# nanleij/ClusteredLowRankSolver.jl

Measured on AMD Instinct MI355X. Metric: interior-point iterations/sec, higher is better.
Workload: dtype f64x5 (multi-word fp64: 5 limbs per number, ~262 bits; problem data f64x5); 1 GPU; SpherePacking cohnelkies(8,15): d=8, 2d=30; 2 clusters P=32, blocks 16x16 r1 + 1x1 dense, N=31; whole interior-point iterations with the reference's default options at its precision (prec=256 -> 5 limbs), 55 per solve; clusters=2, n_free=31, limbs=5, data_limbs=5, multi_gpu=single GPU

## Files before the change

### clusteredlowranksolver.jl_amd/csrc/clrs_hip.hip

```cpp
#include <hip/hip_runtime.h>

#include <algorithm>
#include <array>
#include <climits>
#include <cmath>
#include <cstdio>
#include <cstdlib>
#include <cstring>
#include <map>
#include <string>
#include <vector>

#include "../../include/clrs_hip.h"
#include "clrs_kernels.hip.h"
#include "clrs_fused.hip.h"
#include "clrs_assemble_w3.hip.h"
#include "clrs_assemble_w4.hip.h"
#include "clrs_assemble_w5.hip.h"
#include "clrs_solve_small.hip.h"
#include "clrs_factor_small.hip.h"
#include "clrs_ipm.hip.h"

using namespace clrs;
typedef long long i64;

static thread_local std::string g_last_error;
static int fail(int code, const std::string &msg) {
    g_last_error = msg;
    return code;
}
extern "C" void clrs_set_last_error(const char *msg) { g_last_error = msg ? msg : ""; }
#define HIPCHECK(expr)                                                                                   \
    do {                                                                                                 \
        hipError_t e_ = (expr);                                                                          \
        if (e_ != hipSuccess)                                                                            \
            return fail(CLRS_ERR_HIP, std::string(#expr) + ": " + hipGetErrorString(e_));                \
    } while (0)

static const int INFO_NONE = 0x7f7f7f7f;

static int g_cfg_fused_assemble = 1;
static int g_cfg_split_blocks = 1;
static int g_cfg_fused_factor = 1;
static int g_cfg_wave_assemble = 1;
static int g_cfg_wave2_assemble = 1;
static int g_cfg_wave5_assemble = 1;
static int g_cfg_wave4_assemble = 1;
static int g_cfg_wave3_assemble = 1;
static int g_cfg_dense_block = 1;
static int g_cfg_trsm_blockinv = 1;
static int g_cfg_potrf_levels = 1;
static int g_cfg_pairing_tri = 1;
static int g_cfg_factor_aug = 1;
static int g_cfg_dense_wave = 1;
static int g_cfg_factor_small = 1;
static int g_cfg_solve_small_max = 32768;
static int g_cfg_ipm_wmfma = 3;
int g_cfg_mw_stream_words = 1;
int g_cfg_mw_pipeline64 = 1;
int g_cfg_mw_zt_small_maxn = 64;
int g_cfg_mw_pipeline_x = 1;
int g_cfg_mw_pipeline_x_min = 24;
int g_cfg_mw_sharded_factor_limbs = 1;
int g_cfg_mw_pipeline = 1;
int g_cfg_mw_refine_predictor = 0;
int g_cfg_mw_refine = 1;
int g_cfg_mw_affine_corrector = 1;
int g_cfg_mw_factor_limbs = 0;
int g_cfg_mw_exact_products = 1;
static int g_cfg_solve_small2 = 1;
static const int LDS_BUDGET_DOUBLES = 20000;

enum StepKind { STEP_MEMCPY, STEP_GEMM, STEP_TRSM, STEP_POTRF, STEP_GATHER_S, STEP_GATHER_SCALAR, STEP_SUB, STEP_MEMSET_INFO, STEP_ZERO_UPPER, STEP_FUSED_ASSEMBLE, STEP_SMALL_POTRF, STEP_CLUSTER_FACTOR, STEP_GEMV_T, STEP_CSOLVE_FWD, STEP_Q_SOLVE, STEP_CSOLVE_BWD, STEP_SUM_SLABS, STEP_ASSEMBLE_W1, STEP_GRAM_SMALL, STEP_ASSEMBLE_W2, STEP_SOLVE_SMALL, STEP_DENSE_BLOCK, STEP_ASSEMBLE_W3, STEP_FACTOR_SMALL, STEP_SUM_S_SLABS, STEP_TRTRI32, STEP_DENSE_T32, STEP_TRTRI_DIAG, STEP_COPY2D, STEP_CHOL_LEVEL, STEP_CHOL_PACK, STEP_CHOL_UNPACK, STEP_ASSEMBLE_W4, STEP_ASSEMBLE_W5, STEP_NKINDS };
static const char *const STEP_NAMES[STEP_NKINDS] = {"hipMemcpyAsync(D2D)", "k_gemm_f64_t", "k_trsm_diag", "k_potrf_diag", "k_schur_gather",
                                                    "k_gather_scalar", "k_sub", "hipMemsetAsync", "k_zero_upper", "k_cluster_assemble", "k_small_potrf", "k_cluster_factor", "k_gemv_t",
                                                    "k_cluster_solve_fwd", "k_q_solve", "k_cluster_solve_bwd", "k_sum_slabs", "k_cluster_assemble_w1", "k_gram_small", "k_cluster_assemble_w2", "k_solve_small", "k_dense_block", "k_cluster_assemble_w3", "k_factor_small", "k_sum_S_slabs", "k_trtri32", "k_dense_T32", "k_trtri_diag", "k_copy2d", "k_chol_level", "k_chol_pack", "k_chol_unpack", "k_cluster_assemble_w4", "k_cluster_assemble_w5"};
static const int KT_MAX_EVENTS = 8192;

struct Step {
    StepKind kind;
    int grid = 0;
    void *d0 = nullptr, *d1 = nullptr, *d2 = nullptr;
    void *dst = nullptr;
    const void *src = nullptr;
    size_t bytes = 0;
    i64 n = 0;
    int nmax = 0;
    int aux0 = 0, aux1 = 0;
    bool s_inverse = false;
};

struct Plan {
    std::vector<Step> steps;
    hipGraphExec_t graph = nullptr;
    const void *captured[8] = {nullptr, nullptr, nullptr, nullptr, nullptr, nullptr, nullptr, nullptr};
    int launches() const { return (int)steps.size(); }
};

struct DeviceArena {
    char *base = nullptr;
    size_t size = 0, used = 0;
};

struct TrsmJob {
    const double *L;
    int ldl, n;
    double *B;
    int ldb, nrhs;
};
struct PotrfJob {
    double *A;
    int lda, n, code;
    int stop = 0;
// ... 2453 lines not shown
    c->kt_kinds.clear();
    return 0;
}

extern "C" int clrs_set_kernel_timing(clrs_ctx *c, int kind) {
    if (!c || kind < -2 || kind >= STEP_NKINDS) return fail(CLRS_ERR_INVALID, "bad kernel kind");
    int rc = kt_collect(c);
    if (rc) return rc;
    c->kt_kind = kind;
    for (int k = 0; k < STEP_NKINDS; k++) { c->kt_total[k] = 0; c->kt_count[k] = 0; }
    return 0;
}

extern "C" int clrs_get_kernel_times(clrs_ctx *c, int max_kinds, double *seconds, int64_t *launches) {
    if (!c || !seconds || !launches) return fail(CLRS_ERR_INVALID, "null argument");
    int rc = kt_collect(c);
    if (rc) return rc;
    for (int k = 0; k < max_kinds && k < STEP_NKINDS; k++) { seconds[k] = c->kt_total[k]; launches[k] = c->kt_count[k]; }
    return STEP_NKINDS;
}

extern "C" int clrs_config_set(const char *key, int value) {
    if (!key) return fail(CLRS_ERR_INVALID, "null argument");
    if (!std::strcmp(key, "fused_assemble")) { g_cfg_fused_assemble = value; return 0; }
    if (!std::strcmp(key, "split_blocks")) { g_cfg_split_blocks = value; return 0; }
    if (!std::strcmp(key, "fused_factor")) { g_cfg_fused_factor = value; return 0; }
    if (!std::strcmp(key, "wave_assemble")) { g_cfg_wave_assemble = value; return 0; }
    if (!std::strcmp(key, "wave2_assemble")) { g_cfg_wave2_assemble = value; return 0; }
    if (!std::strcmp(key, "wave3_assemble")) { g_cfg_wave3_assemble = value; return 0; }
    if (!std::strcmp(key, "wave4_assemble")) { g_cfg_wave4_assemble = value; return 0; }
    if (!std::strcmp(key, "wave5_assemble")) { g_cfg_wave5_assemble = value; return 0; }
    if (!std::strcmp(key, "dense_block")) { g_cfg_dense_block = value; return 0; }
    if (!std::strcmp(key, "dense_wave")) { g_cfg_dense_wave = value; return 0; }
    if (!std::strcmp(key, "factor_aug")) { g_cfg_factor_aug = value; return 0; }
    if (!std::strcmp(key, "pairing_tri")) { g_cfg_pairing_tri = value; return 0; }
    if (!std::strcmp(key, "potrf_levels")) { g_cfg_potrf_levels = value; return 0; }
    if (!std::strcmp(key, "trsm_blockinv")) { g_cfg_trsm_blockinv = value; return 0; }
    if (!std::strcmp(key, "solve_small2")) { g_cfg_solve_small2 = value; return 0; }
    if (!std::strcmp(key, "factor_small")) { g_cfg_factor_small = value; return 0; }
    if (!std::strcmp(key, "pin_limit")) { PIN_LIMIT = (size_t)std::max(value, 0); return 0; }
    if (!std::strcmp(key, "ipm_wmfma")) { g_cfg_ipm_wmfma = value; return 0; }
    if (!std::strcmp(key, "solve_small_max")) { g_cfg_solve_small_max = value; return 0; }
    if (!std::strcmp(key, "mw_exact_products")) { g_cfg_mw_exact_products = value; return 0; }
    if (!std::strcmp(key, "mw_refine")) { g_cfg_mw_refine = value; return 0; }
    if (!std::strcmp(key, "mw_factor_limbs")) { g_cfg_mw_factor_limbs = value; return 0; }
    if (!std::strcmp(key, "mw_affine_corrector")) { g_cfg_mw_affine_corrector = value; return 0; }
    if (!std::strcmp(key, "mw_pipeline")) { g_cfg_mw_pipeline = value; return 0; }
    if (!std::strcmp(key, "mw_pipeline64")) { g_cfg_mw_pipeline64 = value; return 0; }
    if (!std::strcmp(key, "mw_zt_small_maxn")) { g_cfg_mw_zt_small_maxn = value; return 0; }
    if (!std::strcmp(key, "mw_pipeline_x")) { g_cfg_mw_pipeline_x = value; return 0; }
    if (!std::strcmp(key, "mw_pipeline_x_min")) { g_cfg_mw_pipeline_x_min = value; return 0; }
    if (!std::strcmp(key, "mw_sharded_factor_limbs")) { g_cfg_mw_sharded_factor_limbs = value; return 0; }
    if (!std::strcmp(key, "mw_stream_words")) { g_cfg_mw_stream_words = value; return 0; }
    if (!std::strcmp(key, "mw_refine_predictor")) { g_cfg_mw_refine_predictor = value; return 0; }
    return fail(CLRS_ERR_INVALID, std::string("unknown configuration key ") + key);
}

#ifdef CLRS_W3_STAMPS
extern "C" int clrs_debug_cf_stamps(clrs_ctx *c, uint64_t out[16]) {
    if (!c || !out) return fail(CLRS_ERR_INVALID, "null argument");
    HIPCHECK(hipStreamSynchronize(c->stream));
    HIPCHECK(hipMemcpyFromSymbol(out, HIP_SYMBOL(g_cf_stamps), 16 * sizeof(uint64_t)));
    return 0;
}
extern "C" int clrs_debug_ss2_stamps(clrs_ctx *c, uint64_t out[16]) {
    if (!c || !out) return fail(CLRS_ERR_INVALID, "null argument");
    HIPCHECK(hipStreamSynchronize(c->stream));
    HIPCHECK(hipMemcpyFromSymbol(out, HIP_SYMBOL(g_ss2_stamps), 16 * sizeof(uint64_t)));
    return 0;
}
extern "C" int clrs_debug_w3_stamps(clrs_ctx *c, uint64_t out[16]) {
    if (!c || !out) return fail(CLRS_ERR_INVALID, "null argument");
    HIPCHECK(hipStreamSynchronize(c->stream));
    HIPCHECK(hipMemcpyFromSymbol(out, HIP_SYMBOL(g_w3_stamps), 16 * sizeof(uint64_t)));
    return 0;
}
#endif

extern "C" int clrs_debug_stamps(clrs_ctx *c, uint64_t out[64]) {
    if (!c || !out) return fail(CLRS_ERR_INVALID, "null argument");
    if (!c->ftables.stamps) { std::memset(out, 0, 64 * sizeof(uint64_t)); return 0; }
    HIPCHECK(hipStreamSynchronize(c->stream));
    HIPCHECK(hipMemcpy(out, c->ftables.stamps, 64 * sizeof(uint64_t), hipMemcpyDeviceToHost));
    return 0;
}

extern "C" int clrs_fused_clusters(const clrs_ctx *c) { return c ? c->n_fused_clusters : 0; }
extern "C" int clrs_wave_clusters(const clrs_ctx *c) { return c ? c->n_wave_clusters + c->n_wave2_clusters : 0; }
extern "C" int clrs_wave2_clusters(const clrs_ctx *c) { return c ? c->n_wave2_clusters : 0; }
extern "C" int clrs_wave4_clusters(const clrs_ctx *c) { return c ? c->n_wave4_clusters : 0; }
extern "C" int clrs_wave5_clusters(const clrs_ctx *c) { return c ? c->n_wave5_clusters : 0; }

extern "C" const char *clrs_kernel_name(int kind) { return (kind >= 0 && kind < STEP_NKINDS) ? STEP_NAMES[kind] : ""; }

extern "C" const char *clrs_strerror(int code) {
    switch (code) {
        case CLRS_OK: return "ok";
        case CLRS_ERR_INVALID: return "invalid argument or malformed SDP description";
        case CLRS_ERR_HIP: return "HIP runtime error";
        case CLRS_ERR_NO_DEVICE: return "no usable HIP device";
        case CLRS_ERR_STATE: return "call order violated";
        default: return code > 0 ? "factorisation failure (non-positive pivot)" : "unknown error";
    }
}
extern "C" const char *clrs_last_error(void) { return g_last_error.c_str(); }
extern "C" const char *clrs_version(void) { return "clrs-hip 0.1.0 (gfx950)"; }
// ... 127 lines not shown
```

### clusteredlowranksolver.jl_amd/csrc/clrs_mw.hip

```cpp
#include <hip/hip_runtime.h>

#include <dlfcn.h>

#include <algorithm>
#include <condition_variable>
#include <cstdio>
#include <cstring>
#include <map>
#include <mutex>
#include <string>
#include <tuple>
#include <vector>

#include "../../include/clrs_hip.h"
#include "clrs_mw_kernels.hip.h"
#include "clrs_mw_pipe.hip.h"
#include "clrs_mw_exact.hip.h"
#include "clrs_mw_ipm.hip.h"
#include "clrs_mw_rank.hip.h"
#include "clrs_mw_inst.h"
#ifdef MW_SPLIT_UNITS
MW_KERNELS_ALL(extern template, 4)
MW_KERNELS_ALL(extern template, 5)
MW_KERNELS_ALL(extern template, 6)
MW_KERNELS_ALL(extern template, 8)
MW_KERNELS_ALL(extern template, 10)
#endif

typedef long long i64;

extern int g_cfg_mw_stream_words;
extern int g_cfg_mw_pipeline64;
extern int g_cfg_mw_zt_small_maxn;
extern int g_cfg_mw_pipeline_x, g_cfg_mw_pipeline_x_min;
extern int g_cfg_mw_sharded_factor_limbs;
extern int g_cfg_mw_pipeline;
extern int g_cfg_mw_refine_predictor;
extern int g_cfg_mw_refine;
extern int g_cfg_mw_exact_products;
extern int g_cfg_mw_affine_corrector;
extern int g_cfg_mw_factor_limbs;
extern "C" void clrs_set_last_error(const char *msg);

static int mw_fail(int code, const std::string &msg) {
    clrs_set_last_error(msg.c_str());
    return code;
}
#define MWCHECK(expr)                                                                                    \
    do {                                                                                                 \
        hipError_t e_ = (expr);                                                                          \
        if (e_ != hipSuccess) return mw_fail(CLRS_ERR_HIP, std::string(#expr) + ": " + hipGetErrorString(e_)); \
    } while (0)

typedef struct { char internal[128]; } mw_nccl_id;
struct MwNccl {
    void *lib = nullptr;
    int (*GetUniqueId)(mw_nccl_id *) = nullptr;
    int (*CommInitRank)(void **, int, mw_nccl_id, int) = nullptr;
    int (*CommDestroy)(void *) = nullptr;
    int (*AllGather)(const void *, void *, size_t, int, void *, hipStream_t) = nullptr;
    const char *(*GetErrorString)(int) = nullptr;
};
static MwNccl g_nccl;
static int mw_nccl_load() {
    if (g_nccl.lib) return 0;
    const char *names[] = {"librccl.so.1", "librccl.so", "/opt/rocm/lib/librccl.so.1"};
    void *h = nullptr;
    for (const char *n : names) if ((h = dlopen(n, RTLD_NOW | RTLD_NOLOAD))) break;
    for (const char *n : names) { if (h) break; h = dlopen(n, RTLD_NOW | RTLD_GLOBAL); }
    if (!h) return mw_fail(CLRS_ERR_INVALID, std::string("RCCL is not available: ") + dlerror());
    g_nccl.GetUniqueId = (int (*)(mw_nccl_id *))dlsym(h, "ncclGetUniqueId");
    g_nccl.CommInitRank = (int (*)(void **, int, mw_nccl_id, int))dlsym(h, "ncclCommInitRank");
    g_nccl.CommDestroy = (int (*)(void *))dlsym(h, "ncclCommDestroy");
    g_nccl.AllGather = (int (*)(const void *, void *, size_t, int, void *, hipStream_t))dlsym(h, "ncclAllGather");
    g_nccl.GetErrorString = (const char *(*)(int))dlsym(h, "ncclGetErrorString");
    if (!g_nccl.GetUniqueId || !g_nccl.CommInitRank || !g_nccl.CommDestroy || !g_nccl.AllGather) return mw_fail(CLRS_ERR_INVALID, "RCCL symbols missing");
    g_nccl.lib = h;
    return 0;
}
#define NCCLCHECK(expr)                                                                                                          \
    do {                                                                                                                         \
        int r_ = (expr);                                                                                                         \
        if (r_ != 0) return mw_fail(CLRS_ERR_HIP, std::string(#expr) + ": " + (g_nccl.GetErrorString ? g_nccl.GetErrorString(r_) : "RCCL error")); \
// ... 35 lines not shown
    bool xinv_valid = false;
    bool lds_x = false, lds_q = false, lds_zt_L = false, dense_two = false;
    int nw_factor = 1;
    int maxcnt = 0;
    double *vz = nullptr;
    bool wide_solve = false;
    const double *ride_fwd = nullptr;
    const int *ride_wait = nullptr;
    int ride_wait_value = 0;
    bool fwd_rode = false;
    int n_one_term = 0, n_many_term = 0;
    int sa_lanes = MW_SA_W;
    int maxTb = 0;
    size_t sm_x = 0, sm_zt = 0, sm_dense = 0, sm_factor = 0, sm_q = 0, sm_fwd = 0, sm_mid = 0, sm_bwd = 0;
    int *h_info = nullptr;
    double *d_Xin = nullptr, *d_Xc = nullptr, *d_Y = nullptr, *d_rx = nullptr, *d_ry = nullptr, *d_dx = nullptr, *d_dy = nullptr;
    bool assembled = false, factored = false;
    bool timing = false;
    hipEvent_t ev[8] = {nullptr, nullptr, nullptr, nullptr, nullptr, nullptr, nullptr, nullptr};
    double times[6] = {0, 0, 0, 0, 0, 0};
    double cnt_mul = 0;
    double cnt_factor = 0, cnt_solve = 0;
    struct MwIpm *ipm = nullptr;
    size_t sm_bp_diag = 0, sm_bp_panel = 0, sm_bp_inv = 0;
    std::vector<MwBp> bp_S, bp_Q;
    const MwBp *d_bp = nullptr;
    bool any_lds_cluster = false;
    void *comm = nullptr;
    void *comm_side = nullptr;
    clrs_mw_local_group *lgroup = nullptr;
    bool local_factored = false, fwd_done = false;
    const double *split_rhs_x = nullptr;
    bool refine_ready = false;
    MwdDev mwd = {};
    int mwd_blocks = 0, mwd_tasks = 0;
    size_t sm_mwd = 0;
    MwxDev mwx = {};
    int mwx_blocks = 0, mwx_maxU16 = 0;
    MwsDev mws = {};
    int mws_blocks = 0;
    int mws_turns = 1;
    size_t sm_mws = 0;
    bool pipe_bp = false;
    bool pipe_S64 = false;
    bool pipe_X = false;
    unsigned long long *pipe_pcx = nullptr;
    double *xpipe_L = nullptr, *xpipe_rd = nullptr;
    int *xpipe_info = nullptr;
    bool pipe_S = false, pipe_Q = false;
    unsigned long long *pipe_pc64 = nullptr;
    int pipe_pcQ = 0;
    unsigned pipe_epoch = 0;
    bool stream_words = true;
    bool refine_skip_next = false;
    int refine_predictor = 0;
    int refine = 1;
    bool ipm_arms_info = false;
    int kf_low = 0, kf_entry = 0;
};

template <class T>
static int mw_upload(clrs_mw_ctx *c, const std::vector<T> &h, const T **d) {
    T *p = nullptr;
    size_t bytes = std::max<size_t>(h.size(), 1) * sizeof(T);
    MWCHECK(hipMalloc((void **)&p, bytes));
    c->allocs.push_back(p);
    if (!h.empty()) MWCHECK(hipMemcpy(p, h.data(), h.size() * sizeof(T), hipMemcpyHostToDevice));
    *d = p;
    return 0;
}
static int mw_dmalloc(clrs_mw_ctx *c, double **d, i64 n) {
    size_t bytes = (size_t)std::max<i64>(n, 1) * sizeof(double);
    MWCHECK(hipMalloc((void **)d, bytes));
    c->allocs.push_back(*d);
    MWCHECK(hipMemset(*d, 0, bytes));
    return 0;
}

#define MW_CASE(Kc, Dc, ...) if (c_K_ == Kc && c_D_ == Dc) { constexpr int KK = Kc; constexpr int DD = Dc; __VA_ARGS__; } else
#define MW_DISPATCH(ctx, ...)                                                                                       \
    do {                                                                                                            \
        const int c_K_ = (ctx)->K, c_D_ = (ctx)->DK;                                                                \
        MW_CASE(2, 1, __VA_ARGS__) MW_CASE(2, 2, __VA_ARGS__) MW_CASE(3, 1, __VA_ARGS__) MW_CASE(3, 2, __VA_ARGS__)  \
        MW_CASE(4, 1, __VA_ARGS__) MW_CASE(4, 2, __VA_ARGS__) MW_CASE(5, 1, __VA_ARGS__) MW_CASE(5, 2, __VA_ARGS__)  \
        MW_CASE(6, 1, __VA_ARGS__) MW_CASE(6, 2, __VA_ARGS__) MW_CASE(8, 1, __VA_ARGS__) MW_CASE(8, 2, __VA_ARGS__)  \
        MW_CASE(10, 1, __VA_ARGS__) MW_CASE(10, 2, __VA_ARGS__)                                                      \
        MW_CASE(3, 3, __VA_ARGS__) MW_CASE(4, 4, __VA_ARGS__) MW_CASE(5, 5, __VA_ARGS__) MW_CASE(6, 6, __VA_ARGS__)  \
        MW_CASE(8, 8, __VA_ARGS__) MW_CASE(10, 10, __VA_ARGS__)                                                      \
        return mw_fail(CLRS_ERR_INVALID, "limbs must be 2..6, 8 or 10 and data limbs 1, 2 or the limbs");           \
    } while (0)

template <class F>
static int mw_set_lds(F kernel, size_t bytes) {
    if (bytes > 48 * 1024) MWCHECK(hipFuncSetAttribute((const void *)kernel, hipFuncAttributeMaxDynamicSharedMemorySize, (int)bytes));
    return 0;
}

extern "C" void clrs_mw_destroy(clrs_mw_ctx *c);
static void mw_ipm_free(clrs_mw_ctx *c);
static int mw_launch_xrd(clrs_mw_ctx *c, const double *d_Xc);

extern "C" int clrs_mw_create_opts(const clrs_sdp_desc *d, int data_limbs, int device, int limbs, const clrs_mw_options *opts, clrs_mw_ctx **out);
extern "C" int clrs_mw_create(const clrs_sdp_desc *d, int device, int limbs, clrs_mw_ctx **out) {
    return clrs_mw_create_opts(d, 1, device, limbs, nullptr, out);
}
extern "C" int clrs_mw_create_ex(const clrs_sdp_desc *d, int data_limbs, int device, int limbs, clrs_mw_ctx **out) {
// ... 200 lines not shown
            (one ? c->n_one_term : c->n_many_term)++;
        }
    }
    c->cnt_mul = cnt_mul;
    for (int j = 0; j < J; j++) {
        const double P = c->clu[j].P;
        c->cnt_factor += P * P * P / 6.0 + 0.5 * P * P * N + 0.5 * P * (double)N * N;
        c->cnt_solve += P * P + 2.0 * P * N;
    }
    c->cnt_factor += (double)N * N * N / 6.0;
    c->cnt_solve += (double)N * N;
    const size_t lim = MW_LDS_MAX / sizeof(double);
    {
        size_t nn = (size_t)c->maxn * c->maxn * K;
        size_t bcw = MW_POTRF_SCR(K, (size_t)c->maxn);
        c->lds_x = nn + bcw <= lim;
        size_t xneed = (c->lds_x ? nn : 0) + bcw;
        for (auto &k : c->blk) {
            const size_t one = (size_t)k.n * k.n * K + MW_POTRF_SCR(K, (size_t)k.n) + (size_t)K * k.n;
            const size_t two = one + (size_t)MW_TRI(k.n) * K;
            k.inv = !c->lds_x ? 0 : two <= lim ? 1 : one <= lim ? 2 : 0;
            if (k.inv) xneed = std::max(xneed, k.inv == 1 ? two : one);
        }
        c->all_inv = !c->blk.empty();
        for (auto &k : c->blk) c->all_inv = c->all_inv && (k.kind != 0 || k.inv != 0);
        c->sm_x = xneed * 8;
        size_t zt = (size_t)c->maxn * MW_CT * K;
        c->lds_zt_L = zt + nn <= lim;
        c->sm_zt = (zt + (c->lds_zt_L ? nn : 0)) * 8;
        if (zt > lim) MW_BAIL(CLRS_ERR_INVALID, "PSD block too large for the multi-word kernels");
        size_t maxnd = 0;
        for (auto &k : c->blk) if (k.kind != 0 && k.n > 1) maxnd = std::max(maxnd, (size_t)k.n);
        if (maxnd * maxnd * K > lim) MW_BAIL(CLRS_ERR_INVALID, "dense block too large for the multi-word kernels");
        c->dense_two = 2 * maxnd * maxnd * K <= lim;
        c->sm_dense = (c->dense_two ? 2 : 1) * maxnd * maxnd * K * 8;
        size_t fmax = 0;
        for (auto &q : c->clu) {
            const size_t need = ((size_t)q.P * q.P + (size_t)MW_TRI(q.P)) * K + MW_POTRF_SCR(K, (size_t)q.P);
            q.lds = need <= lim ? 1 : 0;
            if (q.lds) fmax = std::max(fmax, need);
        }
        c->sm_factor = std::max<size_t>(fmax, 1) * 8;
        c->nw_factor = std::max(1, std::min(MW_INV_WG, 256 / std::max(J, 1)));
        c->sm_fwd = 2 * (size_t)c->maxP * K * 8;
        c->sm_bwd = 3 * (size_t)c->maxP * K * 8;
        const size_t qn = (size_t)N * N * K;
        const size_t qneed = qn + (size_t)MW_TRI(N) * K + MW_POTRF_SCR(K, (size_t)N);
        c->lds_q = qneed <= lim;
        c->sm_q = (c->lds_q ? qneed : 1) * 8;
        c->sm_mid = 2 * (size_t)std::max(N, 1) * K * 8;
        if (c->sm_fwd > MW_LDS_MAX || c->sm_mid > MW_LDS_MAX) MW_BAIL(CLRS_ERR_INVALID, "cluster too large for the multi-word solve kernels");
    }
    MW_DISPATCH(c, {
        MW_TRY(mw_set_lds(k_mw_potrf_x<KK>, c->sm_x)); MW_TRY(mw_set_lds(k_mw_zt<KK, DD>, c->sm_zt)); MW_TRY(mw_set_lds((k_mw_dense_t<KK, DD>), c->sm_dense));
        constexpr int KC = mw_kc(KK);
        const size_t bw = std::min(c->sm_mid + c->sm_bwd, MW_LDS_MAX);
        MW_TRY(mw_set_lds(k_mw_factor<KK>, c->sm_factor)); MW_TRY(mw_set_lds(k_mw_potrf_q<KK>, c->lds_q ? std::max(c->sm_q, c->sm_fwd) : c->sm_fwd));
        MW_TRY(mw_set_lds(k_mw_solve_fwd<KK>, c->sm_fwd)); MW_TRY(mw_set_lds((k_mw_solve_mid<KK, KK>), c->sm_mid)); MW_TRY(mw_set_lds((k_mw_solve_mid<KK, KC>), c->sm_mid));
        MW_TRY(mw_set_lds((k_mw_solve_bwd<KK, KK, DD, 0>), bw)); MW_TRY(mw_set_lds((k_mw_solve_bwd<KK, KK, DD, 1>), bw)); MW_TRY(mw_set_lds((k_mw_solve_bwd<KK, KK, DD, 2>), bw));
        MW_TRY(mw_set_lds((k_mw_solve_bwd<KK, KC, DD, 1>), bw)); MW_TRY(mw_set_lds((k_mw_solve_bwd<KK, KC, DD, 2>), bw));
    });
    std::vector<long long> mws_off((size_t)std::max(NB, 1), -1);
    {
        const int S = mws_slices(K);
        std::vector<float> hVs;
        std::vector<int> hVe, hve_off((size_t)std::max(NB, 1), 0), hsv((size_t)std::max(NB, 1), 0);
        for (int b = 0; b < NB; b++) {
            const MwBlk &k = c->blk[b];
            if (k.kind != 0 || !k.inv || k.n > 32) continue;
            const int n = k.n, U = k.U, np = (n + 3) & ~3, n16 = (n + 15) & ~15, U16 = (U + 15) & ~15, rV = mws_rowstride(U16);
            if ((n16 / 16) * (U16 / 16) > 4 || mws_lds_bytes(S, mws_sv_class(S, 1), n, U) > MW_LDS_MAX) continue;
            if (2 * (n16 / 16) * (U16 / 16) > 4) c->mws_turns = 2;
            mws_off[b] = (long long)hVs.size();
            hve_off[b] = (int)hVe.size();
            hVs.resize(hVs.size() + (size_t)S * np * rV, 0.0f);
            hVe.resize(hVe.size() + U16, 0);
            float *dst = hVs.data() + mws_off[b];
            int sv = 0;
            for (int u = 0; u < U; u++) {
                double mx = 0;
                for (int i = 0; i < n; i++) mx = std::max(mx, std::fabs(hVl[0][k.v_off + (i64)u * n + i]));
                const int e = mwk::mws_exponent(mx);
                hVe[hve_off[b] + u] = e;
                for (int i = 0; i < n; i++) {
                    mwa::mw<2> x;
                    x.l[0] = hVl[0][k.v_off + (i64)u * n + i];
                    x.l[1] = DK > 1 ? hVl[1][k.v_off + (i64)u * n + i] : 0.0;
                    double r0 = std::ldexp(x.l[0], -e), r1 = std::ldexp(x.l[1], -e);
                    for (int s = 0; s < S; s++) {
                        const double g = std::ldexp(1.0, -(s + 1) * MWS_BETA), C = 0x1.8p52 * g;
                        volatile double tv = r0 + C;
                        const double t = tv - C;
                        const float dgt = (float)(t * std::ldexp(1.0, (s + 1) * MWS_BETA));
                        dst[(size_t)s * np * rV + (size_t)i * rV + mws_col(i, u, U16)] = dgt;
                        if (dgt != 0.0f) sv = std::max(sv, s + 1);
                        r0 -= t;
                        double sm, er;
                        mwa::two_sum(r0, r1, sm, er);
                        r0 = sm; r1 = er;
                    }
                }
            }
            if (mws_lds_bytes(S, mws_sv_class(S, sv), n, U) > MW_LDS_MAX) {
                hVs.resize((size_t)mws_off[b]); hVe.resize((size_t)hve_off[b]);
                mws_off[b] = -1;
                continue;
            }
// ... 141 lines not shown
                for (int r = 0; r < P; r++) hBs[(size_t)l * std::max<i64>(Bp, 1) + c->clu[j].coff + r + (i64)a * xlen] = d->B[(i64)l * Bp + off + r + (i64)a * P];
            off += (i64)P * N;
        }
    }
    q.Vp = std::max<i64>((i64)hVl[0].size(), 1); q.dAp = std::max<i64>((i64)hdAl[0].size(), 1); q.lamp = std::max<i64>(T, 1); q.Bp = std::max<i64>(Bp, 1);
    hV.assign((size_t)q.Vp * DK, 0.0);
    hdA.assign((size_t)q.dAp * DK, 0.0);
    for (int l = 0; l < DK; l++) {
        std::copy(hVl[l].begin(), hVl[l].end(), hV.begin() + (size_t)l * q.Vp);
        std::copy(hdAl[l].begin(), hdAl[l].end(), hdA.begin() + (size_t)l * q.dAp);
    }
    MW_TRY(mw_upload(c, c->blk, &q.blk)); MW_TRY(mw_upload(c, c->clu, &q.clu));
    MW_TRY(mw_upload(c, lr_list, &q.lr_list)); MW_TRY(mw_upload(c, dn_list, &q.dn_list));
    MW_TRY(mw_upload(c, hV, &q.V)); MW_TRY(mw_upload(c, hvrow, &q.vrow));
    MW_TRY(mw_upload(c, st_a, &q.st_a)); MW_TRY(mw_upload(c, st_b, &q.st_b)); MW_TRY(mw_upload(c, st_lam, &q.st_lam));
    MW_TRY(mw_upload(c, htptr, &q.tptr));
    MW_TRY(mw_upload(c, st_orig, &q.st_orig)); MW_TRY(mw_upload(c, st_p, &q.st_p)); MW_TRY(mw_upload(c, st_war, &q.st_war)); MW_TRY(mw_upload(c, st_wac, &q.st_wac));
    MW_TRY(mw_upload(c, st_trl, &q.st_trl)); MW_TRY(mw_upload(c, st_trd, &q.st_trd)); MW_TRY(mw_upload(c, st_flag, &q.st_flag));
    MW_TRY(mw_upload(c, ay_a, &q.ay_a)); MW_TRY(mw_upload(c, ay_b, &q.ay_b)); MW_TRY(mw_upload(c, ay_blk, &q.ay_blk));
    MW_TRY(mw_upload(c, hdA, &q.dA)); MW_TRY(mw_upload(c, hdmap, &q.dmap)); MW_TRY(mw_upload(c, hdense_p, &q.dense_p));
    {
        std::sort(drow_pairs.begin(), drow_pairs.end());
        std::vector<int> hptr((size_t)xlen + 1, 0), hblk, hen;
        for (auto &t : drow_pairs) hptr[(size_t)std::get<0>(t) + 1]++;
        for (i64 g = 0; g < xlen; g++) hptr[(size_t)g + 1] += hptr[(size_t)g];
        for (auto &t : drow_pairs) { hblk.push_back(std::get<1>(t)); hen.push_back(std::get<2>(t)); }
        MW_TRY(mw_upload(c, hptr, &q.drow_ptr)); MW_TRY(mw_upload(c, hblk, &q.drow_blk)); MW_TRY(mw_upload(c, hen, &q.drow_en));
        q.dn_big = 0;
        for (auto &k : c->blk) if (k.kind != 0) { c->maxcnt = std::max(c->maxcnt, k.cnt); if (k.n > 1) q.dn_big = 1; }
        q.maxcnt = c->maxcnt;
    }
    MW_TRY(mw_upload(c, hBs, &q.B));
    MW_TRY(mw_dmalloc(c, &q.Z, q.zlen * K)); MW_TRY(mw_dmalloc(c, &q.Tm, q.zlen * K));
    MW_TRY(mw_dmalloc(c, &q.GX, q.glen * K)); MW_TRY(mw_dmalloc(c, &q.GY, q.glen * K));
    MW_TRY(mw_dmalloc(c, &q.W, q.wlen * K)); MW_TRY(mw_dmalloc(c, &q.Sd, q.sdlen * K));
    MW_TRY(mw_dmalloc(c, &q.S, Slen * K)); MW_TRY(mw_dmalloc(c, &q.LB, xlen * (i64)N * K)); MW_TRY(mw_dmalloc(c, &q.Q, (i64)N * N * K));
    MW_TRY(mw_dmalloc(c, &q.Si, Slen * K)); MW_TRY(mw_dmalloc(c, &q.Qi, (i64)N * N * K));

    MW_TRY(mw_dmalloc(c, &q.Xf, xyoff * K)); MW_TRY(mw_dmalloc(c, &q.Xb, xyoff * K)); MW_TRY(mw_dmalloc(c, &q.Xi, xyoff * K));
    MW_TRY(mw_dmalloc(c, &q.xrd, rdoff * K)); MW_TRY(mw_dmalloc(c, &q.srd, xlen * K)); MW_TRY(mw_dmalloc(c, &q.qrd, (i64)N * K));
    MW_TRY(mw_dmalloc(c, &q.t, xlen * K)); MW_TRY(mw_dmalloc(c, &q.u, (i64)J * N * K)); MW_TRY(mw_dmalloc(c, &q.AY, T * K));
    q.AX = nullptr;
    q.aff_mu = q.aff_rhs = q.aff_t = q.aff_u = nullptr; q.aff_wait = nullptr; q.ride2_rhs = nullptr; q.ride2_t = q.ride2_u = nullptr;
    MW_TRY(mw_dmalloc(c, &c->vz, 2 * (i64)N * K));
    MW_TRY(mw_dmalloc(c, &q.S0, Slen * K)); MW_TRY(mw_dmalloc(c, &q.ub, (i64)J * N * K));
    MW_TRY(mw_dmalloc(c, &q.rx2, xlen * K)); MW_TRY(mw_dmalloc(c, &q.dx2, xlen * K));
    MW_TRY(mw_dmalloc(c, &q.u2, (i64)N * K)); MW_TRY(mw_dmalloc(c, &q.dy2, (i64)N * K));
    q.uadd = nullptr;
    c->refine = cfg_refine;
    c->refine_predictor = cfg_refine_pred;
    {
        const char *e = std::getenv("CLRS_MW_STREAM_WORDS");
        c->stream_words = e && *e ? std::atoi(e) != 0 : g_cfg_mw_stream_words != 0;
    }
    c->wide_solve = c->maxP > 64 || N > 64;
    MW_TRY(mw_dmalloc(c, &c->d_Xin, xyoff * K)); MW_TRY(mw_dmalloc(c, &c->d_Xc, xyoff * K)); MW_TRY(mw_dmalloc(c, &c->d_Y, xyoff * K));
    MW_TRY(mw_dmalloc(c, &c->d_rx, xlen * K)); MW_TRY(mw_dmalloc(c, &c->d_dx, xlen * K));
    MW_TRY(mw_dmalloc(c, &c->d_ry, (i64)N * K)); MW_TRY(mw_dmalloc(c, &c->d_dy, (i64)N * K));
    {
        int *info = nullptr;
        MWCHECK(hipMalloc((void **)&info, 2 * sizeof(int)));
        c->allocs.push_back(info);
        q.info = info;
        int init[2] = {MW_INFO_NONE, MW_INFO_NONE};
        MWCHECK(hipMemcpy(info, init, sizeof(init), hipMemcpyHostToDevice));
        int *pc = nullptr;
        MWCHECK(hipMalloc((void **)&pc, (size_t)(2 * J + 3) * sizeof(int)));
        c->allocs.push_back(pc);
        MWCHECK(hipMemset(pc, 0, (size_t)(2 * J + 3) * sizeof(int)));
        q.pcnt = pc;
    }
    {
        for (int j = 0; j < J; j++) {
            const MwClu &cl = c->clu[j];
            if (cl.lds) { c->any_lds_cluster = true; continue; }
            c->bp_S.push_back(MwBp{q.S + cl.Soff, q.Si + cl.Soff, q.srd + cl.coff, q.Slen, q.xlen, cl.P, cl.P, j + 1, 0, (int)c->bp_S.size(), 0});
        }
        if (N > 0) c->bp_Q.push_back(MwBp{q.Q, q.Qi, q.qrd, (i64)N * N, (i64)N, N, N, J + 1, 0, (int)c->bp_S.size(), 0});
        std::vector<MwBp> all = c->bp_S;
        all.insert(all.end(), c->bp_Q.begin(), c->bp_Q.end());
        MW_TRY(mw_upload(c, all, &c->d_bp));
    }
    {
        bool small = c->maxP <= MWP_N;
        for (auto &cl : c->clu) small = small && cl.lds;
        c->pipe_S = cfg_pipe != 0 && (K <= 6 || cfg_pipe >= 2) && small && (i64)J * ((MWP_N / MWP_W) + MWP_WW) <= 256;
        c->pipe_Q = (cfg_pipe >= 2 || (cfg_pipe == 1 && K <= 6 && N > MWP_W)) && N > 0 && N <= MWP_N;
        bool lds_all = !c->clu.empty();
        for (auto &cl : c->clu) lds_all = lds_all && cl.lds;
        c->pipe_S64 = cfg_pipe != 0 && K <= 6 && lds_all && c->maxP > MWP_N && c->maxP <= MWP_N64 && (i64)J * 16 <= 256 && g_cfg_mw_pipeline64 != 0 &&
                      (cfg_pipe >= 2 || c->maxP >= 48);
        const size_t nbp = c->bp_S.size() + c->bp_Q.size();
        const bool any_bp = !c->bp_S.empty() || (N > 0 && !c->lds_q);
        c->pipe_bp = cfg_pipe != 0 && any_bp && (i64)std::max<size_t>(c->bp_S.size(), 1) * ((MWP_N / MWP_W) + MWP_WW) <= 256;
        q.pipe_pc = nullptr;
        q.pipe_stamps = nullptr;
        q.pipe_bp = 0;
        {
            bool all_inv = c->d.NB > 0 && c->lds_x;
            int maxn_x = 0;
            i64 working = 0;
            for (auto &kb : c->blk) {
                all_inv = all_inv && kb.inv == 1;
                maxn_x = std::max(maxn_x, kb.n);
                working += 2 * ((kb.n + MWP_W - 1) / MWP_W + (kb.n > MWP_N ? MWP_N64 / MWP_W : MWP_WW));
            }
            c->pipe_X = cfg_pipe != 0 && K <= 6 && all_inv && maxn_x <= MWP_N64 && g_cfg_mw_pipeline_x != 0 &&
                        (cfg_pipe >= 2 || (maxn_x >= g_cfg_mw_pipeline_x_min && working <= 256));
            if (c->pipe_X) {
                double *pcx = nullptr, *ti = nullptr;
                MW_TRY(mw_dmalloc(c, &pcx, (i64)2 * c->d.NB * MWP_PC_WORDS_N(K, MWP_N64)));
                c->pipe_pcx = (unsigned long long *)pcx;
                MW_TRY(mw_dmalloc(c, &c->xpipe_L, c->d.xylen * K));
                MW_TRY(mw_dmalloc(c, &c->xpipe_rd, c->d.xrdlen * K));
                MW_TRY(mw_dmalloc(c, &ti, c->d.NB + 1));
                c->xpipe_info = (int *)ti;
                MW_DISPATCH(c, { if constexpr (KK <= 6) { MW_TRY(mw_set_lds(k_mw_potrf_x_pipe<KK>, MWP_LDS_ALONE64)); } });
            }
        }
        if (c->pipe_S64) {
            const size_t words64 = (size_t)J * MWP_PC_WORDS_N(K, MWP_N64);
            unsigned long long *pc64 = nullptr;
            if (hipMalloc((void **)&pc64, words64 * sizeof(unsigned long long)) != hipSuccess) MW_BAIL(CLRS_ERR_HIP, "hipMalloc failed");
            c->allocs.push_back(pc64);
            if (hipMemset(pc64, 0xff, words64 * sizeof(unsigned long long)) != hipSuccess) MW_BAIL(CLRS_ERR_HIP, "hipMemset failed");
            c->pipe_pc64 = pc64;
            MW_DISPATCH(c, { if constexpr (KK <= 6) { MW_TRY(mw_set_lds(k_mw_factor_pipe64<KK>, MWP_LDS_ALONE64)); } });
        }
        if (c->pipe_S || c->pipe_Q || c->pipe_bp) {
            const size_t own = (size_t)(c->pipe_S ? J : 0) + 1;
            const size_t words = (own + (c->pipe_bp ? nbp : 0)) * MWP_PC_WORDS(K);
            unsigned long long *pc = nullptr;
            if (hipMalloc((void **)&pc, words * sizeof(unsigned long long)) != hipSuccess) MW_BAIL(CLRS_ERR_HIP, "hipMalloc failed");
            c->allocs.push_back(pc);
            if (hipMemset(pc, 0xff, words * sizeof(unsigned long long)) != hipSuccess) MW_BAIL(CLRS_ERR_HIP, "hipMemset failed");
            q.pipe_pc = pc;
            c->pipe_pcQ = c->pipe_S ? J : 0;
            q.pipe_q = c->pipe_pcQ;
            q.pipe_bp = (int)own;
            MW_DISPATCH(c, {
                MW_TRY(mw_set_lds(k_mw_factor_pipe<KK>, MWP_LDS_ALONE));
                MW_TRY(mw_set_lds(k_mw_potrf_q_pipe<KK>, std::max<size_t>(MWP_LDS_ALONE, c->sm_fwd)));
                MW_TRY(mw_set_lds(k_mw_bp_diag_pipe<KK>, std::max<size_t>(MWP_LDS_ALONE, c->sm_factor)));
            });
        }
    }
    const int MW_PB = MW_PB_OF(K);
    c->sm_bp_diag = ((size_t)MW_POTRF_SCR(K, MW_PB) + (size_t)K * MW_PB * MW_PB + (size_t)K * MW_TRI(MW_PB) + (size_t)K * MW_PB) * 8;
    c->sm_bp_panel = (size_t)K * MW_BP_PR * MW_PB * 8;
    c->sm_bp_inv = (size_t)K * MW_PB * MW_BP_IC * 8;
    MW_DISPATCH(c, { MW_TRY(mw_set_lds(k_mw_bp_diag<KK>, std::max(c->sm_bp_diag, c->sm_factor))); MW_TRY(mw_set_lds(k_mw_bp_panel<KK>, c->sm_bp_panel)); MW_TRY(mw_set_lds(k_mw_bp_inv<KK>, c->sm_bp_inv)); MW_TRY(mw_set_lds(k_mw_bp_inv_row<KK>, c->sm_bp_inv)); });
    q.rank = 0; q.world = 1; q.gathered = 0;
    MW_TRY(mw_dmalloc(c, &q.Qg, (i64)N * N * K)); MW_TRY(mw_dmalloc(c, &q.ug, (i64)N * K));
    {
        bool all_lds = true;
        for (auto &cl : c->clu) all_lds = all_lds && cl.lds;
        (void)all_lds;
        const bool may = mw_kf_of(K) < K && c->refine == 1;
        c->kf_low = may ? mw_kf_of(K) : K;
// ... 13 lines not shown
    return 0;
#undef MW_BAIL
#undef MW_TRY
}

extern "C" void clrs_mw_destroy(clrs_mw_ctx *c) {
    if (!c) return;
    (void)hipSetDevice(c->device);
    if (c->stream) (void)hipStreamSynchronize(c->stream);
    mw_ipm_free(c);
    if (c->comm && g_nccl.CommDestroy) { (void)g_nccl.CommDestroy(c->comm); c->comm = nullptr; }
    if (c->comm_side && g_nccl.CommDestroy) { (void)g_nccl.CommDestroy(c->comm_side); c->comm_side = nullptr; }
    if (c->lgroup) { std::lock_guard<std::mutex> lk(c->lgroup->m); c->lgroup->attached--; c->lgroup = nullptr; }
    for (void *p : c->allocs) (void)hipFree(p);
    for (auto &e : c->ev) if (e) (void)hipEventDestroy(e);
    if (c->h_info) (void)hipHostFree(c->h_info);
    if (c->stream && c->own_stream) (void)hipStreamDestroy(c->stream);
    delete c;
}

extern "C" int clrs_mw_limbs(const clrs_mw_ctx *c) { return c ? c->K : 0; }
extern "C" void *clrs_mw_stream(clrs_mw_ctx *c) { return c ? (void *)c->stream : nullptr; }
extern "C" int clrs_mw_set_stream(clrs_mw_ctx *c, void *stream) {
    if (!c) return mw_fail(CLRS_ERR_INVALID, "null context");
    if (c->own_stream && c->stream) { (void)hipStreamSynchronize(c->stream); (void)hipStreamDestroy(c->stream); }
    c->stream = (hipStream_t)stream;
    c->own_stream = false;
    return 0;
}
extern "C" int clrs_mw_get_dims(const clrs_mw_ctx *c, clrs_dims *o) {
    if (!c || !o) return mw_fail(CLRS_ERR_INVALID, "null argument");
    o->xy_len = c->d.xylen; o->x_len = c->d.xlen; o->S_len = c->d.Slen; o->n_terms = c->d.T;
    o->n_free = c->d.N; o->n_clusters = c->d.J; o->n_blocks = c->d.NB; o->reserved = c->K;
    return 0;
}
extern "C" int clrs_mw_get_unique_count(const clrs_mw_ctx *c, int32_t block, int32_t *n_unique) {
    if (!c || !n_unique || block < 0 || block >= c->d.NB) return mw_fail(CLRS_ERR_INVALID, "bad argument");
    *n_unique = c->blk[block].U;
    return 0;
}
extern "C" int clrs_mw_set_timing(clrs_mw_ctx *c, int on) {
    if (!c) return mw_fail(CLRS_ERR_INVALID, "null context");
    c->timing = on != 0;
    return 0;
}
extern "C" int clrs_mw_get_counters(const clrs_mw_ctx *c, double *assemble_muladds, double *factor_muladds, double *solve_muladds) {
    if (!c) return mw_fail(CLRS_ERR_INVALID, "null context");
    if (assemble_muladds) *assemble_muladds = c->cnt_mul;
    if (factor_muladds) *factor_muladds = c->cnt_factor;
    if (solve_muladds) *solve_muladds = c->cnt_solve;
    return 0;
}

static int mw_reset_info(clrs_mw_ctx *c, int which) {
    if (c->ipm_arms_info) return 0;
    MWCHECK(hipMemsetAsync(c->d.info + which, 0x7f, sizeof(int), c->stream));
    return 0;
}
static int mw_read_info(clrs_mw_ctx *c, int which, int *status) {
    MWCHECK(hipMemcpyAsync(c->h_info + which, c->d.info + which, sizeof(int), hipMemcpyDeviceToHost, c->stream));
    MWCHECK(hipStreamSynchronize(c->stream));
    *status = c->h_info[which] == MW_INFO_NONE ? 0 : c->h_info[which];
    return 0;
}

static int mw_cholesky_blocks_dev2(clrs_mw_ctx *c, const double *d_X, double *d_Xchol, const double *d_Y2, double *d_Yi, int *d_yfail) {
    if (!c || !d_X || !d_Xchol) return mw_fail(CLRS_ERR_INVALID, "null argument");
    MWCHECK(hipSetDevice(c->device));
    int rc;
    if ((rc = mw_reset_info(c, 1))) return rc;
    if (c->d.NB == 0) return 0;
    const int grid = d_Y2 ? 2 * c->d.NB : c->d.NB;
    bool in_mem = false;
    for (auto &k : c->blk) in_mem = in_mem || k.inv == 2 || mw_x_shares(k);
    if (c->pipe_X) {
        c->pipe_epoch = (c->pipe_epoch + 1) & 0x3ffffff;
        MW_DISPATCH(c, { if constexpr (KK <= 6) { hipLaunchKernelGGL(k_mw_potrf_x_pipe<KK>, dim3(mwp_blocks64(grid)), dim3(MWP_NT64), MWP_LDS_ALONE64, c->stream, c->d, d_X, d_Xchol, d_Y2, d_Yi, d_yfail,
                                                                     c->xpipe_L, c->xpipe_rd, c->xpipe_info, c->pipe_pcx, c->pipe_epoch); } });
    } else
    MW_DISPATCH(c, hipLaunchKernelGGL(k_mw_potrf_x<KK>, dim3(grid, in_mem && c->lds_x ? MW_INV_WG : 1), dim3(MW_PT), c->sm_x, c->stream, c->d, d_X, d_Xchol, c->lds_x ? 1 : 0, d_Y2, d_Yi, d_yfail));
    MWCHECK(hipGetLastError());
    c->xinv_valid = true;
    return 0;
}
extern "C" int clrs_mw_cholesky_blocks_dev(clrs_mw_ctx *c, const double *d_X, double *d_Xchol) { return mw_cholesky_blocks_dev2(c, d_X, d_Xchol, nullptr, nullptr, nullptr); }
extern "C" int clrs_mw_sync_status_cholesky(clrs_mw_ctx *c) {
    if (!c) return mw_fail(CLRS_ERR_INVALID, "null context");
    int st = 0, rc;
    if ((rc = mw_read_info(c, 1, &st))) return rc;
    return st;
}

extern "C" int clrs_mw_schur_assemble_dev(clrs_mw_ctx *c, const double *d_Xchol, const double *d_Y) {
    if (!c || !d_Xchol || !d_Y) return mw_fail(CLRS_ERR_INVALID, "null argument");
    MWCHECK(hipSetDevice(c->device));
    const MwDev &q = c->d;
    if (c->timing) MWCHECK(hipEventRecord(c->ev[0], c->stream));
    MW_DISPATCH(c, {
        const bool exact = c->mws_blocks > 0 && c->xinv_valid;
        bool dense_done = exact && q.ndn && !q.dn_big;
        const int pair_grid = q.nlr + (dense_done ? q.ndn : 0);
        if constexpr (DD <= 2) {
            if (exact && c->mws_turns == 1) hipLaunchKernelGGL((k_mws_pair<KK, DD, 1>), dim3(pair_grid), dim3(MWS_NT), c->sm_mws, c->stream, q, c->mws, d_Y);
            else if (exact) hipLaunchKernelGGL((k_mws_pair<KK, DD, 2>), dim3(pair_grid), dim3(MWS_NT), c->sm_mws, c->stream, q, c->mws, d_Y);
        }
        if (q.nlr && !(exact && c->mws_blocks == q.nlr)) {
            MwDev q2 = q;
            q2.mws_on = exact ? 1 : 0;
            const int gper = MW_NT / MW_GRAM_W;
            const int zt_ct = (c->xinv_valid && c->all_inv && (i64)q.nlr * c->maxU <= 2048 && c->maxn <= g_cfg_mw_zt_small_maxn) ? 2 : MW_CT;
            hipLaunchKernelGGL((k_mw_zt<KK, DD>), dim3((c->maxU + zt_ct - 1) / zt_ct, q.nlr), dim3(MW_NT), c->sm_zt, c->stream, q2, d_Y, c->lds_zt_L ? 1 : 0, c->xinv_valid ? 1 : 0, zt_ct);
            const bool ride_gram = !dense_done && q.ndn && !q.dn_big;
            dense_done = dense_done || ride_gram;
            q2.mwx_on = c->mwx_blocks > 0 ? 1 : 0;
            hipLaunchKernelGGL((k_mw_gram<KK, DD>), dim3((c->maxU * (c->maxU + 1) / 2 + gper - 1) / gper, q.nlr + (ride_gram ? q.ndn : 0)), dim3(MW_NT), 0, c->stream, q2, d_Y);
            if (q2.mwx_on) {
                const int nt = c->mwx_maxU16 / 16;
                hipLaunchKernelGGL(k_mwx_slice<KK>, dim3(nt, 2, q.nlr), dim3(MWS_NT), 0, c->stream, q2, c->mwx);
                hipLaunchKernelGGL(k_mwx_gram<KK>, dim3((nt * (nt + 1) / 2 + MWS_NT / 64 - 1) / (MWS_NT / 64), 2, q.nlr), dim3(MWS_NT), 0, c->stream, q2, c->mwx);
            }
        }
        if (q.ndn && !dense_done) {
            const bool panels = c->xinv_valid && c->maxn_dense > 16 && c->maxn_dense <= MW_NT;
            MwDev q3 = q;
            q3.mwd_on = (panels && c->mwd_blocks > 0) ? 1 : 0;
            hipLaunchKernelGGL((k_mw_dense_t<KK, DD>), dim3(q.ndn, q.dn_big ? c->maxcnt : 1), dim3(MW_NT), c->sm_dense, c->stream, q3, d_Y, c->xinv_valid ? 1 : 0, c->dense_two ? 1 : 0, panels ? 1 : 0);
            if (panels) {
                const int pcmin = std::max(1, MW_NT / c->maxn_dense);
                if (c->mwd_blocks < q.ndn)
                    hipLaunchKernelGGL((k_mw_dense_tp<KK, DD>), dim3(q.ndn, c->maxcnt, (c->maxn_dense + pcmin - 1) / pcmin), dim3(MW_NT), (size_t)2 * KK * MW_NT * 8, c->stream, q3, d_Y);
                c->mwd.stamps = c->mws.stamps;
                if constexpr (DD <= 2) { if (q3.mwd_on) hipLaunchKernelGGL((k_mwx_dense<KK, DD>), dim3(c->mwd_tasks), dim3(MWS_NT), c->sm_mwd, c->stream, q3, c->mwd, d_Y); }
            }
            const int pairs = c->maxcnt * (c->maxcnt + 1) / 2;
            const int ds_lanes = c->maxn_dense * c->maxn_dense <= 128 ? 8 : c->maxn_dense * c->maxn_dense <= 512 ? 16 : 64;
            if (q.dn_big) hipLaunchKernelGGL((k_mw_dense_s<KK, DD>), dim3(q.ndn, (pairs + MW_NT / ds_lanes - 1) / (MW_NT / ds_lanes)), dim3(MW_NT), 0, c->stream, q, ds_lanes);
        }
        if (c->n_many_term) hipLaunchKernelGGL((k_mw_saccum<KK, DD>), dim3((c->maxP * (c->maxP + 1) / 2 * c->sa_lanes + MW_NT - 1) / MW_NT, q.J), dim3(MW_NT), 0, c->stream, q, c->sa_lanes);
        if (c->n_one_term) hipLaunchKernelGGL((k_mw_saccum_one<KK, DD>), dim3((c->maxP * (c->maxP + 1) / 2 + MW_NT - 1) / MW_NT, q.J), dim3(MW_NT), 0, c->stream, q, c->n_many_term ? 0 : 1);
    });
    MWCHECK(hipGetLastError());
    if (c->timing) MWCHECK(hipEventRecord(c->ev[1], c->stream));
    c->assembled = true;
    c->factored = false;
    c->local_factored = false;
    return 0;
}


extern "C" int clrs_comm_unique_id(void *id128) {
    if (!id128) return mw_fail(CLRS_ERR_INVALID, "null argument");
    int rc = mw_nccl_load();
    if (rc) return rc;
    NCCLCHECK(g_nccl.GetUniqueId((mw_nccl_id *)id128));
    return 0;
}

extern "C" int clrs_mw_set_shard(clrs_mw_ctx *c, int rank, int world) {
    if (!c || world < 1 || rank < 0 || rank >= world) return mw_fail(CLRS_ERR_INVALID, "bad rank / world");
    MWCHECK(hipSetDevice(c->device));
    MWCHECK(hipStreamSynchronize(c->stream));
    MwDev &q = c->d;
    if (world != q.world) {
// ... 694 lines not shown
```

### clusteredlowranksolver.jl_amd/csrc/clrs_mw_inst.h

```cpp
#ifndef CLRS_MW_INST_H
#define CLRS_MW_INST_H

#define MW_KERNELS_K(X, K)                                                                                             \
    X __global__ void k_mw_potrf_x<K>(const MwDev, const double *, double *, int, const double *, double *, int *);    \
    X __global__ void k_mw_factor<K>(const MwDev);                                                                     \
    X __global__ void k_mw_qgram<K>(const MwDev, int);                                                                 \
    X __global__ void k_mw_potrf_q<K>(const MwDev, int, const double *, const int *, int);                             \
    X __global__ void k_mw_factor_pipe<K>(const MwDev, unsigned);                                                      \
    X __global__ void k_mw_factor_pipe64<K>(const MwDev, unsigned);                                                    \
    X __global__ void k_mw_potrf_x_pipe<K>(const MwDev, const double *, double *, const double *, double *, int *, double *, double *, int *, unsigned long long *, unsigned); \
    X __global__ void k_mw_potrf_q_pipe<K>(const MwDev, unsigned, const double *, const int *, int);                   \
    X __global__ void k_mw_bp_diag_pipe<K>(const MwDev, const MwBp *, int, int, unsigned, int, int);                   \
    X __global__ void k_mw_bp_inv_row<K>(const MwDev, const MwBp *, int);                                               \
    X __global__ void k_mw_qsum<K>(const MwDev);                                                                       \
    X __global__ void k_mw_bp_diag<K>(const MwDev, const MwBp *, int, int);                                             \
    X __global__ void k_mw_bp_panel<K>(const MwDev, const MwBp *, int);                                                \
    X __global__ void k_mw_bp_syrk<K>(const MwDev, const MwBp *, int);                                                 \
    X __global__ void k_mw_bp_inv<K>(const MwDev, const MwBp *, int);                                                  \
    X __global__ void k_mw_bp_finish<K>(const MwDev, const MwBp *);                                                    \
    X __global__ void k_mw_usum<K>(const MwDev);                                                                       \
    X __global__ void k_mw_keep_S<K>(const MwDev);                                                                     \
    X __global__ void k_mw_solve_fwd<K>(const MwDev, const double *);                                                  \
    X __global__ void k_mw_solve_mid<K, K>(const MwDev, const double *, double *);                                     \
    X __global__ void k_mw_solve_mid<K, mw_kc(K)>(const MwDev, const double *, double *);                              \
    X __global__ void k_mw_solve_wide<K>(const MwDev, int, const double *, const double *, double *, double *, double *);\
    X __global__ void k_mw_xrd<K>(const MwDev, const double *);                                                        \
    X __global__ void k_mwi_R<K>(const MwDev, const MwIpmDev, int);                                                    \
    X __global__ void k_mwi_Z<K>(const MwDev, const MwIpmDev, int, int);                                               \
    X __global__ void k_mwi_Zi<K>(const MwDev, const MwIpmDev, int);                                                   \
    X __global__ void k_mwi_bmm<K>(const MwDev, const MwIpmDev, int, int);                                             \
    X __global__ void k_mwx_slice<K>(const MwDev, const MwxDev);                                                       \
    X __global__ void k_mwx_gram<K>(const MwDev, const MwxDev);                                                        \
    X __global__ void k_mwi_update<K>(const MwDev, const MwIpmDev);                                                    \
    X __global__ void k_mwi_init<K>(const MwDev, const MwIpmDev, double, double);                                      \
    X __global__ void k_mw_rank_reveal<K>(const MwRankMat *, double *, double *, mwi64, double *, int *, int *, double *, mwi64);

#define MW_KERNELS_KD(X, K, DK)                                                                                        \
    X __global__ void k_mw_zt<K, DK>(const MwDev, const double *, int, int, int);                                      \
    X __global__ void k_mw_gram<K, DK>(const MwDev, const double *);                                                                   \
    X __global__ void k_mw_dense_t<K, DK>(const MwDev, const double *, int, int, int);                                 \
    X __global__ void k_mw_dense_tp<K, DK>(const MwDev, const double *);                                               \
    X __global__ void k_mw_dense_s<K, DK>(const MwDev, int);                                                           \
    X __global__ void k_mw_saccum<K, DK>(const MwDev, int);                                                                 \
    X __global__ void k_mw_saccum_one<K, DK>(const MwDev, int);                                                             \
    X __global__ void k_mw_linvb<K, DK>(const MwDev);                                                                  \
    X __global__ void k_mw_refine<K, DK>(const MwDev, int, const double *, double *, double *);                        \
    X __global__ void k_mw_solve_bwd<K, K, DK, 0>(const MwDev, const double *, double *, const double *, double *, const double *);        \
    X __global__ void k_mw_solve_bwd<K, K, DK, 1>(const MwDev, const double *, double *, const double *, double *, const double *);        \
    X __global__ void k_mw_solve_bwd<K, K, DK, 2>(const MwDev, const double *, double *, const double *, double *, const double *);        \
    X __global__ void k_mw_solve_bwd<K, mw_kc(K), DK, 1>(const MwDev, const double *, double *, const double *, double *, const double *); \
    X __global__ void k_mw_solve_bwd<K, mw_kc(K), DK, 2>(const MwDev, const double *, double *, const double *, double *, const double *); \
    X __global__ void k_mwi_scalar<K, DK>(const MwDev, const MwIpmDev, int, int);                                      \
    X __global__ void k_mwi_dots<K, DK>(const MwDev, const MwIpmDev, int, int);                                             \
    X __global__ void k_mwi_coef<K, DK>(const MwDev, const MwIpmDev, const double *);                                  \
    X __global__ void k_mwi_wA<K, DK>(const MwDev, const MwIpmDev, int, int, int);                                          \
    X __global__ void k_mwi_wB<K, DK>(const MwDev, const MwIpmDev, int);                                                    \
    X __global__ void k_mwi_MV<K, DK>(const MwDev, const double *);                                                    \
    X __global__ void k_mwi_rows_dn<K, DK>(const MwDev, const MwIpmDev, int);                                          \
    X __global__ void k_mwi_rows<K, DK>(const MwDev, const MwIpmDev, int, int);                                        \
    X __global__ void k_mwi_rows_fwd<K, DK>(const MwDev, const MwIpmDev);                                              \
    X __global__ void k_mwi_pv<K, DK>(const MwDev, const MwIpmDev, int);                                               \
    X __global__ void k_mwi_pvfin<K, DK>(const MwDev, const MwIpmDev);                                                 \
    X __global__ void k_mwi_gpack<K, DK>(const MwDev, const MwIpmDev, int);                                               \
    X __global__ void k_mwi_step<K, DK>(const MwDev, const MwIpmDev, int, int, int, int);

#define MW_KERNELS_KDX(X, K, DK)                                                                                       \
    X __global__ void k_mws_pair<K, DK, 1>(const MwDev, const MwsDev, const double *);                                 \
    X __global__ void k_mws_pair<K, DK, 2>(const MwDev, const MwsDev, const double *);                                 \
    X __global__ void k_mwx_dense<K, DK>(const MwDev, const MwdDev, const double *);

#define MW_KERNELS_ALL(X, K) MW_KERNELS_K(X, K) MW_KERNELS_KD(X, K, 1) MW_KERNELS_KDX(X, K, 1) MW_KERNELS_KD(X, K, 2) MW_KERNELS_KDX(X, K, 2) MW_KERNELS_KD(X, K, K)

#endif
```

### clusteredlowranksolver.jl_amd/csrc/clrs_mw_ipm.hip.h

```cpp

enum { MSC_MU = 0, MSC_MUS, MSC_XY, MSC_XdY, MSC_dXY, MSC_dXdY, MSC_CY, MSC_DOBJ, MSC_POBJ, MSC_GAP, MSC_COUNT = 16 };
enum { MREC_ITER = 0, MREC_MU, MREC_DOBJ, MREC_POBJ, MREC_GAP, MREC_DERR, MREC_PERR, MREC_AD, MREC_AP, MREC_BETA, MREC_MAXP, MREC_MAXp, MREC_MAXd,
       MREC_PDFEAS, MREC_ERR, MREC_FSTAT, MREC_XSTAT, MREC_REFB, MREC_COUNT = 24 };

struct MwIpmDev {
    double *x, *y, *X, *Y, *dx, *dy, *dX, *dY, *R, *Xc, *Pm, *d, *rhsx, *pv, *coef;
    double *Yi;
    int *yfail;
    int wBn;
    double *Zs;
    double *Zt;
    double *wB;
    int *zcnt;
    unsigned long long *stamps;
    double *dtr;
    double *sc, *part;
    unsigned long long *fmax;
    double *eig;
    double *Wd;
    int *wcnt;
    double *rec;
    int *flags;
    int klow, pad4;
    double *tau, *ttau, *utau;
    int *sync;
    const double *C, *c, *b;
    const int *row_clu;
    double sgn, constant;
    int Ktot, pad;
    double beta_infeasible, beta_feasible, gamma, dual_thr, primal_thr, max_gap, step_thr;
    int safe_step, corrector_only;
    double gap_thr;
    int stop_on, need_dual, need_primal, pad3;
    double *gsM, *gsS;
    int GL, Jglob;
    const int *clu_gid, *blk_gid;
};
#define MWG_S1(K, N) 0
#define MWG_S2(K, N) (K)
#define MWG_BX(K, N) (2 * (K))
#define MWG_D(K, N) (2 * (K) + (K) * (N))
#define MWG_XY(K, N) (MWG_D(K, N) + 8)
#define MWG_LEN(K, N) (MWG_D(K, N) + 8 + (K))

namespace mwk {

template <int K> __device__ __noinline__ mw<K> s_div(const mw<K> a, const mw<K> b) { return div<K>(a, b); }
template <int K> __device__ __noinline__ mw<K> s_mul(const mw<K> a, const mw<K> b) { return mul<K>(a, b); }
template <int K> __device__ __noinline__ mw<K> s_mul_d(const mw<K> a, double b) { return mul_d<K>(a, b); }
template <int K> __device__ __noinline__ mw<K> s_add(const mw<K> a, const mw<K> b) { return add<K>(a, b); }
template <int K> __device__ __noinline__ mw<K> s_sub(const mw<K> a, const mw<K> b) { return sub<K>(a, b); }
template <int K> __device__ __noinline__ mw<K> s_result(const acc<K> s) { return acc_result<K>(s); }
template <int K> __device__ __noinline__ mw<K> s_lanes64(const mw<K> v) { return lanes_sum<K, 64>(v); }
template <int K> __device__ __forceinline__ bool s_less(const mw<K> &a, const mw<K> &b) { return s_sub<K>(a, b).l[0] < 0.0; }

template <int K>
__device__ __noinline__ mw<K> wg_reduce_sum(const mw<K> &v, lds_d *red, int tid) {
    mw<K> w = lanes_sum<K, 64>(v);
    if ((tid & 63) == 0) stx<K>(red, MW_NT / 64, tid >> 6, w);
    __syncthreads();
    acc<K> s;
    acc_zero<K>(s);
#pragma unroll
    for (int i = 0; i < MW_NT / 64; i++) acc_add<K, K>(s, ldx<K>(red, MW_NT / 64, i));
    __syncthreads();
    return acc_result<K>(s);
}
__device__ __forceinline__ void atomic_max_abs(unsigned long long *slot, double v) {
    atomicMax(slot, (unsigned long long)__double_as_longlong(__builtin_fabs(v)));
}

__device__ __forceinline__ double wg_sum_d(double v, lds_d *red, int tid) {
#pragma unroll
    for (int off = 32; off > 0; off >>= 1) v += __shfl_xor(v, off, 64);
    if ((tid & 63) == 0) red[tid >> 6] = v;
    __syncthreads();
// ... 194 lines not shown
        d2[tid] = (tid < n) ? ldexp(dd[tid], -sexp) : 0.0;
        const double es = (tid >= 1 && tid < n) ? ldexp(ee[tid - 1], -sexp) : 0.0;
        e2s[tid] = es * es;
    }
    lo = ldexp(lo, -sexp) - 1e-3;
    hi = ldexp(hi, -sexp) + 1e-3;
    __syncthreads();
    MWS_STAMP(7);
    constexpr int ROUNDS = NT >= 1024 ? 6 : 7;
    for (int round = 0; round < ROUNDS; round++) {
        const double h = (hi - lo) * (1.0 / (NT + 1));
        const double sft = lo + h * (tid + 1);
        double pm = 1.0, pc = (d2[0] - sft) + 1e-300;
        auto hi32 = [](double v) { return (unsigned)(__double_as_longlong(v) >> 32); };
        unsigned cnt = hi32(pc) >> 31;
        auto step = [&](double tvu, double e2u) {
            const double pn = __builtin_fma(tvu, pc, __builtin_fma(-e2u, pm, 1e-300));
            cnt += (hi32(pn) ^ hi32(pc)) >> 31;
            pm = pc;
            pc = pn;
        };
        int i0 = 1;
        for (; i0 + 4 <= n; i0 += 4) {
#pragma unroll
            for (int u = 0; u < 4; u++) step(d2[i0 + u] - sft, e2s[i0 + u]);
            const int ex = __builtin_amdgcn_frexp_exp(pc);
            pc = ldexp(pc, -ex);
            pm = ldexp(pm, -ex);
        }
        for (; i0 < n; i0++) step(d2[i0] - sft, e2s[i0]);
        const unsigned long long zero = __ballot(cnt == 0u);
        if (lane == 0) zc[round & 1][wave] = __popcll(zero);
        __syncthreads();
        int idx = 0;
#pragma unroll
        for (int w = 0; w < NT / 64; w++) idx += zc[round & 1][w];
        const double nlo = lo + h * idx;
        hi = (idx == NT) ? hi : lo + h * (idx + 1);
        lo = nlo;
    }
    return ldexp(0.5 * (lo + hi), sexp);
}

}

template <int K>
__device__ __noinline__ mwa::mw<K> mwi_sum_part(const MwDev &q, const MwIpmDev &p, int slot) {
    using namespace mwk;
    acc<K> s;
    acc_zero<K>(s);
    for (int b = 0; b < q.NB; b++) acc_add<K, K>(s, ldx<K>(p.part, 5L * q.NB, (long)slot * q.NB + b));
    return acc_result<K>(s);
}
__device__ __forceinline__ bool mwi_last_block(int *counter, unsigned total) { return mwk::wg_last_block(counter, total); }
template <int K>
__device__ __noinline__ mwa::mw<K> mwi_gsum(const MwDev &q, const double *gs, int GL, int off) {
    using namespace mwk;
    acc<K> s;
    acc_zero<K>(s);
    for (int r = 0; r < q.world; r++) {
        mw<K> v;
#pragma unroll
        for (int l = 0; l < K; l++) v.l[l] = gs[(long)r * GL + off + l];
        acc_add<K, K>(s, v);
    }
    return acc_result<K>(s);
}
template <int K>
__device__ __forceinline__ void mwi_scalar_stage3(const MwDev &q, const MwIpmDev &p) {
    using namespace mwk;
    const bool pre = q.world <= 1 && q.NB <= 8;
    double pev[2][8];
#pragma unroll
    for (int w = 0; w < 2; w++)
#pragma unroll
        for (int b = 0; b < 8; b++) pev[w][b] = (pre && b < q.NB) ? p.eig[(long)w * q.NB + b] : 1e300;
    const int f0 = p.flags[0];
    int f1 = p.flags[1], f2 = p.flags[2];
    unsigned long long rs[4] = {0ull, 0ull, 0ull, 0ull};
    if (q.refstat) {
        if (q.world > 1) {
#pragma unroll
            for (int i = 0; i < 4; i++) {
                double m = 0.0;
                for (int r = 0; r < q.world; r++) m = fmax(m, p.gsM[(long)r * p.GL + MWG_S1(K, q.N) + i]);
                rs[i] = (unsigned long long)__double_as_longlong(m);
            }
        } else {
#pragma unroll
            for (int i = 0; i < 4; i++) rs[i] = q.refstat[i];
        }
    }
    double al[2];
    for (int w = 0; w < 2; w++) {
        double mn;
        if (q.world > 1) {
            mn = p.gsM[MWG_D(K, q.N) + 2 + w];
            for (int r = 1; r < q.world; r++) mn = fmin(mn, p.gsM[(long)r * p.GL + MWG_D(K, q.N) + 2 + w]);
            for (int r = 0; r < q.world; r++) if (p.gsM[(long)r * p.GL + MWG_D(K, q.N) + 6] != 0.0) f2 = 1;
        } else if (pre) {
            mn = pev[w][0];
#pragma unroll
            for (int b = 1; b < 8; b++) mn = fmin(mn, pev[w][b]);
        } else {
            mn = p.eig[(long)w * q.NB];
            for (int b = 1; b < q.NB; b++) mn = fmin(mn, p.eig[(long)w * q.NB + b]);
        }
        const bool unsafe = f0 && !p.safe_step;
        al[w] = (mn > -p.gamma && !unsafe) ? 1.0 : -p.gamma / mn;
    }
    if (f2 && f1 == 0) f1 = 1;
    double amin = fmin(al[0], al[1]);
    if (!(amin >= p.step_thr) && f1 == 0) f1 = 4;
    double refb = 0.0;
    if (q.refstat) {
        const double c0 = __longlong_as_double((long long)rs[0]), v0 = __longlong_as_double((long long)rs[1]);
        const double c1 = __longlong_as_double((long long)rs[2]), v1 = __longlong_as_double((long long)rs[3]);
        double ratio = 0.0;
        if (v0 > 0.0) ratio = fmax(ratio, c0 / v0);
        if (v1 > 0.0) ratio = fmax(ratio, c1 / v1);
        refb = (v0 > 0.0 || v1 > 0.0) ? (ratio > 0.0 ? fmin(1023.0, fmax(1.0, -log2(ratio))) : 1023.0) : 0.0;
    }
    p.flags[2] = f2;
    p.flags[1] = f1;
    p.rec[MREC_AD] = al[0]; p.rec[MREC_AP] = al[1];
    if (f0 && p.safe_step) al[0] = al[1] = amin;
    p.sc[MSC_COUNT * 0 + 10] = al[0];
    p.sc[MSC_COUNT * 0 + 11] = al[1];
    p.rec[MREC_ERR] = f1;
    if (q.refstat) {
        p.rec[MREC_REFB] = refb;
        q.refstat[0] = q.refstat[1] = q.refstat[2] = q.refstat[3] = 0ull;
    }
}
template <int K, int DK>
__device__ void mwi_scalar_stage(const MwDev &q, const MwIpmDev &p, int stage, int iter) {
    using namespace mwk;
    const long SP = MSC_COUNT;
    if (stage == 4) {
        const int lane = threadIdx.x;
        acc<K> s;
        acc_zero<K>(s);
        for (long i = lane; i < q.xlen; i += 64) acc_fma<K, K, DK>(s, ldx<K>(p.x, q.xlen, i), ldx<DK>(p.c, q.xlen, i), p.sgn);
        mw<K> cx = s_lanes64<K>(s_result<K>(s));
        acc_zero<K>(s);
        for (int a = lane; a < q.N; a += 64) acc_fma<K, K, DK>(s, ldx<K>(p.y, q.N, a), ldx<DK>(p.b, q.N, a));
        mw<K> by = s_lanes64<K>(s_result<K>(s));
        if (lane != 0) return;
        if (q.world > 1) cx = mwi_gsum<K>(q, p.gsS, p.GL, MWG_S2(K, q.N));
        mw<K> dobj = s_add<K>(cx, from_double<K>(p.constant));
        acc_zero<K>(s);
        acc_add<K, K>(s, q.world > 1 ? mwi_gsum<K>(q, p.gsS, p.GL, MWG_S1(K, q.N)) : mwi_sum_part<K>(q, p, 4));
        acc_add<K, K>(s, by);
        acc_add_d<K>(s, p.constant);
        mw<K> pobj = s_result<K>(s);
        mw<K> den = abs<K>(s_add<K>(dobj, pobj));
        if (s_less<K>(den, from_double<K>(1.0))) den = from_double<K>(1.0);
        mw<K> gap = s_div<K>(abs<K>(s_sub<K>(dobj, pobj)), den);
        stx<K>(p.sc, SP, MSC_DOBJ, dobj); stx<K>(p.sc, SP, MSC_POBJ, pobj); stx<K>(p.sc, SP, MSC_GAP, gap);
// ... 569 lines not shown
    using namespace mwk;
    const bool nomu = which == 2;
    if (nomu) which = 0;
    const MwBlk &k = q.blk[blockIdx.x];
    if (!k.inv) return;
    const int n = k.n, tid = threadIdx.x, sub = tid % MWI_ZL;
    const int zs = gridDim.y, pc0 = (n + zs - 1) / zs, c0 = blockIdx.y * pc0, pc = max(0, min(pc0, n - c0));
    const long np = (long)n * pc0;
    lds_d *M = MW_LDS, *M2 = M + (long)K * np;
    const double *A = (which == 0 ? p.Pm : p.dX) + k.xyoff, *Xi = q.Xi + k.xyoff;
    const double sg = which == 0 ? 1.0 : -1.0;
#ifdef CLRS_MW_STAMPS
    const bool stamp = p.stamps && blockIdx.x == 0 && blockIdx.y == 0 && tid == 0;
    int nst = 0;
#define MWZ_STAMP() do { if (stamp) p.stamps[nst++] = wall_clock64(); } while (0)
#else
#define MWZ_STAMP() do { } while (0)
#endif
    MWZ_STAMP();
    for (int e0 = 0; e0 < n * pc; e0 += MW_PT / MWI_ZL) {
        const int e = e0 + tid / MWI_ZL;
        const bool live = e < n * pc;
        const int ee = live ? e : 0, i = ee % n, c = c0 + ee / n;
        acc<KA> s;
        acc_zero<KA>(s);
        for (int kk = sub; kk < n; kk += MWI_ZL) acc_fma<KA, KA, KA>(s, ldx<KA>(A, q.xylen, i + (long)kk * n), ldx<KA>(p.Y + k.xyoff, q.xylen, kk + (long)c * n), sg);
        if (sub == 0) acc_add<KA, KA>(s, ldx<KA>(p.R + k.xyoff, q.xylen, i + (long)c * n), -sg);
        if (sub == 1 && i == c && !nomu) acc_add<KA, KA>(s, ldx<KA>(p.sc, MSC_COUNT, MSC_MUS), -sg);
        const mw<KA> v = lanes_sum<KA, MWI_ZL>(acc_result<KA>(s));
        if (live && sub == 0) stx<KA>(M, np, ee, v);
    }
    __syncthreads();
    MWZ_STAMP();
    for (int e0 = 0; e0 < n * pc; e0 += MW_PT / MWI_ZL) {
        const int e = e0 + tid / MWI_ZL;
        const bool live = e < n * pc;
        const int ee = live ? e : 0, i = ee % n, cl = ee / n;
        acc<KA> s;
        acc_zero<KA>(s);
        for (int r = sub; r <= i; r += MWI_ZL) acc_fma<KA, KA, KA>(s, ldx<KA>(Xi, q.xylen, i + (long)r * n), ldx<KA>(M, np, r + (long)cl * n));
        const mw<KA> v = lanes_sum<KA, MWI_ZL>(acc_result<KA>(s));
        if (live && sub == 0) stx<KA>(M2, np, ee, v);
    }
    __syncthreads();
    MWZ_STAMP();
    for (int e0 = 0; e0 < n * pc; e0 += MW_PT / MWI_ZL) {
        const int e = e0 + tid / MWI_ZL;
        const bool live = e < n * pc;
        const int ee = live ? e : 0, i = ee % n, cl = ee / n;
        acc<KA> s;
        acc_zero<KA>(s);
        for (int r = i + sub; r < n; r += MWI_ZL) acc_fma<KA, KA, KA>(s, ldx<KA>(Xi, q.xylen, r + (long)i * n), ldx<KA>(M2, np, r + (long)cl * n));
        const mw<KA> v = lanes_sum<KA, MWI_ZL>(acc_result<KA>(s));
        if (live && sub == 0) stx<K>(p.Zs + k.xyoff, q.xylen, i + (long)(c0 + cl) * n, cvt<K, KA>(v));
    }
    MWZ_STAMP();
    if (!mwi_last_block(&p.zcnt[blockIdx.x], zs)) return;
    MWZ_STAMP();
    for (int e = tid; e < n * n; e += MW_PT) {
        const int i = e % n, c = e / n;
        if (c > i) continue;
        const mw<K> v = cvt<K, KA>(mul_pow2<KA>(add<KA>(ldx<KA>(p.Zs + k.xyoff, q.xylen, i + (long)c * n), ldx<KA>(p.Zs + k.xyoff, q.xylen, c + (long)i * n)), 0.5));
        stx<K>(p.dY + k.xyoff, q.xylen, i + (long)c * n, v);
        stx<K>(p.dY + k.xyoff, q.xylen, c + (long)i * n, v);
    }
    MWZ_STAMP();
#undef MWZ_STAMP
}
template <int K>
__global__ __launch_bounds__(MW_PT) void k_mwi_Zi(const MwDev q, const MwIpmDev p, int which) {
    mw_mark(q);
    if constexpr (mw_kf_of(K) < K) { if (p.klow < K) { mwi_Zi_body<K, mw_kf_of(K)>(q, p, which); return; } }
    mwi_Zi_body<K, K>(q, p, which);
}

#ifndef MWI_BT
#define MWI_BT 8
#endif
template <int K>
__global__ __launch_bounds__(MW_NT) void k_mwi_bmm(const MwDev q, const MwIpmDev p, int op, int which) {
    using namespace mwk;
    const MwBlk &k = q.blk[blockIdx.y];
    if (!k.inv) return;
    const int n = k.n, nt = (n + MWI_BT - 1) / MWI_BT;
    if ((int)blockIdx.x >= nt * nt) return;
    const int ti = blockIdx.x % nt, tj = blockIdx.x / nt;
    if (op == 3) {
        if (tj > ti) return;
        const int e = threadIdx.x;
        if (e >= MWI_BT * MWI_BT) return;
        const int i = ti * MWI_BT + e % MWI_BT, c = tj * MWI_BT + e / MWI_BT;
        if (i >= n || c > i) return;
        mw<K> v = mul_pow2<K>(add<K>(ldx<K>(p.Zt + k.xyoff, q.xylen, i + (long)c * n), ldx<K>(p.Zt + k.xyoff, q.xylen, c + (long)i * n)), 0.5);
        stx<K>(p.dY + k.xyoff, q.xylen, i + (long)c * n, v);
        stx<K>(p.dY + k.xyoff, q.xylen, c + (long)i * n, v);
        return;
    }
    constexpr int LW = MW_NT / (MWI_BT * MWI_BT);
    const int e = threadIdx.x / LW, sub = threadIdx.x % LW;
    const int i0 = ti * MWI_BT + e % MWI_BT, c0 = tj * MWI_BT + e / MWI_BT;
    const bool live = i0 < n && c0 < n;
    const int wh = blockIdx.z;
    if (op >= 4) {
        if (n == 1 || (wh == 1 && p.yfail[blockIdx.y])) return;
        if (op == 5 && tj > ti) return;
    }
    const double *Lp, *Rp;
    int l_si, l_sk, r_sk, r_sc, k_lo = 0, k_hi = n;
    const double *Xi = q.Xi + k.xyoff;
    if (op == 0) { Lp = (which == 0 ? p.Pm : p.dX) + k.xyoff; l_si = 1; l_sk = n; Rp = p.Y + k.xyoff; r_sk = 1; r_sc = n; }
    else if (op == 1) { Lp = Xi; l_si = 1; l_sk = n; Rp = p.Zt + k.xyoff; r_sk = 1; r_sc = n; k_hi = min(n, ti * MWI_BT + MWI_BT); }
    else if (op == 2) { Lp = Xi; l_si = n; l_sk = 1; Rp = p.Zs + k.xyoff; r_sk = 1; r_sc = n; k_lo = ti * MWI_BT; }
    else if (op == 4) { Lp = (wh == 0 ? p.dX : p.dY) + k.xyoff; l_si = 1; l_sk = n; Rp = (wh == 0 ? q.Xi : p.Yi) + k.xyoff; r_sk = n; r_sc = 1; k_hi = min(n, tj * MWI_BT + MWI_BT); }
    else { Lp = (wh == 0 ? q.Xi : p.Yi) + k.xyoff; l_si = 1; l_sk = n; Rp = (wh == 0 ? p.Zs : p.Zt) + k.xyoff; r_sk = 1; r_sc = n; k_hi = min(n, ti * MWI_BT + MWI_BT); }
    const int klen = k_hi - k_lo;
// ... 53 lines not shown
}

template <int K, class PF, class PR, class PW>
__device__ __forceinline__ void mwi_step_congruence(PF F, PR rd, PW W, long wplane, long nn, int n, const double *dMg, long gplane, mwk::lds_d *Wd, int tid) {
    using namespace mwk;
    wg_copy<K>(W, wplane, n, dMg, gplane, n, n, n, tid);
    __syncthreads();
    wg_trsm_f<K>(F, nn, n, rd, n, n, W, wplane, n, n, tid);
    for (int e = tid; e < nn; e += MW_NT) {
        const int i = e % n, c = e / n;
        if (c >= i) continue;
        mw<K> a = ldx<K>(W, wplane, i + (long)c * n), b2 = ldx<K>(W, wplane, c + (long)i * n);
        stx<K>(W, wplane, i + (long)c * n, b2);
        stx<K>(W, wplane, c + (long)i * n, a);
    }
    __syncthreads();
    wg_trsm_f<K>(F, nn, n, rd, n, n, W, wplane, n, n, tid);
    for (int e = tid; e < nn; e += MW_NT) {
        const int i = e % n, c = e / n;
        Wd[e] = 0.5 * ((double)W[i + (long)c * n] + (double)W[c + (long)i * n]);
    }
}

#define MWI_SW 4
template <int K, int KA, int SW>
__device__ __forceinline__ bool mwi_step_panels_ka(const MwDev &q, const MwIpmDev &p, const MwBlk &k, int which, const double *Li, const double *dMg) {
    using namespace mwk;
    const int n = k.n, tid = threadIdx.x, sub = tid % SW;
    const int zs = gridDim.z, pc0 = (n + zs - 1) / zs, c0 = blockIdx.z * pc0, pc = max(0, min(pc0, n - c0));
    const long np = (long)n * pc0;
    lds_d *Us = MW_LDS;
    for (int e0 = 0; e0 < n * pc; e0 += MW_NT / SW) {
        const int e = e0 + tid / SW;
        const bool live = e < n * pc;
        const int ee = live ? e : 0, r = ee % n, c = c0 + ee / n;
        acc<KA> s;
        acc_zero<KA>(s);
        for (int t = sub; t <= c; t += SW) acc_fma<KA, KA, KA>(s, ldx<KA>(dMg, q.xylen, r + (long)t * n), ldx<KA>(Li, q.xylen, c + (long)t * n));
        const mw<KA> v = lanes_sum<KA, SW>(acc_result<KA>(s));
        if (live && sub == 0) stx<KA>(Us, np, ee, v);
    }
    __syncthreads();
    MWS_STAMP(1);
    double *Wg = p.Wd + (long)which * q.xylen + k.xyoff;
    for (int e0 = 0; e0 < n * pc; e0 += MW_NT / SW) {
        const int e = e0 + tid / SW;
        const bool live = e < n * pc;
        const int ee = live ? e : 0, i = ee % n, cl = ee / n, c = c0 + cl;
        acc<KA> s;
        acc_zero<KA>(s);
        if (i >= c)
            for (int r = sub; r <= i; r += SW) acc_fma<KA, KA, KA>(s, ldx<KA>(Li, q.xylen, i + (long)r * n), ldx<KA>(Us, np, r + (long)cl * n));
        const mw<KA> v = lanes_sum<KA, SW>(acc_result<KA>(s));
        if (live && sub == 0 && i >= c) Wg[i + (long)c * n] = v.l[0];
    }
    MWS_STAMP(2);
    return mwi_last_block(&p.wcnt[which * q.NB + blockIdx.x], zs);
}
template <int K>
__device__ __forceinline__ bool mwi_step_panels(const MwDev &q, const MwIpmDev &p, const MwBlk &k, int which, const double *Li, const double *dMg) {
    const bool wide = (int)gridDim.z >= k.n && k.n <= 16;
    if constexpr (mw_kf_of(K) < K) {
        if (q.kf < K) return wide ? mwi_step_panels_ka<K, mw_kf_of(K), 16>(q, p, k, which, Li, dMg) : mwi_step_panels_ka<K, mw_kf_of(K), MWI_SW>(q, p, k, which, Li, dMg);
    }
    return wide ? mwi_step_panels_ka<K, K, 16>(q, p, k, which, Li, dMg) : mwi_step_panels_ka<K, K, MWI_SW>(q, p, k, which, Li, dMg);
}

template <int K>
__device__ __forceinline__ bool mwi_step_body(const MwDev &q, const MwIpmDev &p, int w_in_lds, int inv_path, int which_base) {
    using namespace mwk;
    const int which = which_base + blockIdx.y;
    MWS_STAMP(0);
    const MwBlk &k = q.blk[blockIdx.x];
    const int n = k.n, tid = threadIdx.x;
    const long nn = (long)n * n;
    const double *Mg = (which == 0 ? p.X : p.Y) + k.xyoff, *dMg = (which == 0 ? p.dX : p.dY) + k.xyoff;
    if (blockIdx.z != 0 && (n == 1 || inv_path != 2 || (which == 1 && p.yfail[blockIdx.x]))) return false;
    if (n == 1) {
        if (tid == 0) {
            mw<K> m = ldx<K>(Mg, q.xylen, 0);
            if (!(m.l[0] > 0.0)) { p.flags[2] = 1; p.eig[(long)which * q.NB + blockIdx.x] = 0.0; }
            else p.eig[(long)which * q.NB + blockIdx.x] = div<K>(ldx<K>(dMg, q.xylen, 0), m).l[0];
        }
        return true;
    }
    if (inv_path >= 2) {
        lds_d *T1 = MW_LDS, *Wd = T1 + (long)K * nn, *work = Wd + nn;
        if (which == 1 && p.yfail[blockIdx.x]) {
            if (tid == 0) { p.flags[2] = 1; p.eig[(long)which * q.NB + blockIdx.x] = 0.0; }
            return true;
        }
        if (gridDim.z > 1 || inv_path == 3) {
            if (inv_path == 2 && !mwi_step_panels<K>(q, p, k, which, (which == 0 ? q.Xi : p.Yi) + k.xyoff, dMg)) return false;
            MWS_STAMP(3);
            lds_d *Wl = MW_LDS, *wk = Wl + nn;
            const double *Wg = p.Wd + (long)which * q.xylen + k.xyoff;
            for (int e = tid; e < nn; e += MW_NT) {
                const int i = e % n, c = e / n;
                Wl[e] = i >= c ? Wg[e] : Wg[c + (long)i * n];
            }
            __syncthreads();
            MWS_STAMP(4);
            const double ev = n <= 64 ? wg_min_eig32(Wl, n, wk, tid) : wg_min_eig(Wl, n, wk, tid);
            if (tid == 0) p.eig[(long)which * q.NB + blockIdx.x] = ev - 1e-5;
            MWS_STAMP(5);
            return true;
        }
        mwi_step_congruence_inv<K>((which == 0 ? q.Xi : p.Yi) + k.xyoff, q.xylen, n, dMg, q.xylen, T1, Wd, tid);
        __syncthreads();
        const double ev = n <= 64 ? wg_min_eig32(Wd, n, work, tid) : wg_min_eig(Wd, n, work, tid);
        if (tid == 0) p.eig[(long)which * q.NB + blockIdx.x] = ev - 1e-5;
        return true;
    }
    if (inv_path && k.inv == 1) {
        lds_d *Li = MW_LDS, *T1 = Li + (long)K * nn, *Mf = T1 + (long)K * nn;
        lds_d *rd = Mf + (long)K * nn, *Wd = rd + (long)K * n, *work = Wd + nn, *scr = work + 3 * n + 2 * MW_NT;
        if (which == 0) {
            mwi_step_congruence_inv<K>(q.Xi + k.xyoff, q.xylen, n, dMg, q.xylen, T1, Wd, tid);
        } else {
            wg_copy<K>(Mf, nn, n, Mg, q.xylen, n, n, n, tid);
            __syncthreads();
            if (!wg_potrf<K, true, MW_NT, false>(Mf, nn, n, n, rd, n, Li, nn, n, scr, tid)) {
                if (tid == 0) { p.flags[2] = 1; p.eig[(long)which * q.NB + blockIdx.x] = 0.0; }
                return true;
            }
            mwi_step_congruence_inv<K>(Li, nn, n, dMg, q.xylen, T1, Wd, tid);
        }
        __syncthreads();
        const double ev = n <= 64 ? wg_min_eig32(Wd, n, work, tid) : wg_min_eig(Wd, n, work, tid);
        if (tid == 0) p.eig[(long)which * q.NB + blockIdx.x] = ev - 1e-5;
        return true;
    }
    lds_d *F = MW_LDS;
    lds_d *Wl = F + (long)K * nn;
    lds_d *rd = w_in_lds ? Wl + (long)K * nn : Wl;
    lds_d *Wd = rd + (long)K * n, *work = Wd + nn, *bc = work + 3 * n + 2 * MW_NT;
    if (which == 0) {
        wg_copy<K>(F, nn, n, q.Xf + k.xyoff, q.xylen, n, n, n, tid);
        for (int i = tid; i < n; i += MW_NT) stx<K>(rd, n, i, ldx<K>(q.xrd + k.rd_off, q.xrdlen, i));
        __syncthreads();
    } else {
        wg_copy<K>(F, nn, n, Mg, q.xylen, n, n, n, tid);
        __syncthreads();
        if (!wg_potrf<K, false>(F, nn, n, n, rd, n, F, 0, 0, bc, tid)) {
            if (tid == 0) { p.flags[2] = 1; p.eig[(long)which * q.NB + blockIdx.x] = 0.0; }
            return true;
        }
        for (int e = tid; e < nn; e += MW_NT) {
            const int i = e % n, c = e / n;
            if (i > c) stx<K>(F, nn, e, mul<K>(ldx<K>(F, nn, e), ldx<K>(rd, n, i)));
        }
        __syncthreads();
    }
    if (w_in_lds) mwi_step_congruence<K>(F, rd, Wl, nn, nn, n, dMg, q.xylen, Wd, tid);
    else mwi_step_congruence<K>(F, rd, (which == 0 ? p.R : p.Pm) + k.xyoff, q.xylen, nn, n, dMg, q.xylen, Wd, tid);
    __syncthreads();
    const double ev = n <= 64 ? wg_min_eig32(Wd, n, work, tid) : wg_min_eig(Wd, n, work, tid);
    if (tid == 0) p.eig[(long)which * q.NB + blockIdx.x] = ev - 1e-5;
    return true;
}

template <int K>
__global__ __launch_bounds__(MW_NT) void k_mwi_update(const MwDev q, const MwIpmDev p) {
    using namespace mwk;
    if (p.flags[1] != 0 || p.flags[6] != 0) return;
    const double ad = p.sc[10], ap = p.sc[11];
    const mwi64 tot = q.xylen + q.xlen + q.N;
    for (mwi64 i = (mwi64)blockIdx.x * MW_NT + threadIdx.x; i < tot; i += (mwi64)gridDim.x * MW_NT) {
        if (i < q.xylen) {
            acc<K> s;
            acc_zero<K>(s);
            acc_add<K, K>(s, ldx<K>(p.X, q.xylen, i));
            acc_fma_d<K, K>(s, ldx<K>(p.dX, q.xylen, i), ad);
            stx<K>(p.X, q.xylen, i, acc_result<K>(s));
            acc_zero<K>(s);
            acc_add<K, K>(s, ldx<K>(p.Y, q.xylen, i));
            acc_fma_d<K, K>(s, ldx<K>(p.dY, q.xylen, i), ap);
            stx<K>(p.Y, q.xylen, i, acc_result<K>(s));
        } else if (i < q.xylen + q.xlen) {
            const mwi64 g = i - q.xylen;
            acc<K> s;
            acc_zero<K>(s);
            acc_add<K, K>(s, ldx<K>(p.x, q.xlen, g));
            acc_fma_d<K, K>(s, ldx<K>(p.dx, q.xlen, g), ad);
            stx<K>(p.x, q.xlen, g, acc_result<K>(s));
        } else {
            const mwi64 a = i - q.xylen - q.xlen;
            acc<K> s;
            acc_zero<K>(s);
            acc_add<K, K>(s, ldx<K>(p.y, q.N, a));
            acc_fma_d<K, K>(s, ldx<K>(p.dy, q.N, a), ap);
            stx<K>(p.y, q.N, a, acc_result<K>(s));
        }
    }
}

template <int K, int DK>
__global__ __launch_bounds__(MW_NT) void k_mwi_step(const MwDev q, const MwIpmDev p, int w_in_lds, int inv_path, int iter, int which_base) {
    if (!mwi_step_body<K>(q, p, w_in_lds, inv_path, which_base)) return;
    if (q.world > 1) return;
#ifdef CLRS_MW_STAMPS
    if (mwi_last_block(&p.flags[4], 2u * q.NB)) {
        if (threadIdx.x == 0) mwi_scalar_stage3<K>(q, p);
        if (threadIdx.x == 0 && p.stamps) {
            const int me = blockIdx.x + gridDim.x * (blockIdx.y + gridDim.y * blockIdx.z);
            unsigned long long t0 = ~0ull;
            const int nw = gridDim.x * gridDim.y * gridDim.z;
            for (int w = 0; w < nw && w < 256; w++) t0 = mwk::g_mws_stamp[w][0] < t0 ? mwk::g_mws_stamp[w][0] : t0;
            p.stamps[8] = t0;
            { const int sel[6] = {0, 2, 4, 6, 7, 5}; for (int i = 0; i < 6; i++) p.stamps[9 + i] = mwk::g_mws_stamp[me][sel[i]]; }
            p.stamps[15] = wall_clock64();
        }
    }
    return;
#endif
    if (mwi_last_block(&p.flags[4], 2u * q.NB) && threadIdx.x == 0) mwi_scalar_stage3<K>(q, p);
}

template <int K>
__global__ __launch_bounds__(MW_NT) void k_mwi_init(const MwDev q, const MwIpmDev p, double omega_p, double omega_d) {
    const MwBlk &k = q.blk[blockIdx.x];
    const int n = k.n;
    for (int e = threadIdx.x; e < n * n; e += MW_NT) {
        const int i = e % n, c = e / n;
        for (int l = 0; l < K; l++) {
            p.X[(long)l * q.xylen + k.xyoff + e] = (l == 0 && i == c) ? omega_p : 0.0;
            p.Y[(long)l * q.xylen + k.xyoff + e] = (l == 0 && i == c) ? omega_d : 0.0;
        }
    }
}
```

### clusteredlowranksolver.jl_amd/csrc/clrs_mw_ipm_host.inc

```
struct MwIpm {
    MwIpmDev d = {};
    bool ready = false;
    int iter = 0;
    bool xy_with_tail = false;
    bool upd_recorded = false;
    int sync_seq = 0;
    bool global_set = false;
    int gs_world = 0;
    bool forked = false, tail_pending = false;
    bool frozen = false;
    int held_refine_bits = 0;
    bool aff_ok = false;
    double *AX = nullptr;
    int kf_now = 0;
    double *h_rec = nullptr;
    double *d_rec = nullptr;
    size_t sm_Z = 0, sm_Zi = 0, sm_step = 0;
    int zs = MWI_ZS;
    int zs_step = MWI_ZS;
    size_t sm_bmm = 0;
    bool z_tiled = false;
    size_t maxn_inv = 0;
    bool lds_ZL = false, step_w_lds = true, step_inv = false, y_with_x = false, any_xinv = false, any_xsub = false;
    hipStream_t side = nullptr;
// ... 10 lines not shown
    delete c->ipm;
    c->ipm = nullptr;
}

extern "C" int clrs_mw_ipm_create_ex(clrs_mw_ctx *c, const clrs_ipm_data *data, int data_limbs);
extern "C" int clrs_mw_ipm_create(clrs_mw_ctx *c, const clrs_ipm_data *data) { return clrs_mw_ipm_create_ex(c, data, 1); }

extern "C" int clrs_mw_ipm_create_ex(clrs_mw_ctx *c, const clrs_ipm_data *data, int data_limbs) {
    if (!c || !data) return mw_fail(CLRS_ERR_INVALID, "null argument");
    if (data_limbs < 1 || data_limbs > c->DK) return mw_fail(CLRS_ERR_INVALID, "data limbs of the objective exceed those of the context");
    MWCHECK(hipSetDevice(c->device));
    const MwDev &q = c->d;
    const int K = c->K, N = q.N, NB = q.NB;
    if (NB == 0) return mw_fail(CLRS_ERR_INVALID, "no PSD blocks");
    if (!c->ipm) c->ipm = new MwIpm();
    MwIpm *st = c->ipm;
    MwIpmDev &p = st->d;
    int rc;
    if (!st->ready) {
        double **xy[] = {&p.X, &p.Y, &p.dX, &p.dY, &p.R, &p.Xc, &p.Pm};
        for (double **b : xy) if ((rc = mw_dmalloc(c, b, q.xylen * K))) return rc;
        double **xs[] = {&p.x, &p.dx, &p.d, &p.rhsx};
        for (double **b : xs) if ((rc = mw_dmalloc(c, b, q.xlen * K))) return rc;
        double **ys[] = {&p.y, &p.dy, &p.pv};
        for (double **b : ys) if ((rc = mw_dmalloc(c, b, (i64)N * K))) return rc;
        if ((rc = mw_dmalloc(c, &p.coef, q.T * K)) || (rc = mw_dmalloc(c, &p.dtr, q.xlen * K))) return rc;
        p.wBn = 0; p.wB = nullptr;
        if (c->maxTb >= 128) {
            int maxn_lr = 1;
            for (auto &k : c->blk) if (k.kind == 0) maxn_lr = std::max(maxn_lr, k.n);
            p.wBn = maxn_lr;
            if ((rc = mw_dmalloc(c, &p.wB, q.T * (i64)maxn_lr * K))) return rc;
        }
        if ((rc = mw_dmalloc(c, &p.Yi, q.xylen * K)) || (rc = mw_dmalloc(c, &p.Zs, q.xylen * K))) return rc;
        if ((rc = mw_dmalloc(c, &p.Zt, q.xylen * K))) return rc;
        { double *t3 = nullptr; if ((rc = mw_dmalloc(c, &t3, (NB + 1) / 2 + 1))) return rc; p.zcnt = (int *)t3; }
        { double *t2 = nullptr; if ((rc = mw_dmalloc(c, &t2, (NB + 1) / 2 + 1))) return rc; p.yfail = (int *)t2; }
        if ((rc = mw_dmalloc(c, &p.sc, (i64)MSC_COUNT * K))) return rc;
        if ((rc = mw_dmalloc(c, &p.part, 5LL * NB * K))) return rc;
        if ((rc = mw_dmalloc(c, &p.eig, 2LL * NB))) return rc;
        if ((rc = mw_dmalloc(c, &p.Wd, 2LL * q.xylen))) return rc;
        { double *t4 = nullptr; if ((rc = mw_dmalloc(c, &t4, NB + 1))) return rc; p.wcnt = (int *)t4; }
        if ((rc = mw_dmalloc(c, &st->d_rec, 2 * MREC_COUNT))) return rc;
        p.rec = st->d_rec;
        double *tmp = nullptr;
        if ((rc = mw_dmalloc(c, &tmp, 4))) return rc;
        p.fmax = (unsigned long long *)tmp;
        if ((rc = mw_dmalloc(c, &tmp, 4))) return rc;
        p.flags = (int *)tmp;
        if ((rc = mw_dmalloc(c, &tmp, 4))) return rc;
        p.sync = (int *)tmp;
        p.tau = p.ttau = p.utau = nullptr;
        p.klow = K;
        std::vector<int> row_clu((size_t)q.xlen);
        for (int j = 0; j < q.J; j++)
            for (int r = 0; r < c->clu[j].P; r++) row_clu[c->clu[j].coff + r] = j;
        if ((rc = mw_upload(c, row_clu, &p.row_clu))) return rc;
        double *dC, *dc, *db;
        if ((rc = mw_dmalloc(c, &dC, q.xylen * c->DK)) || (rc = mw_dmalloc(c, &dc, q.xlen * c->DK)) || (rc = mw_dmalloc(c, &db, (i64)N * c->DK))) return rc;
        p.C = dC; p.c = dc; p.b = db;
        MWCHECK(hipHostMalloc((void **)&st->h_rec, sizeof(double) * 2 * MREC_COUNT, hipHostMallocDefault));
        MWCHECK(hipStreamCreateWithFlags(&st->side, hipStreamNonBlocking));
        for (int e = 0; e < MwIpm::E_COUNT; e++)
            MWCHECK(hipEventCreateWithFlags(&st->ev[e], e < MwIpm::E_REC0 ? (hipEventDisableTiming | hipEventDisableSystemFence) : hipEventDisableTiming));
        p.Ktot = 0;
        size_t maxn = 0;
        for (auto &k : c->blk) { p.Ktot += k.n; maxn = std::max(maxn, (size_t)k.n); }
        const size_t lim = MW_LDS_MAX / sizeof(double), nnK = maxn * maxn * K;
        if (nnK > lim) return mw_fail(CLRS_ERR_INVALID, "device-resident multi-word iteration needs PSD blocks that fit in LDS");
        st->lds_ZL = 3 * nnK <= lim;
        st->sm_Z = (st->lds_ZL ? 3 : 1) * nnK * 8;
        const size_t step_rest = (size_t)K * maxn + maxn * maxn + 3 * maxn + 2 * MW_NT + MW_POTRF_SCR(K, maxn) + 8;
        st->step_w_lds = 2 * nnK + step_rest <= lim;
        const size_t stepd = (st->step_w_lds ? 2 : 1) * nnK + step_rest;
        if (stepd > lim) return mw_fail(CLRS_ERR_INVALID, "device-resident multi-word iteration needs PSD blocks that fit in LDS");
        st->sm_step = stepd * 8;
        size_t &maxn_inv = st->maxn_inv;
        maxn_inv = 0;
        for (auto &k : c->blk) {
            if (k.inv) { st->any_xinv = true; maxn_inv = std::max(maxn_inv, (size_t)k.n); }
            else st->any_xsub = true;
        }
        {
            const int pc = std::max<int>(1, (MW_PT / MWI_ZL) / (int)std::max<size_t>(maxn_inv, 1)), want = ((int)maxn_inv + pc - 1) / pc;
            const int old_rule = std::max<int>(MWI_ZS, (int)((maxn_inv + 7) / 8));
            st->zs = std::max<int>(old_rule, std::min<int>(want, 320 / std::max(q.NB, 1)));
            {
                const int pcs = std::max<int>(1, 64 / (int)std::max<size_t>(maxn_inv, 1)), wants = ((int)maxn_inv + pcs - 1) / pcs;
                st->zs_step = std::max<int>(old_rule, std::min<int>(wants, 320 / std::max(q.NB, 1)));
            }
        }
        st->z_tiled = maxn_inv > 24;
        st->sm_bmm = (size_t)2 * K * MWI_BT * maxn_inv * 8;
        st->sm_Zi = 2 * maxn_inv * ((maxn_inv + st->zs - 1) / st->zs) * K * 8;
        const size_t step_inv_need = 3 * maxn_inv * maxn_inv * K + step_rest;
        bool all_lds_inv = st->any_xinv;
        for (auto &k : c->blk) all_lds_inv = all_lds_inv && k.inv == 1;
        st->step_inv = all_lds_inv && step_inv_need <= lim;
        const size_t step_need2 = nnK + maxn * maxn + 3 * maxn + 2 * MW_NT + 8;
        st->y_with_x = st->any_xinv && !st->any_xsub && step_need2 <= lim;
        if (st->step_inv) st->sm_step = std::max(st->sm_step, step_inv_need * 8);
        if (st->y_with_x) st->sm_step = std::max(st->sm_step, step_need2 * 8);
        MW_DISPATCH(c, {
            if ((rc = mw_set_lds(k_mwi_Zi<KK>, st->sm_Zi))) return rc;
            if ((rc = mw_set_lds((k_mwi_rows_fwd<KK, DD>), c->sm_fwd))) return rc;
            if ((rc = mw_set_lds(k_mwi_bmm<KK>, st->sm_bmm))) return rc;
            if ((rc = mw_set_lds(k_mwi_Z<KK>, st->sm_Z))) return rc;
            if ((rc = mw_set_lds((k_mwi_step<KK, DD>), st->sm_step))) return rc;
        });
        {
            int mostb = 1;
            for (int j = 0; j < q.J; j++) mostb = std::max(mostb, c->clu[j].b1 - c->clu[j].b0);
            st->aff_ok = N > 0 && !c->wide_solve && (c->lds_q || c->pipe_Q) && mostb < 16 && q.J <= 4 && !q.dn_big && st->any_xinv && !st->any_xsub && !st->z_tiled &&
                         !q.mws_on && !q.mwx_on && c->refine != 0 && g_cfg_mw_affine_corrector != 0;
            if (st->aff_ok) {
                if ((rc = mw_dmalloc(c, &st->AX, q.T * K)) || (rc = mw_dmalloc(c, &p.tau, q.xlen * K)) || (rc = mw_dmalloc(c, &p.ttau, q.xlen * K)) ||
                    (rc = mw_dmalloc(c, &p.utau, (i64)q.J * N * K))) return rc;
            }
        }
        p.beta_infeasible = 0.3; p.beta_feasible = 0.1; p.gamma = 0.9; p.dual_thr = 1e-30; p.primal_thr = 1e-30;
        p.max_gap = 1e100; p.step_thr = 1e-7; p.safe_step = 1; p.corrector_only = 0;
        p.gap_thr = 0.0; p.stop_on = 0; p.need_dual = 0; p.need_primal = 0;
        st->ready = true;
    }
    MWCHECK(hipMemset((void *)p.C, 0, sizeof(double) * q.xylen * c->DK));
    MWCHECK(hipMemset((void *)p.c, 0, sizeof(double) * q.xlen * c->DK));
    if (N) MWCHECK(hipMemset((void *)p.b, 0, sizeof(double) * N * c->DK));
    MWCHECK(hipMemcpy((void *)p.C, data->C, sizeof(double) * q.xylen * data_limbs, hipMemcpyHostToDevice));
    MWCHECK(hipMemcpy((void *)p.c, data->c, sizeof(double) * q.xlen * data_limbs, hipMemcpyHostToDevice));
    if (N) MWCHECK(hipMemcpy((void *)p.b, data->b, sizeof(double) * N * data_limbs, hipMemcpyHostToDevice));
    p.sgn = data->maximize ? 1.0 : -1.0;
    p.constant = data->constant;
    return 0;
}

extern "C" int clrs_mw_ipm_set_params(clrs_mw_ctx *c, const clrs_ipm_params *prm) {
    if (!c || !prm || !c->ipm || !c->ipm->ready) return mw_fail(CLRS_ERR_STATE, "clrs_mw_ipm_create first");
    MwIpmDev &p = c->ipm->d;
    p.beta_infeasible = prm->beta_infeasible; p.beta_feasible = prm->beta_feasible; p.gamma = prm->gamma;
    p.dual_thr = prm->dual_error_threshold; p.primal_thr = prm->primal_error_threshold; p.max_gap = prm->max_complementary_gap;
    p.step_thr = prm->step_length_threshold; p.safe_step = prm->safe_step; p.corrector_only = prm->corrector_only != 0;
    return 0;
}

static int mw_ipm_exchange(clrs_mw_ctx *c, hipStream_t stream, int stage) {
    const MwDev &q = c->d;
    if (q.world <= 1) return 0;
    MwIpm *st = c->ipm;
    const MwIpmDev &p = st->d;
    if (!st->global_set || st->gs_world != q.world) return mw_fail(CLRS_ERR_STATE, "sharded interior-point iteration: clrs_mw_ipm_set_global first");
    const bool onM = stage == 2 || stage == 3;
    MW_DISPATCH(c, hipLaunchKernelGGL((k_mwi_gpack<KK, DD>), dim3(1), dim3(64), 0, stream, q, p, stage));
    MWCHECK(hipGetLastError());
// ... 137 lines not shown
    const MwDev &q = c->d;
    const MwIpmDev &p = c->ipm->d;
    const int maxnn = c->maxn * c->maxn;
    const size_t sm = (size_t)c->maxTb * c->K * 8;
    const bool in_lds = sm <= 48 * 1024;
    MW_DISPATCH(c, {
        if (q.T && !in_lds) hipLaunchKernelGGL((k_mwi_coef<KK, DD>), dim3((unsigned)((q.T + MW_NT - 1) / MW_NT)), dim3(MW_NT), 0, stream, q, p, (const double *)(mode == 0 ? p.x : p.dx));
        const int ew = c->maxTb >= 24 ? 16 : MWI_EW;
        if (p.wBn) hipLaunchKernelGGL((k_mwi_wB<KK, DD>), dim3((unsigned)((q.T * (i64)p.wBn + MW_NT - 1) / MW_NT)), dim3(MW_NT), 0, stream, q, p, mode);
        hipLaunchKernelGGL((k_mwi_wA<KK, DD>), dim3((maxnn * ew + MW_NT - 1) / MW_NT, q.NB), dim3(MW_NT), in_lds && !p.wBn ? sm : 0, stream, q, p, mode, in_lds && !p.wBn ? 1 : 0, p.wBn ? 17 : ew);
    });
    MWCHECK(hipGetLastError());
    return 0;
}
static int mw_ipm_solve_dX(clrs_mw_ctx *c, bool predictor = false) {
    const MwIpmDev &p = c->ipm->d;
    int rc;
    c->refine_skip_next = predictor && !c->refine_predictor;
    if ((rc = clrs_mw_schur_solve_dev(c, p.rhsx, p.pv, p.dx, p.dy))) return rc;
    return mw_ipm_wA(c, c->stream, 1);
}

static int mw_ipm_tail(clrs_mw_ctx *c, int word_value = 0, bool with_next = false) {
    MwIpm *st = c->ipm;
    if (!st->tail_pending) return 0;
    const int par = st->iter & 1;
    int rc;
    if (word_value > 0) hipLaunchKernelGGL(k_mwi_wait<0>, dim3(1), dim3(64), 0, st->side, (const int *)(st->d.sync + 2), word_value, c->d.info, c->d.J + 1);
    else {
        if (!st->upd_recorded) MWCHECK(hipEventRecord(st->ev[MwIpm::E_UPD], c->stream));
        MWCHECK(hipStreamWaitEvent(st->side, st->ev[MwIpm::E_UPD], 0));
    }
    if ((rc = mw_ipm_objectives(c, st->side, word_value != 0 || with_next))) return rc;
    st->xy_with_tail = word_value != 0 || with_next;
    MWCHECK(hipMemcpyAsync(st->h_rec + (size_t)par * MREC_COUNT, st->d.rec, sizeof(double) * MREC_COUNT, hipMemcpyDeviceToHost, st->side));
    MWCHECK(hipEventRecord(st->ev[MwIpm::E_REC0 + par], st->side));
    st->tail_pending = false;
    return 0;
}
static int mw_ipm_enqueue_body(clrs_mw_ctx *c) {
    const MwDev &q = c->d;
    MwIpm *st = c->ipm;
    const int maxnn = c->maxn * c->maxn;
    const size_t sm_red = (size_t)c->K * 8 * 8;
    hipStream_t M = c->stream, S = st->side;
    int rc;
    const bool words = !q.gathered && c->stream_words;
    c->d.kf = st->kf_now;
    const int seq = ++st->sync_seq;
    const MwIpmDev &p = st->d;
    c->ipm_arms_info = true;
    c->d.mark_word = words ? p.sync + 2 : nullptr;
    c->d.mark_value = seq;
    rc = mw_cholesky_blocks_dev2(c, p.X, p.Xc, st->y_with_x ? p.Y : nullptr, p.Yi, p.yfail);
    c->d.mark_word = nullptr;
    if (rc) return rc;
    st->xy_with_tail = false;
    if ((rc = mw_ipm_tail(c, words ? seq : 0, true))) return rc;
    if (!st->forked) {
        MWCHECK(hipEventRecord(st->ev[MwIpm::E_UPD], M));
        MWCHECK(hipStreamWaitEvent(S, st->ev[MwIpm::E_UPD], 0));
        st->forked = true;
    }
    st->iter++;
    st->d.rec = st->d_rec + (size_t)(st->iter & 1) * MREC_COUNT;
    const bool aff = st->aff_ok && !q.gathered;
    c->d.AX = aff ? st->AX : nullptr;
    if ((rc = clrs_mw_schur_assemble_dev(c, p.Xc, p.Y))) return rc;
    if (!words) MWCHECK(hipEventRecord(st->ev[MwIpm::E_ASM], M));
    c->d.mark_word = words ? p.sync + 1 : nullptr;
    const bool split_factor = q.N > 0;
    rc = split_factor ? clrs_mw_schur_factor_local_dev(c) : clrs_mw_schur_factor_dev(c);
    c->d.mark_word = nullptr;
    if (rc) return rc;
    if (split_factor && q.gathered && (rc = mw_allgather(c, 0, q.Qg, (size_t)q.N * q.N * c->K, M))) return rc;
    c->ipm_arms_info = false;
    if (!st->xy_with_tail) {
        MW_DISPATCH(c, hipLaunchKernelGGL((k_mwi_dots<KK, DD>), dim3(q.NB), dim3(MW_NT), sm_red, S, q, p, 1, 0));
        if ((rc = mw_ipm_exchange(c, S, 0))) return rc;
    }
    MW_DISPATCH(c, hipLaunchKernelGGL((k_mwi_scalar<KK, DD>), dim3(1), dim3(1), 0, S, q, p, st->xy_with_tail ? 10 : 0, st->iter));
    MWCHECK(hipGetLastError());
    const bool res_with_tail = st->xy_with_tail && q.world > 1;
    if (res_with_tail) {
        MW_DISPATCH(c, hipLaunchKernelGGL((k_mwi_pvfin<KK, DD>), dim3(1), dim3(MW_NT), 0, S, q, p));
        MWCHECK(hipGetLastError());
    } else if ((rc = mw_ipm_wA(c, S, 0))) return rc;
    MW_DISPATCH(c, hipLaunchKernelGGL(k_mwi_R<KK>, dim3((maxnn * MWI_EW + MW_NT - 1) / MW_NT, q.NB), dim3(MW_NT), 0, S, q, p, 0));
    MWCHECK(hipGetLastError());
    if (words) hipLaunchKernelGGL(k_mwi_wait<0>, dim3(1), dim3(64), 0, S, (const int *)(p.sync + 1), seq, q.info, q.J + 1);
    else MWCHECK(hipStreamWaitEvent(S, st->ev[MwIpm::E_ASM], 0));
    if ((rc = mw_ipm_rhs(c, S, 0))) return rc;
    if ((rc = mw_ipm_trace_rhs(c, S))) return rc;
    MW_DISPATCH(c, {
        if (q.dn_big) hipLaunchKernelGGL((k_mwi_rows_dn<KK, DD>), dim3((unsigned)((q.xlen + MW_NT / 64 - 1) / (MW_NT / 64))), dim3(MW_NT), 0, S, q, p, 0);
    });
    {
        double *const keep_tau = st->d.tau;
        if (!aff) st->d.tau = nullptr;
        rc = mw_ipm_rows(c, S, 0);
        st->d.tau = keep_tau;
        if (rc) return rc;
    }
    if (!res_with_tail) {
        MW_DISPATCH(c, {
            if (q.N) hipLaunchKernelGGL((k_mwi_pv<KK, DD>), dim3((q.N + MW_NT / 8 - 1) / (MW_NT / 8)), dim3(MW_NT), 0, S, q, p, st->iter);
        });
        if ((rc = mw_ipm_exchange(c, S, 1))) return rc;
    }
    MW_DISPATCH(c, {
        if (q.world > 1 && !res_with_tail) hipLaunchKernelGGL((k_mwi_pvfin<KK, DD>), dim3(1), dim3(MW_NT), 0, S, q, p);
        if (q.dn_big) hipLaunchKernelGGL((k_mwi_rows_dn<KK, DD>), dim3((unsigned)((q.xlen + MW_NT / 64 - 1) / (MW_NT / 64))), dim3(MW_NT), 0, S, q, p, 1);
    });
    MWCHECK(hipGetLastError());
    if ((rc = mw_ipm_rows(c, S, 1))) return rc;
    const bool word_sync = words && split_factor && !c->wide_solve && (c->lds_q || c->pipe_Q);
    if (word_sync) hipLaunchKernelGGL(k_mwi_mark<0>, dim3(1), dim3(1), 0, S, p.sync, seq);
    else {
        MWCHECK(hipEventRecord(st->ev[MwIpm::E_PREP], S));
        MWCHECK(hipStreamWaitEvent(M, st->ev[MwIpm::E_PREP], 0));
    }
// ... 32 lines not shown
    } else {
        MW_DISPATCH(c, hipLaunchKernelGGL((k_mwi_scalar<KK, DD>), dim3(1), dim3(1), 0, M, q, p, 2, st->iter));
        MWCHECK(hipGetLastError());
        if ((rc = mw_ipm_rhs(c, M, aff ? 2 : 0))) return rc;
    }
    if ((rc = mw_ipm_trace_rhs(c, M))) return rc;
    {
        int mostb = 1;
        for (int j = 0; j < q.J; j++) mostb = std::max(mostb, c->clu[j].b1 - c->clu[j].b0);
        if (!c->wide_solve && mostb < 16 && q.J <= 64) {
            MW_DISPATCH(c, hipLaunchKernelGGL((k_mwi_rows_fwd<KK, DD>), dim3(q.J), dim3(MW_NT), c->sm_fwd, M, q, p));
            MWCHECK(hipGetLastError());
            c->fwd_rode = true;
        } else if ((rc = mw_ipm_rows(c, M, 1))) return rc;
    }
    if (aff) {
        if (!c->fwd_rode) return mw_fail(CLRS_ERR_STATE, "affine corrector without the fused forward half");
        c->d.aff_mu = p.sc + MSC_MUS; c->d.aff_mu_plane = MSC_COUNT; c->d.aff_rhs = p.tau; c->d.aff_t = p.ttau; c->d.aff_u = p.utau;
        c->d.aff_wait = aff_async ? p.sync + 4 : nullptr; c->d.aff_wait_value = seq;
    }
    rc = mw_ipm_solve_dX(c);
    c->d.aff_mu = nullptr;
    if (rc) return rc;
    if ((rc = mw_ipm_rhs(c, M, 1))) return rc;
    const int ip = st->y_with_x ? 2 : st->step_inv ? 1 : 0, wl = st->step_w_lds ? 1 : 0;
    if (ip == 2 && st->z_tiled) {
        const int nt = ((int)st->maxn_inv + MWI_BT - 1) / MWI_BT;
        MW_DISPATCH(c, {
            hipLaunchKernelGGL(k_mwi_bmm<KK>, dim3(nt * nt, q.NB, 2), dim3(MW_NT), st->sm_bmm, M, q, p, 4, 0);
            hipLaunchKernelGGL(k_mwi_bmm<KK>, dim3(nt * nt, q.NB, 2), dim3(MW_NT), st->sm_bmm, M, q, p, 5, 0);
            hipLaunchKernelGGL((k_mwi_step<KK, DD>), dim3(q.NB, 2, 1), dim3(MW_NT), st->sm_step, M, q, p, wl, 3, st->iter, 0);
        });
    } else
    MW_DISPATCH(c, hipLaunchKernelGGL((k_mwi_step<KK, DD>), dim3(q.NB, 2, ip == 2 ? st->zs_step : 1), dim3(MW_NT), st->sm_step, M, q, p, wl, ip, st->iter, 0));
    if ((rc = mw_ipm_exchange(c, M, 3))) return rc;
    MW_DISPATCH(c, {
        if (q.world > 1) hipLaunchKernelGGL((k_mwi_scalar<KK, DD>), dim3(1), dim3(1), 0, M, q, p, 3, st->iter);
        hipLaunchKernelGGL(k_mwi_update<KK>, dim3((unsigned)std::min<i64>(1024, (q.xylen + q.xlen + q.N + MW_NT - 1) / MW_NT)), dim3(MW_NT), 0, M, q, p);
    });
    MWCHECK(hipGetLastError());
    if (!words) MWCHECK(hipEventRecord(st->ev[MwIpm::E_UPD], M));
    st->upd_recorded = !words;
    st->tail_pending = true;
    return 0;
}
static int mw_ipm_enqueue(clrs_mw_ctx *c) {
    const int rc = mw_ipm_enqueue_body(c);
    c->d.kf = c->kf_entry;
    c->ipm->d.klow = c->K;
    c->d.AX = nullptr; c->d.aff_mu = nullptr; c->d.ride2_rhs = nullptr;
    c->ipm_arms_info = false;
    c->ride_fwd = nullptr;
    c->ride_wait = nullptr;
    c->d.mark_word = nullptr;
    if (rc) { c->fwd_rode = false; c->ipm->tail_pending = false; }
    return rc;
}
static int mw_ipm_finish(clrs_mw_ctx *c) { return mw_ipm_tail(c); }
static void mw_ipm_read_record(const double *r, clrs_ipm_record *out) {
    out->iter = (int)r[MREC_ITER]; out->pd_feas = (int)r[MREC_PDFEAS]; out->error_code = (int)r[MREC_ERR];
    out->factor_status = (int)r[MREC_FSTAT]; out->cholesky_status = (int)r[MREC_XSTAT]; out->refine_bits = (int)r[MREC_REFB];
    out->mu = r[MREC_MU]; out->d_obj = r[MREC_DOBJ]; out->p_obj = r[MREC_POBJ]; out->gap = r[MREC_GAP];
    out->dual_error = r[MREC_DERR]; out->primal_error = r[MREC_PERR]; out->alpha_d = r[MREC_AD]; out->alpha_p = r[MREC_AP];
    out->beta_c = r[MREC_BETA]; out->max_P = r[MREC_MAXP]; out->max_p = r[MREC_MAXp]; out->max_d = r[MREC_MAXd];
}
static int mw_ipm_drain(clrs_mw_ctx *c) {
    MWCHECK(hipStreamSynchronize(c->stream));
    MWCHECK(hipStreamSynchronize(c->ipm->side));
    return 0;
}

extern "C" int clrs_mw_ipm_iterate(clrs_mw_ctx *c, clrs_ipm_record *out) {
    if (!c || !out || !c->ipm || !c->ipm->ready) return mw_fail(CLRS_ERR_STATE, "clrs_mw_ipm_create first");
    MWCHECK(hipSetDevice(c->device));
    MwIpm *st = c->ipm;
    st->d.stop_on = 0;
    int rc;
    if (st->frozen) { MWCHECK(hipMemsetAsync(st->d.flags + 6, 0, sizeof(int), c->stream)); st->frozen = false; }
    const int held = st->held_refine_bits;
    if ((rc = mw_ipm_enqueue(c))) return rc;
    mw_ipm_note_bits(c, held);
    if ((rc = mw_ipm_finish(c))) return rc;
    MWCHECK(hipEventSynchronize(st->ev[MwIpm::E_REC0 + (st->iter & 1)]));
    mw_ipm_read_record(st->h_rec + (size_t)(st->iter & 1) * MREC_COUNT, out);
    st->held_refine_bits = out->refine_bits;
    return 0;
}

static int mw_ipm_solve_body(clrs_mw_ctx *c, const clrs_ipm_stop *stop, clrs_ipm_record_fn on_record, void *user, clrs_ipm_record *records, int max_records, int *n_iter, int *error_code);
extern "C" int clrs_mw_ipm_solve_cb(clrs_mw_ctx *c, const clrs_ipm_stop *stop, clrs_ipm_record_fn on_record, void *user, clrs_ipm_record *records, int max_records,
                                    int *n_iter, int *error_code) {
    if (!c || !stop || !n_iter || !error_code || !c->ipm || !c->ipm->ready) return mw_fail(CLRS_ERR_STATE, "clrs_mw_ipm_create first");
    MWCHECK(hipSetDevice(c->device));
    const int rc = mw_ipm_solve_body(c, stop, on_record, user, records, max_records, n_iter, error_code);
    c->ipm->d.stop_on = 0;
    if (rc) c->ipm->frozen = true;
    return rc;
}
extern "C" int clrs_mw_ipm_solve(clrs_mw_ctx *c, const clrs_ipm_stop *stop, clrs_ipm_record *records, int max_records, int *n_iter, int *error_code) {
    return clrs_mw_ipm_solve_cb(c, stop, nullptr, nullptr, records, max_records, n_iter, error_code);
}
static int mw_ipm_solve_body(clrs_mw_ctx *c, const clrs_ipm_stop *stop, clrs_ipm_record_fn on_record, void *user, clrs_ipm_record *records, int max_records, int *n_iter,
                             int *error_code) {
    MwIpm *st = c->ipm;
    MwIpmDev &p = st->d;
    p.stop_on = 1; p.gap_thr = stop->duality_gap_threshold; p.need_dual = stop->need_dual_feasible; p.need_primal = stop->need_primal_feasible;
// ... 85 lines not shown
```

### clusteredlowranksolver.jl_amd/csrc/clrs_mw_kernels.hip.h

```cpp
#ifndef CLRS_MW_KERNELS_HIP_H
#define CLRS_MW_KERNELS_HIP_H

#include <hip/hip_runtime.h>

#include <type_traits>

#include "clrs_mw_arith.h"

#define MW_NT 256
#define MW_PT 512
#define MW_CT 8
#define MW_INFO_NONE 0x7f7f7f7f
#define MW_INFO_TIMEOUT 0x7f7f7f00
#define MW_WAIT_TICKS 3000000000ull
#define MW_INV_WG 4

typedef long long mwi64;

struct MwBlk {
    int j, n, kind, delta, U, cnt, P, inv;
    mwi64 xyoff;
    mwi64 rd_off;
    mwi64 v_off;
    mwi64 vrow_off;
// ... 18 lines not shown
__host__ __device__ constexpr bool mw_km_ok(int K, int KM) { return KM == K || (KM < K && 2 * KM >= K && (KM <= 6 || KM == 8)); }
#define MW_KM_CASE(KMc) if constexpr (mw_km_ok(K, KMc) && KMc < K) { if (km == KMc) { f(std::integral_constant<int, KMc>{}); return; } }
template <int K, class F>
__device__ __forceinline__ void mw_km_switch(int km, F f) {
    MW_KM_CASE(2) MW_KM_CASE(3) MW_KM_CASE(4) MW_KM_CASE(5) MW_KM_CASE(6) MW_KM_CASE(8)
    f(std::integral_constant<int, K>{});
}

struct MwDev {
    int J, N, NB, nlr, ndn, kf;
    mwi64 xylen, xlen, Slen, T, xrdlen;
    const MwBlk *blk;
    const MwClu *clu;
    const int *lr_list, *dn_list;
    const double *V;
    const int *vrow;
    const int *st_a, *st_b;
    const double *st_lam;
    const int *tptr;
    const int *st_orig, *st_p, *st_war, *st_wac, *st_trl, *st_trd, *st_flag;
    const int *ay_a, *ay_b, *ay_blk;
    const double *dA;
    const int *dmap, *dense_p;
    const int *drow_ptr, *drow_blk, *drow_en;
    int dn_big, maxcnt;
    const double *B;
    mwi64 Vp, lamp, dAp, Bp;
    double *Z, *Tm, *GX, *GY, *W, *Sd;
    mwi64 zlen, glen, wlen, sdlen;
    double *S, *LB, *Q, *Qs;
    double *Xf, *Xb;
    double *xrd, *srd, *qrd;
    double *Si, *Qi;
    double *Xi;
    double *t, *u, *AY;
    double *S0;
    int *mark_word;
    int mark_value, km;
    int pipe_q, pipe_bp;
    unsigned long long *pipe_stamps;
    unsigned long long *pipe_pc;
    double *ub;
    const double *aff_mu, *aff_rhs, *aff_t, *aff_u;
    const int *aff_wait;
    int aff_wait_value, aff_mu_plane;
    const double *ride2_rhs;
    double *ride2_t, *ride2_u;
    double *AX;
    unsigned long long *refstat;
    double *rx2, *u2, *dx2, *dy2;
    const double *uadd;
    int *info;
    int *pcnt;
    int rank, world, gathered, pad3;
    double *Qg, *ug;
    const long long *mws_off;
    int mws_on, mwx_on;
    const long long *mwd_off;
    int mwd_on, pad5;
    const long long *mwx_off;
};

__device__ __forceinline__ void mw_mark(const MwDev &q);
namespace mwk {
using namespace mwa;

typedef __attribute__((address_space(3))) double lds_d;

template <int K, class P>
__device__ __forceinline__ mw<K> ldx(P p, long plane, long i) {
    mw<K> r;
#pragma unroll
    for (int l = 0; l < K; l++) r.l[l] = p[(long)l * plane + i];
    return r;
}
template <int K, class P>
__device__ __forceinline__ void stx(P p, long plane, long i, const mw<K> &v) {
#pragma unroll
    for (int l = 0; l < K; l++) p[(long)l * plane + i] = v.l[l];
}

__device__ __forceinline__ void tri_index(int e, int &ii, int &jj) {
    ii = (int)((__builtin_sqrtf(8.0f * (float)e + 1.0f) - 1.0f) * 0.5f);
    while ((ii + 1) * (ii + 2) / 2 <= e) ii++;
    while (ii * (ii + 1) / 2 > e) ii--;
    jj = e - ii * (ii + 1) / 2;
}

template <int K, int W>
__device__ __forceinline__ mw<K> lanes_sum(mw<K> v) {
#pragma unroll
    for (int off = W / 2; off > 0; off >>= 1) {
        mw<K> o;
#pragma unroll
        for (int l = 0; l < K; l++) o.l[l] = __shfl_xor(v.l[l], off, 64);
        v = add<K>(v, o);
    }
    return v;
}

__device__ __forceinline__ int w_col(int c, int n, int ldw) { return ldw ? c * ldw : c * n - c * (c + 1) / 2; }
__device__ __forceinline__ long w_index(int i, int c, int n, int ldw) { return w_col(c, n, ldw) + i; }
#define MW_TRI(n) ((long)(n) * ((n) + 1) / 2)

__device__ __forceinline__ void pivot_scale(double head, double &p1, double &ph) {
    int ex = ((__double2hiint(head) >> 20) & 0x7ff) - 1023;
    ex += ex & 1;
    p1 = __hiloint2double((1023 - ex) << 20, 0);
    ph = __hiloint2double((1023 - ex / 2) << 20, 0);
}
#define MW_POTRF_SCR(K, n) (2 * (K) * (n))

template <int K, bool INV, int NT = MW_NT, bool UT = !INV, class PM, class PR, class PW>
__device__ __forceinline__ bool wg_potrf(PM M, long plane, int n, int ld, PR rd, long rdplane, PW W, long wplane, int ldw, lds_d *scr, int tid, int cw = 0,
                                         int cnw = 1) {
    if (INV) {
        for (int e = tid; e < n * n; e += NT) {
            const int i = e % n, c = e / n;
            if (ldw && cnw > 1 && c % cnw != cw) continue;
            if (ldw || i >= c) stx<K>(W, wplane, ldw ? i + (long)c * ldw : w_index(i, c, n, 0), i == c ? from_double<K>(1.0) : zero<K>());
        }
        __syncthreads();
    }
    lds_d *fs = scr, *us = scr + (long)K * n;
    mw<K> srun = from_double<K>(1.0);
    if (tid == NT - 1) stx<K>(us, n, 0, srun);
    for (int k = 0; k < n; k++) {
#ifdef MW_STAMPS
        if (tid == 0 && k > 0) g_stamps[k] = wall_clock64();
#endif
        const mw<K> d = ldx<K>(M, plane, k + (long)k * ld);
        if (!(d.l[0] > 0.0)) return false;
        if (k + 1 < n) {
            double p1, ph;
            pivot_scale(d.l[0], p1, ph);
            const mw<K> dh = mul_pow2<K>(d, p1);
            const int m = n - k - 1, trail = m * (m + 1) / 2;
            const int wcols = !INV || k < cw ? 0 : (k - cw) / cnw + 1;
            const int total = trail + m * wcols;
            for (int e = tid; e < total; e += NT) {
                int i, c;
                const bool tr = e < trail;
                if (tr) { tri_index(e, i, c); i += k + 1; c += k + 1; }
                else { const int e2 = e - trail; i = k + 1 + e2 % m; c = cw + cnw * (e2 / m); }
                const mw<K> ci = mul_pow2<K>(ldx<K>(M, plane, i + k * ld), ph);
                const int cb = tr ? c * ld : w_col(c, n, ldw);
                const mw<K> cj = mul_pow2<K>(tr ? ldx<K>(M, plane, c + k * ld) : ldx<K>(W, wplane, cb + k), ph);
                const mw<K> v = tr ? ldx<K>(M, plane, cb + i) : ldx<K>(W, wplane, cb + i);
                acc<K> s;
                acc_zero<K>(s);
                acc_fma<K, K, K>(s, dh, v);
                acc_fma<K, K, K>(s, ci, cj, -1.0);
                const mw<K> r = acc_result<K>(s);
                if (tr) stx<K>(M, plane, cb + i, r);
                else stx<K>(W, wplane, cb + i, r);
            }
            if (tid == NT - 1) {
                srun = mul<K>(srun, dh);
                stx<K>(us, n, k + 1, srun);
                if (INV && (!ldw || cnw == 1 || (k + 1) % cnw == cw)) stx<K>(W, wplane, w_index(k + 1, k + 1, n, ldw), srun);
            }
        }
        __syncthreads();
    }
#ifdef MW_STAMPS
    if (tid == 0) g_stamps[n] = wall_clock64();
#endif
    for (int k = tid; k < n; k += NT) {
        const long kk = k + (long)k * ld;
        const mw<K> sk = ldx<K>(us, n, k), dt = ldx<K>(M, plane, kk);
        const mw<K> f = rsqrt<K>(mul<K>(sk, dt)), rs = mul<K>(f, sk);
        stx<K>(rd, rdplane, k, rs);
        stx<K>(M, plane, kk, mul<K>(dt, f));
        stx<K>(fs, n, k, f);
        if (UT) stx<K>(us, n, k, mul<K>(f, rs));
    }
    __syncthreads();
#ifdef MW_STAMPS
    if (tid == 0) g_stamps[100] = wall_clock64();
#endif
    const int T = n * (n - 1) / 2;
    for (int e = tid; e < (INV ? 2 * T : T); e += NT) {
        int i, c;
        tri_index(e < T ? e : e - T, i, c);
        i += 1;
        if (e < T) {
            const mw<K> a = ldx<K>(M, plane, i + (long)c * ld);
            if (UT) stx<K>(M, plane, c + (long)i * ld, mul<K>(a, ldx<K>(us, n, c)));
            stx<K>(M, plane, i + (long)c * ld, mul<K>(a, ldx<K>(fs, n, c)));
        } else if (c % cnw == cw) {
            const long idx = w_index(i, c, n, ldw);
            stx<K>(W, wplane, idx, mul<K>(ldx<K>(W, wplane, idx), ldx<K>(fs, n, i)));
        }
    }
    if (INV) for (int i = tid; i < n; i += NT) if (!ldw || cnw == 1 || i % cnw == cw) stx<K>(W, wplane, w_index(i, i, n, ldw), ldx<K>(rd, rdplane, i));
    __syncthreads();
#ifdef MW_STAMPS
    if (tid == 0) g_stamps[101] = wall_clock64();
#endif
    return true;
}

template <int K, int NT = MW_NT, class PL, class PR, class PF, class PB>
__device__ __forceinline__ void wg_scaled_factors_u(PL L, long lplane, int ldl, PR rd, long rdplane, int n, PF F, long fplane, int ldf, PB Bk,
                                                    long bplane, int ldb, int tid) {
    for (int e = tid; e < n * n; e += NT) {
        const int i = e % n, k = e / n;
        if (i > k) {
            stx<K>(F, fplane, i + (long)k * ldf, mul<K>(ldx<K>(L, lplane, i + (long)k * ldl), ldx<K>(rd, rdplane, i)));
        } else {
            stx<K>(F, fplane, i + (long)k * ldf, zero<K>());
            stx<K>(Bk, bplane, i + (long)k * ldb, i == k ? zero<K>() : ldx<K>(L, lplane, i + (long)k * ldl));
        }
    }
}

#define MW_TV_W 8
template <int K, class PT, class PV>
__device__ __forceinline__ void wg_trmv_n(PT T, long tplane, int ldt, int n, PV v, long vplane, PV y, long yplane, int tid) {
    const int sub = tid % MW_TV_W;
    for (int i0 = 0; i0 < n; i0 += MW_NT / MW_TV_W) {
        const int i = i0 + tid / MW_TV_W;
        const bool live = i < n;
        const int ii = live ? i : 0;
        acc<K> s;
        acc_zero<K>(s);
        for (int c = sub; c <= ii; c += MW_TV_W) acc_fma<K, K, K>(s, ldx<K>(T, tplane, ii + (long)c * ldt), ldx<K>(v, vplane, c));
        const mw<K> r = lanes_sum<K, MW_TV_W>(acc_result<K>(s));
        if (live && sub == 0) stx<K>(y, yplane, i, r);
    }
    __syncthreads();
}
template <int K, class PT, class PV>
__device__ __forceinline__ void wg_trmv_t(PT T, long tplane, int ldt, int n, PV v, long vplane, PV y, long yplane, int tid) {
    const int sub = tid % MW_TV_W;
    for (int i0 = 0; i0 < n; i0 += MW_NT / MW_TV_W) {
        const int i = i0 + tid / MW_TV_W;
        const bool live = i < n;
        const int ii = live ? i : 0;
        acc<K> s;
        acc_zero<K>(s);
// ... 19 lines not shown
        }
    }
}

template <int K, class PF, class PR, class PB>
__device__ __forceinline__ void wg_trsm_f(PF F, long fplane, int ldf, PR rd, long rdplane, int n, PB B, long bplane, int ldb, int nrhs, int tid) {
    for (int e = tid; e < n * nrhs; e += MW_NT) {
        const int i = e % n, c = e / n;
        const long idx = i + (long)c * ldb;
        stx<K>(B, bplane, idx, mul<K>(ldx<K>(B, bplane, idx), ldx<K>(rd, rdplane, i)));
    }
    __syncthreads();
    for (int k = 0; k < n - 1; k++) {
        const int m = n - k - 1;
        for (int e = tid; e < m * nrhs; e += MW_NT) {
            const int i = k + 1 + e % m, c = e / m;
            const long idx = i + (long)c * ldb;
            stx<K>(B, bplane, idx, fnma<K>(ldx<K>(B, bplane, idx), ldx<K>(F, fplane, i + (long)k * ldf), ldx<K>(B, bplane, k + (long)c * ldb)));
        }
        __syncthreads();
    }
}
template <int K, class PF, class PR, class PB>
__device__ __forceinline__ void wg_trsm_b(PF Bk, long fplane, int ldf, PR rd, long rdplane, int n, PB B, long bplane, int ldb, int nrhs, int tid) {
    for (int e = tid; e < n * nrhs; e += MW_NT) {
        const int i = e % n, c = e / n;
        const long idx = i + (long)c * ldb;
        stx<K>(B, bplane, idx, mul<K>(ldx<K>(B, bplane, idx), ldx<K>(rd, rdplane, i)));
    }
    __syncthreads();
    for (int k = n - 1; k > 0; k--) {
        for (int e = tid; e < k * nrhs; e += MW_NT) {
            const int i = e % k, c = e / k;
            const long idx = i + (long)c * ldb;
            stx<K>(B, bplane, idx, fnma<K>(ldx<K>(B, bplane, idx), ldx<K>(Bk, fplane, i + (long)k * ldf), ldx<K>(B, bplane, k + (long)c * ldb)));
        }
        __syncthreads();
    }
}

__device__ __forceinline__ bool wg_last_block(int *counter, unsigned total) {
    __shared__ int last;
    __threadfence();
    __syncthreads();
    if (threadIdx.x == 0) {
        const unsigned old = atomicAdd((unsigned *)counter, 1u);
        last = (old == total - 1) ? 1 : 0;
        if (last) *counter = 0;
    }
    __syncthreads();
    if (last) __threadfence();
    return last != 0;
}

template <int K, int NT = MW_NT, class PD, class PS>
__device__ __forceinline__ void wg_copy(PD dst, long dplane, int ldd, PS src, long splane, int lds_, int rows, int cols, int tid) {
    constexpr int U = K <= 6 ? 4 : 2;
    const int total = rows * cols;
    for (int e0 = tid; e0 < total; e0 += U * NT) {
        double v[U][K];
#pragma unroll
        for (int u = 0; u < U; u++) {
            const int e = min(e0 + u * NT, total - 1), i = e % rows, c = e / rows;
#pragma unroll
            for (int l = 0; l < K; l++) v[u][l] = src[(long)l * splane + i + (long)c * lds_];
        }
#pragma unroll
        for (int u = 0; u < U; u++) {
            const int e = e0 + u * NT, i = e % rows, c = e / rows;
            if (e < total) {
#pragma unroll
                for (int l = 0; l < K; l++) dst[(long)l * dplane + i + (long)c * ldd] = v[u][l];
            }
        }
    }
}

}

extern __shared__ double mw_lds[];
#define MW_LDS ((mwk::lds_d *)mw_lds)
#ifdef CLRS_MW_STAMPS
#define MW_CHAIN_STAMP(q, idx, cond) do { if ((q).pipe_stamps && (cond)) (q).pipe_stamps[8 * 40 + (idx)] = wall_clock64(); } while (0)
#else
#define MW_CHAIN_STAMP(q, idx, cond) do { } while (0)
#endif

#define MW_X_SHARE 32
__host__ __device__ __forceinline__ bool mw_x_shares(const MwBlk &k) { return k.inv == 1 && k.n > MW_X_SHARE; }
template <int K, bool INV, class PM, class PW>
__device__ __forceinline__ void mw_potrf_x_body(const MwDev &q, const MwBlk &k, PM M, long plane, PW W, long wplane, bool w_in_place, double *__restrict__ Xc, mwk::lds_d *bc,
                                                int tid, int bid) {
    using namespace mwk;
    const int n = k.n;
    const bool share = w_in_place || (INV && mw_x_shares(k));
    const int cw = share ? blockIdx.y : 0, cnw = share ? gridDim.y : 1;
    const bool ok = wg_potrf<K, INV, MW_PT, true>(M, plane, n, n, q.xrd + k.rd_off, q.xrdlen, W, wplane, w_in_place ? n : 0, bc, tid, cw, cnw);
    if (!ok && tid == 0) atomicMin(&q.info[1], bid + 1);
    __syncthreads();
    if (INV && !w_in_place && cnw > 1) {
        for (int e = tid; e < n * n; e += MW_PT) {
            const int i = e % n, c = e / n;
            if (c % cnw != cw) continue;
#pragma unroll
            for (int l = 0; l < K; l++) q.Xi[(long)l * q.xylen + k.xyoff + e] = (ok && i >= c) ? (double)W[(long)l * wplane + w_index(i, c, n, 0)] : 0.0;
        }
    }
    if (cw != 0) return;
    if (ok) wg_scaled_factors_u<K, MW_PT>(M, plane, n, q.xrd + k.rd_off, q.xrdlen, n, q.Xf + k.xyoff, q.xylen, n, q.Xb + k.xyoff, q.xylen, n, tid);
    for (int e = tid; e < n * n; e += MW_PT) {
        const int i = e % n, c = e / n;
#pragma unroll
        for (int l = 0; l < K; l++) {
            Xc[(long)l * q.xylen + k.xyoff + e] = (i >= c) ? (double)M[(long)l * plane + e] : 0.0;
            if (INV && !w_in_place && cnw == 1) q.Xi[(long)l * q.xylen + k.xyoff + e] = (ok && i >= c) ? (double)W[(long)l * wplane + w_index(i, c, n, 0)] : 0.0;
        }
    }
}
template <int K>
__global__ __launch_bounds__(MW_PT) void k_mw_potrf_x(const MwDev q, const double *__restrict__ X, double *__restrict__ Xc, int lds, const double *__restrict__ Y2,
                                                      double *__restrict__ Yi, int *__restrict__ yfail) {
    using namespace mwk;
    mw_mark(q);
    const bool second = (int)blockIdx.x >= q.NB;
    const MwBlk &k = q.blk[second ? blockIdx.x - q.NB : blockIdx.x];
    const int n = k.n, tid = threadIdx.x;
    if (blockIdx.y != 0 && !(lds && (k.inv == 2 || mw_x_shares(k)))) return;
    lds_d *bc = MW_LDS;
    if (second) {
        lds_d *M = MW_LDS + MW_POTRF_SCR(K, n);
        wg_copy<K, MW_PT>(M, (long)n * n, n, Y2 + k.xyoff, q.xylen, n, n, n, tid);
        __syncthreads();
        bool ok;
        if (k.inv == 1) {
            lds_d *W = M + (long)K * n * n, *rdl = W + (long)K * MW_TRI(n);
            const int cw = mw_x_shares(k) ? blockIdx.y : 0, cnw = mw_x_shares(k) ? gridDim.y : 1;
            ok = wg_potrf<K, true, MW_PT, false>(M, (long)n * n, n, n, rdl, n, W, MW_TRI(n), 0, bc, tid, cw, cnw);
            if (ok) {
                for (int e = tid; e < n * n; e += MW_PT) {
                    const int i = e % n, c = e / n;
                    if (c % cnw != cw) continue;
#pragma unroll
                    for (int l = 0; l < K; l++) Yi[(long)l * q.xylen + k.xyoff + e] = (i >= c) ? (double)W[(long)l * MW_TRI(n) + w_index(i, c, n, 0)] : 0.0;
                }
            }
        } else {
            lds_d *rdl = M + (long)K * n * n;
            ok = wg_potrf<K, true, MW_PT, false>(M, (long)n * n, n, n, rdl, n, Yi + k.xyoff, q.xylen, n, bc, tid, blockIdx.y, gridDim.y);
        }
        if (tid == 0 && blockIdx.y == 0) yfail[blockIdx.x - q.NB] = ok ? 0 : 1;
        return;
    }
    if (lds) {
        lds_d *M = MW_LDS + MW_POTRF_SCR(K, n);
        wg_copy<K, MW_PT>(M, (long)n * n, n, X + k.xyoff, q.xylen, n, n, n, tid);
        __syncthreads();
        if (k.inv == 1) mw_potrf_x_body<K, true>(q, k, M, (long)n * n, M + (long)K * n * n, MW_TRI(n), false, Xc, bc, tid, blockIdx.x);
        else if (k.inv == 2) mw_potrf_x_body<K, true>(q, k, M, (long)n * n, q.Xi + k.xyoff, q.xylen, true, Xc, bc, tid, blockIdx.x);
        else mw_potrf_x_body<K, false>(q, k, M, (long)n * n, M, 0, false, Xc, bc, tid, blockIdx.x);
    } else {
        double *M = Xc + k.xyoff;
        wg_copy<K, MW_PT>(M, q.xylen, n, X + k.xyoff, q.xylen, n, n, n, tid);
        __syncthreads();
        mw_potrf_x_body<K, false>(q, k, M, q.xylen, M, 0, false, Xc, bc, tid, blockIdx.x);
    }
}

template <int K, int KM, int DK, int ZW>
__device__ __forceinline__ void mw_zt_products_km(const MwDev &q, const MwBlk &k, const double *__restrict__ Y, int c0, int nc, bool with_z) {
    using namespace mwk;
    const int n = k.n, tid = threadIdx.x, dl = k.delta, sub = tid % ZW;
    const double *V = q.V + k.v_off;
    const int *vrow = q.vrow + k.vrow_off;
    for (int e0 = 0; e0 < n * nc; e0 += MW_NT / ZW) {
        const int e = e0 + tid / ZW;
        const bool live = e < n * nc;
        const int ee = live ? e : 0;
        const int i = ee % n, c = c0 + ee / n, r0 = vrow[c];
        acc<KM> s;
        acc_zero<KM>(s);
        for (int kk = r0 + sub; kk < r0 + dl; kk += ZW) acc_fma<KM, KM, DK>(s, ldx<KM>(Y + k.xyoff, q.xylen, i + (long)kk * n), ldx<DK>(V, q.Vp, kk + (long)c * n));
        mw<KM> v = lanes_sum<KM, ZW>(acc_result<KM>(s));
        if (live && sub == 0) stx<K>(q.Tm + k.z_off, q.zlen, i + (long)c * n, cvt<K, KM>(v));
    }
    if (!with_z) return;
    const double *Xi = q.Xi + k.xyoff;
    for (int e0 = 0; e0 < n * nc; e0 += MW_NT / ZW) {
        const int e = e0 + tid / ZW;
        const bool live = e < n * nc;
        const int ee = live ? e : 0;
        const int i = ee % n, c = c0 + ee / n, r0 = vrow[c];
        acc<KM> s;
        acc_zero<KM>(s);
        for (int kk = r0 + sub; kk <= i; kk += ZW) acc_fma<KM, KM, DK>(s, ldx<KM>(Xi, q.xylen, i + (long)kk * n), ldx<DK>(V, q.Vp, kk + (long)c * n));
        mw<KM> v = lanes_sum<KM, ZW>(acc_result<KM>(s));
        if (live && sub == 0) stx<K>(q.Z + k.z_off, q.zlen, i + (long)c * n, cvt<K, KM>(v));
    }
}
template <int K, int DK, int ZW>
__device__ __forceinline__ void mw_zt_products(const MwDev &q, const MwBlk &k, const double *__restrict__ Y, int c0, int nc, bool with_z) {
    mw_km_switch<K>(q.km, [&](auto kmc) { mw_zt_products_km<K, decltype(kmc)::value, DK, ZW>(q, k, Y, c0, nc, with_z); });
}
template <int K, int DK>
__global__ __launch_bounds__(MW_NT) void k_mw_zt(const MwDev q, const double *__restrict__ Y, int lds_L, int use_inv, int ct) {
    using namespace mwk;
    if (q.mws_on && q.mws_off[q.lr_list[blockIdx.y]] >= 0) return;
    const MwBlk &k = q.blk[q.lr_list[blockIdx.y]];
    const int n = k.n, U = k.U, tid = threadIdx.x;
    const int c0 = blockIdx.x * ct;
    if (c0 >= U) return;
    const int nc = min(ct, U - c0);
    const double *V = q.V + k.v_off;
    if (ct != MW_CT) { mw_zt_products<K, DK, 8>(q, k, Y, c0, nc, true); return; }
    mw_zt_products<K, DK, 2>(q, k, Y, c0, nc, use_inv && k.inv);
    if (use_inv && k.inv) return;
    lds_d *Zt = MW_LDS;
    const long zp = (long)n * MW_CT;
    for (int e = tid; e < n * nc; e += MW_NT) {
        const int i = e % n, c = e / n;
#pragma unroll
        for (int l = 0; l < K; l++) Zt[(long)l * zp + e] = l < DK ? V[(long)l * q.Vp + i + (long)(c0 + c) * n] : 0.0;
    }
    if (lds_L) {
        lds_d *Ls = MW_LDS + (long)K * zp;
        wg_copy<K>(Ls, (long)n * n, n, q.Xf + k.xyoff, q.xylen, n, n, n, tid);
        __syncthreads();
        wg_trsm_f<K>(Ls, (long)n * n, n, q.xrd + k.rd_off, q.xrdlen, n, Zt, zp, n, nc, tid);
    } else {
        __syncthreads();
        wg_trsm_f<K>(q.Xf + k.xyoff, q.xylen, n, q.xrd + k.rd_off, q.xrdlen, n, Zt, zp, n, nc, tid);
    }
    for (int e = tid; e < n * nc; e += MW_NT) {
#pragma unroll
        for (int l = 0; l < K; l++) q.Z[(long)l * q.zlen + k.z_off + (long)c0 * n + e] = Zt[(long)l * zp + e];
    }
}

#ifndef MW_GRAM_W
#define MW_GRAM_W 4
#endif
template <int K, int DK>
__device__ __forceinline__ void mw_dense_1x1(const MwDev &q, const MwBlk &k, const double *__restrict__ Y, int tid) {
    using namespace mwk;
    const int cnt = k.cnt;
    const double *A = q.dA + k.a_off;
    double *W = q.W + k.w_off;
    mw<K> rd = ldx<K>(q.xrd + k.rd_off, q.xrdlen, 0);
    mw<K> yx = mul<K>(ldx<K>(Y + k.xyoff, q.xylen, 0), mul<K>(rd, rd));
    for (int ee = tid; ee < cnt; ee += MW_NT) stx<K>(W, q.wlen, ee, mulx<K, K, DK>(yx, ldx<DK>(A, q.dAp, ee)));
    __syncthreads();
    for (int o = tid; o < cnt * (cnt + 1) / 2; o += MW_NT) {
        int e2, e1;
        tri_index(o, e2, e1);
        const mw<K> v = mulx<K, K, DK>(ldx<K>(W, q.wlen, e1), ldx<DK>(A, q.dAp, e2));
        stx<K>(q.Sd + k.sd_off, q.sdlen, e1 + (long)e2 * cnt, v);
        stx<K>(q.Sd + k.sd_off, q.sdlen, e2 + (long)e1 * cnt, v);
    }
}
template <int K, int KM, int DK>
__device__ __forceinline__ void mw_gram_km(const MwDev &q) {
    using namespace mwk;
    const MwBlk &k = q.blk[q.lr_list[blockIdx.y]];
    const int n = k.n, U = k.U, dl = k.delta;
    const int e = blockIdx.x * (MW_NT / MW_GRAM_W) + threadIdx.x / MW_GRAM_W, sub = threadIdx.x % MW_GRAM_W;
    const int tot = U * (U + 1) / 2;
    if (blockIdx.x * (MW_NT / MW_GRAM_W) >= tot) return;
    const bool live = e < tot;
    int a, b;
    tri_index(live ? e : 0, a, b);
    const double *V = q.V + k.v_off;
    const int *vrow = q.vrow + k.vrow_off;
    const double *Z = q.Z + k.z_off, *T = q.Tm + k.z_off;
    acc<KM> s;
    acc_zero<KM>(s);
    const int i0 = max(vrow[a], vrow[b]);
    for (int i = i0 + sub; i < n; i += MW_GRAM_W) acc_fma<KM, KM, KM>(s, ldx<KM>(Z, q.zlen, i + (long)a * n), ldx<KM>(Z, q.zlen, i + (long)b * n));
    const mw<K> gx = cvt<K, KM>(lanes_sum<KM, MW_GRAM_W>(acc_result<KM>(s)));
    acc_zero<KM>(s);
    const int r0 = vrow[a];
    for (int i = r0 + sub; i < r0 + dl; i += MW_GRAM_W) acc_fma<KM, KM, DK>(s, ldx<KM>(T, q.zlen, i + (long)b * n), ldx<DK>(V, q.Vp, i + (long)a * n));
    const mw<K> gy = cvt<K, KM>(lanes_sum<KM, MW_GRAM_W>(acc_result<KM>(s)));
    if (live && sub == 0) {
        stx<K>(q.GX + k.g_off, q.glen, a + (long)b * U, gx);
        stx<K>(q.GX + k.g_off, q.glen, b + (long)a * U, gx);
        stx<K>(q.GY + k.g_off, q.glen, a + (long)b * U, gy);
        stx<K>(q.GY + k.g_off, q.glen, b + (long)a * U, gy);
    }
}
template <int K, int DK>
__global__ __launch_bounds__(MW_NT) void k_mw_gram(const MwDev q, const double *__restrict__ Y) {
    using namespace mwk;
    if ((int)blockIdx.y >= q.nlr) {
        if (blockIdx.x == 0) mw_dense_1x1<K, DK>(q, q.blk[q.dn_list[blockIdx.y - q.nlr]], Y, threadIdx.x);
        return;
    }
    if (q.mws_on && q.mws_off[q.lr_list[blockIdx.y]] >= 0) return;
    if (q.mwx_on && q.mwx_off[q.lr_list[blockIdx.y]] >= 0) return;
    mw_km_switch<K>(q.km, [&](auto kmc) { mw_gram_km<K, decltype(kmc)::value, DK>(q); });
}

template <int K, int DK>
__global__ __launch_bounds__(MW_NT) void k_mw_dense_t(const MwDev q, const double *__restrict__ Y, int use_inv, int two_buffers, int panels) {
    using namespace mwk;
    const MwBlk &k = q.blk[q.dn_list[blockIdx.x]];
    const int n = k.n, cnt = k.cnt, tid = threadIdx.x, e = blockIdx.y;
    const double *A = q.dA + k.a_off;
    double *W = q.W + k.w_off;
    const long nn = (long)n * n;
    if (n == 1) {
        if (e == 0) mw_dense_1x1<K, DK>(q, k, Y, tid);
        return;
    }
    if (e >= cnt || (panels && use_inv && k.inv && n > 16)) return;
    lds_d *M = MW_LDS, *M2 = M + (long)K * nn;
    if (use_inv && k.inv && two_buffers) {
        const double *Xi = q.Xi + k.xyoff;
        for (int o = tid; o < nn; o += MW_NT) {
            const int i = o % n, c = o / n;
            acc<K> s;
            acc_zero<K>(s);
            for (int r = 0; r <= i; r++) acc_fma<K, K, DK>(s, ldx<K>(Xi, q.xylen, i + (long)r * n), ldx<DK>(A, q.dAp, (long)e * nn + r + (long)c * n));
            stx<K>(M, nn, o, acc_result<K>(s));
        }
        __syncthreads();
        for (int o = tid; o < nn; o += MW_NT) {
            const int i = o % n, c = o / n;
            acc<K> s;
            acc_zero<K>(s);
            for (int r = i; r < n; r++) acc_fma<K, K, K>(s, ldx<K>(Xi, q.xylen, r + (long)i * n), ldx<K>(M, nn, r + (long)c * n));
            stx<K>(M2, nn, o, acc_result<K>(s));
        }
        __syncthreads();
        M = M2;
    } else {
        for (int i = tid; i < nn; i += MW_NT) {
#pragma unroll
            for (int l = 0; l < K; l++) M[(long)l * nn + i] = l < DK ? A[(long)l * q.dAp + (long)e * nn + i] : 0.0;
        }
        __syncthreads();
        wg_trsm_f<K>(q.Xf + k.xyoff, q.xylen, n, q.xrd + k.rd_off, q.xrdlen, n, M, nn, n, n, tid);
// ... 950 lines not shown
```

Baseline: 2334 iterations/s.

## Ride Y-pairing products on X factor kernel, skip unused X factors, lighter chain sync

Adds extra blocks to the X Cholesky kernel that compute the Y-side T and GY pairing products concurrently, so the later zt/gram kernels can skip that work when the small-cluster conditions hold. It also skips writing the scaled Xf/Xb factors when every consumer takes the inverse path. The step-length chain now uses write-through stores and a last-block counter with optional acquire fences in place of full fences. The risks are more complex kernel dispatch and memory-ordering subtleties in the relaxed synchronization.

```diff
diff --git a/clusteredlowranksolver.jl_amd/csrc/clrs_hip.hip b/clusteredlowranksolver.jl_amd/csrc/clrs_hip.hip
--- a/clusteredlowranksolver.jl_amd/csrc/clrs_hip.hip
+++ b/clusteredlowranksolver.jl_amd/csrc/clrs_hip.hip
@@ -59,6 +59,9 @@
 int g_cfg_mw_stream_words = 1;
 int g_cfg_mw_pipeline64 = 1;
 int g_cfg_mw_zt_small_maxn = 64;
+int g_cfg_mw_chain_hop = 1;
+int g_cfg_mw_y_riders = 1;
+int g_cfg_mw_skip_xfb = 1;
 int g_cfg_mw_pipeline_x = 1;
 int g_cfg_mw_pipeline_x_min = 24;
 int g_cfg_mw_sharded_factor_limbs = 1;
@@ -2618,6 +2621,9 @@
     if (!std::strcmp(key, "mw_pipeline_x_min")) { g_cfg_mw_pipeline_x_min = value; return 0; }
     if (!std::strcmp(key, "mw_sharded_factor_limbs")) { g_cfg_mw_sharded_factor_limbs = value; return 0; }
     if (!std::strcmp(key, "mw_stream_words")) { g_cfg_mw_stream_words = value; return 0; }
+    if (!std::strcmp(key, "mw_chain_hop")) { g_cfg_mw_chain_hop = value; return 0; }
+    if (!std::strcmp(key, "mw_skip_xfb")) { g_cfg_mw_skip_xfb = value; return 0; }
+    if (!std::strcmp(key, "mw_y_riders")) { g_cfg_mw_y_riders = value; return 0; }
     if (!std::strcmp(key, "mw_refine_predictor")) { g_cfg_mw_refine_predictor = value; return 0; }
     return fail(CLRS_ERR_INVALID, std::string("unknown configuration key ") + key);
 }
diff --git a/clusteredlowranksolver.jl_amd/csrc/clrs_mw.hip b/clusteredlowranksolver.jl_amd/csrc/clrs_mw.hip
--- a/clusteredlowranksolver.jl_amd/csrc/clrs_mw.hip
+++ b/clusteredlowranksolver.jl_amd/csrc/clrs_mw.hip
@@ -29,6 +29,7 @@
 
 typedef long long i64;
 
+extern int g_cfg_mw_chain_hop, g_cfg_mw_skip_xfb, g_cfg_mw_y_riders;
 extern int g_cfg_mw_stream_words;
 extern int g_cfg_mw_pipeline64;
 extern int g_cfg_mw_zt_small_maxn;
@@ -170,6 +171,9 @@
     int pipe_pcQ = 0;
     unsigned pipe_epoch = 0;
     bool stream_words = true;
+    bool y_riders = true;
+    const double *ride_y = nullptr;
+    int chain_hop = 1;
     bool refine_skip_next = false;
     int refine_predictor = 0;
     int refine = 1;
@@ -476,7 +480,7 @@
         if (c->sm_fwd > MW_LDS_MAX || c->sm_mid > MW_LDS_MAX) MW_BAIL(CLRS_ERR_INVALID, "cluster too large for the multi-word solve kernels");
     }
     MW_DISPATCH(c, {
-        MW_TRY(mw_set_lds(k_mw_potrf_x<KK>, c->sm_x)); MW_TRY(mw_set_lds(k_mw_zt<KK, DD>, c->sm_zt)); MW_TRY(mw_set_lds((k_mw_dense_t<KK, DD>), c->sm_dense));
+        MW_TRY(mw_set_lds(k_mw_potrf_x<KK>, c->sm_x)); MW_TRY(mw_set_lds((k_mw_potrf_x_ride<KK, DD>), c->sm_x)); MW_TRY(mw_set_lds(k_mw_zt<KK, DD>, c->sm_zt)); MW_TRY(mw_set_lds((k_mw_dense_t<KK, DD>), c->sm_dense));
         constexpr int KC = mw_kc(KK);
         const size_t bw = std::min(c->sm_mid + c->sm_bwd, MW_LDS_MAX);
         MW_TRY(mw_set_lds(k_mw_factor<KK>, c->sm_factor)); MW_TRY(mw_set_lds(k_mw_potrf_q<KK>, c->lds_q ? std::max(c->sm_q, c->sm_fwd) : c->sm_fwd));
@@ -724,6 +728,8 @@
     {
         const char *e = std::getenv("CLRS_MW_STREAM_WORDS");
         c->stream_words = e && *e ? std::atoi(e) != 0 : g_cfg_mw_stream_words != 0;
+        c->chain_hop = std::min(std::max(g_cfg_mw_chain_hop, 0), 2);
+        c->y_riders = g_cfg_mw_y_riders != 0;
     }
     c->wide_solve = c->maxP > 64 || N > 64;
     MW_TRY(mw_dmalloc(c, &c->d_Xin, xyoff * K)); MW_TRY(mw_dmalloc(c, &c->d_Xc, xyoff * K)); MW_TRY(mw_dmalloc(c, &c->d_Y, xyoff * K));
@@ -777,6 +783,7 @@
                 maxn_x = std::max(maxn_x, kb.n);
                 working += 2 * ((kb.n + MWP_W - 1) / MWP_W + (kb.n > MWP_N ? MWP_N64 / MWP_W : MWP_WW));
             }
+            q.no_xfb = (all_inv && (!q.dn_big || c->dense_two) && g_cfg_mw_skip_xfb != 0) ? 1 : 0;
             c->pipe_X = cfg_pipe != 0 && K <= 6 && all_inv && maxn_x <= MWP_N64 && g_cfg_mw_pipeline_x != 0 &&
                         (cfg_pipe >= 2 || (maxn_x >= g_cfg_mw_pipeline_x_min && working <= 256));
             if (c->pipe_X) {
@@ -896,6 +903,10 @@
     return 0;
 }
 
+static bool mw_zt_small(const clrs_mw_ctx *c) { return c->all_inv && (i64)c->d.nlr * c->maxU <= 2048 && c->maxn <= g_cfg_mw_zt_small_maxn; }
+static bool mw_y_riders_ok(const clrs_mw_ctx *c) {
+    return c->y_riders && mw_zt_small(c) && c->d.nlr > 0 && c->mws_blocks == 0 && c->mwx_blocks == 0 && !c->pipe_X && !c->d.gathered && c->d.world <= 1;
+}
 static int mw_reset_info(clrs_mw_ctx *c, int which) {
     if (c->ipm_arms_info) return 0;
     MWCHECK(hipMemsetAsync(c->d.info + which, 0x7f, sizeof(int), c->stream));
@@ -921,6 +932,10 @@
         c->pipe_epoch = (c->pipe_epoch + 1) & 0x3ffffff;
         MW_DISPATCH(c, { if constexpr (KK <= 6) { hipLaunchKernelGGL(k_mw_potrf_x_pipe<KK>, dim3(mwp_blocks64(grid)), dim3(MWP_NT64), MWP_LDS_ALONE64, c->stream, c->d, d_X, d_Xchol, d_Y2, d_Yi, d_yfail,
                                                                      c->xpipe_L, c->xpipe_rd, c->xpipe_info, c->pipe_pcx, c->pipe_epoch); } });
+    } else if (c->ride_y && mw_y_riders_ok(c)) {
+        const int ntile = (c->maxU + 1) / 2;
+        MW_DISPATCH(c, hipLaunchKernelGGL((k_mw_potrf_x_ride<KK, DD>), dim3(grid + c->d.nlr * ntile, in_mem && c->lds_x ? MW_INV_WG : 1), dim3(MW_PT), c->sm_x, c->stream, c->d, d_X, d_Xchol,
+                                          c->lds_x ? 1 : 0, d_Y2, d_Yi, d_yfail, c->ride_y, grid, ntile));
     } else
     MW_DISPATCH(c, hipLaunchKernelGGL(k_mw_potrf_x<KK>, dim3(grid, in_mem && c->lds_x ? MW_INV_WG : 1), dim3(MW_PT), c->sm_x, c->stream, c->d, d_X, d_Xchol, c->lds_x ? 1 : 0, d_Y2, d_Yi, d_yfail));
     MWCHECK(hipGetLastError());
@@ -952,7 +967,7 @@
             MwDev q2 = q;
             q2.mws_on = exact ? 1 : 0;
             const int gper = MW_NT / MW_GRAM_W;
-            const int zt_ct = (c->xinv_valid && c->all_inv && (i64)q.nlr * c->maxU <= 2048 && c->maxn <= g_cfg_mw_zt_small_maxn) ? 2 : MW_CT;
+            const int zt_ct = (c->xinv_valid && mw_zt_small(c)) ? 2 : MW_CT;
             hipLaunchKernelGGL((k_mw_zt<KK, DD>), dim3((c->maxU + zt_ct - 1) / zt_ct, q.nlr), dim3(MW_NT), c->sm_zt, c->stream, q2, d_Y, c->lds_zt_L ? 1 : 0, c->xinv_valid ? 1 : 0, zt_ct);
             const bool ride_gram = !dense_done && q.ndn && !q.dn_big;
             dense_done = dense_done || ride_gram;
diff --git a/clusteredlowranksolver.jl_amd/csrc/clrs_mw_inst.h b/clusteredlowranksolver.jl_amd/csrc/clrs_mw_inst.h
--- a/clusteredlowranksolver.jl_amd/csrc/clrs_mw_inst.h
+++ b/clusteredlowranksolver.jl_amd/csrc/clrs_mw_inst.h
@@ -38,6 +38,7 @@
 #define MW_KERNELS_KD(X, K, DK)                                                                                        \
     X __global__ void k_mw_zt<K, DK>(const MwDev, const double *, int, int, int);                                      \
     X __global__ void k_mw_gram<K, DK>(const MwDev, const double *);                                                                   \
+    X __global__ void k_mw_potrf_x_ride<K, DK>(const MwDev, const double *, double *, int, const double *, double *, int *, const double *, int, int); \
     X __global__ void k_mw_dense_t<K, DK>(const MwDev, const double *, int, int, int);                                 \
     X __global__ void k_mw_dense_tp<K, DK>(const MwDev, const double *);                                               \
     X __global__ void k_mw_dense_s<K, DK>(const MwDev, int);                                                           \
diff --git a/clusteredlowranksolver.jl_amd/csrc/clrs_mw_ipm.hip.h b/clusteredlowranksolver.jl_amd/csrc/clrs_mw_ipm.hip.h
--- a/clusteredlowranksolver.jl_amd/csrc/clrs_mw_ipm.hip.h
+++ b/clusteredlowranksolver.jl_amd/csrc/clrs_mw_ipm.hip.h
@@ -21,7 +21,7 @@
     int *wcnt;
     double *rec;
     int *flags;
-    int klow, pad4;
+    int klow, hop;
     double *tau, *ttau, *utau;
     int *sync;
     const double *C, *c, *b;
@@ -322,7 +322,11 @@
     for (int b = 0; b < q.NB; b++) acc_add<K, K>(s, ldx<K>(p.part, 5L * q.NB, (long)slot * q.NB + b));
     return acc_result<K>(s);
 }
-__device__ __forceinline__ bool mwi_last_block(int *counter, unsigned total) { return mwk::wg_last_block(counter, total); }
+__device__ __forceinline__ bool mwi_last_block(const MwIpmDev &p, int *counter, unsigned total) {
+    return p.hop ? mwk::wg_last_block_wt(counter, total, p.hop == 1) : mwk::wg_last_block(counter, total);
+}
+__device__ __forceinline__ void mwi_put_eig(const MwIpmDev &p, long idx, double v) { mwk::st_wt(p.eig + idx, v, p.hop != 0); }
+__device__ __forceinline__ void mwi_put_fail(const MwIpmDev &p) { mwk::st_wt(p.flags + 2, 1, p.hop != 0); }
 template <int K>
 __device__ __noinline__ mwa::mw<K> mwi_gsum(const MwDev &q, const double *gs, int GL, int off) {
     using namespace mwk;
@@ -344,9 +348,9 @@
 #pragma unroll
     for (int w = 0; w < 2; w++)
 #pragma unroll
-        for (int b = 0; b < 8; b++) pev[w][b] = (pre && b < q.NB) ? p.eig[(long)w * q.NB + b] : 1e300;
+        for (int b = 0; b < 8; b++) pev[w][b] = (pre && b < q.NB) ? ld_wt(p.eig + (long)w * q.NB + b, p.hop == 2) : 1e300;
     const int f0 = p.flags[0];
-    int f1 = p.flags[1], f2 = p.flags[2];
+    int f1 = p.flags[1], f2 = ld_wt(p.flags + 2, p.hop == 2);
     unsigned long long rs[4] = {0ull, 0ull, 0ull, 0ull};
     if (q.refstat) {
         if (q.world > 1) {
@@ -373,8 +377,8 @@
 #pragma unroll
             for (int b = 1; b < 8; b++) mn = fmin(mn, pev[w][b]);
         } else {
-            mn = p.eig[(long)w * q.NB];
-            for (int b = 1; b < q.NB; b++) mn = fmin(mn, p.eig[(long)w * q.NB + b]);
+            mn = ld_wt(p.eig + (long)w * q.NB, p.hop == 2);
+            for (int b = 1; b < q.NB; b++) mn = fmin(mn, ld_wt(p.eig + (long)w * q.NB + b, p.hop == 2));
         }
         const bool unsafe = f0 && !p.safe_step;
         al[w] = (mn > -p.gamma && !unsafe) ? 1.0 : -p.gamma / mn;
@@ -1050,15 +1054,15 @@
         acc_zero<KA>(s);
         for (int r = i + sub; r < n; r += MWI_ZL) acc_fma<KA, KA, KA>(s, ldx<KA>(Xi, q.xylen, r + (long)i * n), ldx<KA>(M2, np, r + (long)cl * n));
         const mw<KA> v = lanes_sum<KA, MWI_ZL>(acc_result<KA>(s));
-        if (live && sub == 0) stx<K>(p.Zs + k.xyoff, q.xylen, i + (long)(c0 + cl) * n, cvt<K, KA>(v));
+        if (live && sub == 0) stx_wt<K>(p.Zs + k.xyoff, q.xylen, i + (long)(c0 + cl) * n, cvt<K, KA>(v), p.hop != 0);
     }
     MWZ_STAMP();
-    if (!mwi_last_block(&p.zcnt[blockIdx.x], zs)) return;
+    if (!mwi_last_block(p, &p.zcnt[blockIdx.x], zs)) return;
     MWZ_STAMP();
     for (int e = tid; e < n * n; e += MW_PT) {
         const int i = e % n, c = e / n;
         if (c > i) continue;
-        const mw<K> v = cvt<K, KA>(mul_pow2<KA>(add<KA>(ldx<KA>(p.Zs + k.xyoff, q.xylen, i + (long)c * n), ldx<KA>(p.Zs + k.xyoff, q.xylen, c + (long)i * n)), 0.5));
+        const mw<K> v = cvt<K, KA>(mul_pow2<KA>(add<KA>(ldx_wt<KA>(p.Zs + k.xyoff, q.xylen, i + (long)c * n, p.hop == 2), ldx_wt<KA>(p.Zs + k.xyoff, q.xylen, c + (long)i * n, p.hop == 2)), 0.5));
         stx<K>(p.dY + k.xyoff, q.xylen, i + (long)c * n, v);
         stx<K>(p.dY + k.xyoff, q.xylen, c + (long)i * n, v);
     }
@@ -1218,10 +1222,10 @@
         if (i >= c)
             for (int r = sub; r <= i; r += SW) acc_fma<KA, KA, KA>(s, ldx<KA>(Li, q.xylen, i + (long)r * n), ldx<KA>(Us, np, r + (long)cl * n));
         const mw<KA> v = lanes_sum<KA, SW>(acc_result<KA>(s));
-        if (live && sub == 0 && i >= c) Wg[i + (long)c * n] = v.l[0];
+        if (live && sub == 0 && i >= c) st_wt(Wg + i + (long)c * n, v.l[0], p.hop != 0);
     }
     MWS_STAMP(2);
-    return mwi_last_block(&p.wcnt[which * q.NB + blockIdx.x], zs);
+    return mwi_last_block(p, &p.wcnt[which * q.NB + blockIdx.x], zs);
 }
 template <int K>
 __device__ __forceinline__ bool mwi_step_panels(const MwDev &q, const MwIpmDev &p, const MwBlk &k, int which, const double *Li, const double *dMg) {
@@ -1245,15 +1249,15 @@
     if (n == 1) {
         if (tid == 0) {
             mw<K> m = ldx<K>(Mg, q.xylen, 0);
-            if (!(m.l[0] > 0.0)) { p.flags[2] = 1; p.eig[(long)which * q.NB + blockIdx.x] = 0.0; }
-            else p.eig[(long)which * q.NB + blockIdx.x] = div<K>(ldx<K>(dMg, q.xylen, 0), m).l[0];
+            if (!(m.l[0] > 0.0)) { mwi_put_fail(p); mwi_put_eig(p, (long)which * q.NB + blockIdx.x, 0.0); }
+            else mwi_put_eig(p, (long)which * q.NB + blockIdx.x, div<K>(ldx<K>(dMg, q.xylen, 0), m).l[0]);
         }
         return true;
     }
     if (inv_path >= 2) {
         lds_d *T1 = MW_LDS, *Wd = T1 + (long)K * nn, *work = Wd + nn;
         if (which == 1 && p.yfail[blockIdx.x]) {
-            if (tid == 0) { p.flags[2] = 1; p.eig[(long)which * q.NB + blockIdx.x] = 0.0; }
+            if (tid == 0) { mwi_put_fail(p); mwi_put_eig(p, (long)which * q.NB + blockIdx.x, 0.0); }
             return true;
         }
         if (gridDim.z > 1 || inv_path == 3) {
@@ -1263,19 +1267,19 @@
             const double *Wg = p.Wd + (long)which * q.xylen + k.xyoff;
             for (int e = tid; e < nn; e += MW_NT) {
                 const int i = e % n, c = e / n;
-                Wl[e] = i >= c ? Wg[e] : Wg[c + (long)i * n];
+                Wl[e] = ld_wt(i >= c ? Wg + e : Wg + c + (long)i * n, p.hop == 2);
             }
             __syncthreads();
             MWS_STAMP(4);
             const double ev = n <= 64 ? wg_min_eig32(Wl, n, wk, tid) : wg_min_eig(Wl, n, wk, tid);
-            if (tid == 0) p.eig[(long)which * q.NB + blockIdx.x] = ev - 1e-5;
+            if (tid == 0) mwi_put_eig(p, (long)which * q.NB + blockIdx.x, ev - 1e-5);
             MWS_STAMP(5);
             return true;
         }
         mwi_step_congruence_inv<K>((which == 0 ? q.Xi : p.Yi) + k.xyoff, q.xylen, n, dMg, q.xylen, T1, Wd, tid);
         __syncthreads();
         const double ev = n <= 64 ? wg_min_eig32(Wd, n, work, tid) : wg_min_eig(Wd, n, work, tid);
-        if (tid == 0) p.eig[(long)which * q.NB + blockIdx.x] = ev - 1e-5;
+        if (tid == 0) mwi_put_eig(p, (long)which * q.NB + blockIdx.x, ev - 1e-5);
         return true;
     }
     if (inv_path && k.inv == 1) {
@@ -1287,14 +1291,14 @@
             wg_copy<K>(Mf, nn, n, Mg, q.xylen, n, n, n, tid);
             __syncthreads();
             if (!wg_potrf<K, true, MW_NT, false>(Mf, nn, n, n, rd, n, Li, nn, n, scr, tid)) {
-                if (tid == 0) { p.flags[2] = 1; p.eig[(long)which * q.NB + blockIdx.x] = 0.0; }
+                if (tid == 0) { mwi_put_fail(p); mwi_put_eig(p, (long)which * q.NB + blockIdx.x, 0.0); }
                 return true;
             }
             mwi_step_congruence_inv<K>(Li, nn, n, dMg, q.xylen, T1, Wd, tid);
         }
         __syncthreads();
         const double ev = n <= 64 ? wg_min_eig32(Wd, n, work, tid) : wg_min_eig(Wd, n, work, tid);
-        if (tid == 0) p.eig[(long)which * q.NB + blockIdx.x] = ev - 1e-5;
+        if (tid == 0) mwi_put_eig(p, (long)which * q.NB + blockIdx.x, ev - 1e-5);
         return true;
     }
     lds_d *F = MW_LDS;
@@ -1309,7 +1313,7 @@
         wg_copy<K>(F, nn, n, Mg, q.xylen, n, n, n, tid);
         __syncthreads();
         if (!wg_potrf<K, false>(F, nn, n, n, rd, n, F, 0, 0, bc, tid)) {
-            if (tid == 0) { p.flags[2] = 1; p.eig[(long)which * q.NB + blockIdx.x] = 0.0; }
+            if (tid == 0) { mwi_put_fail(p); mwi_put_eig(p, (long)which * q.NB + blockIdx.x, 0.0); }
             return true;
         }
         for (int e = tid; e < nn; e += MW_NT) {
@@ -1322,7 +1326,7 @@
     else mwi_step_congruence<K>(F, rd, (which == 0 ? p.R : p.Pm) + k.xyoff, q.xylen, nn, n, dMg, q.xylen, Wd, tid);
     __syncthreads();
     const double ev = n <= 64 ? wg_min_eig32(Wd, n, work, tid) : wg_min_eig(Wd, n, work, tid);
-    if (tid == 0) p.eig[(long)which * q.NB + blockIdx.x] = ev - 1e-5;
+    if (tid == 0) mwi_put_eig(p, (long)which * q.NB + blockIdx.x, ev - 1e-5);
     return true;
 }
 
@@ -1366,7 +1370,7 @@
     if (!mwi_step_body<K>(q, p, w_in_lds, inv_path, which_base)) return;
     if (q.world > 1) return;
 #ifdef CLRS_MW_STAMPS
-    if (mwi_last_block(&p.flags[4], 2u * q.NB)) {
+    if (mwi_last_block(p, &p.flags[4], 2u * q.NB)) {
         if (threadIdx.x == 0) mwi_scalar_stage3<K>(q, p);
         if (threadIdx.x == 0 && p.stamps) {
             const int me = blockIdx.x + gridDim.x * (blockIdx.y + gridDim.y * blockIdx.z);
@@ -1380,7 +1384,7 @@
     }
     return;
 #endif
-    if (mwi_last_block(&p.flags[4], 2u * q.NB) && threadIdx.x == 0) mwi_scalar_stage3<K>(q, p);
+    if (mwi_last_block(p, &p.flags[4], 2u * q.NB) && threadIdx.x == 0) mwi_scalar_stage3<K>(q, p);
 }
 
 template <int K>
diff --git a/clusteredlowranksolver.jl_amd/csrc/clrs_mw_ipm_host.inc b/clusteredlowranksolver.jl_amd/csrc/clrs_mw_ipm_host.inc
--- a/clusteredlowranksolver.jl_amd/csrc/clrs_mw_ipm_host.inc
+++ b/clusteredlowranksolver.jl_amd/csrc/clrs_mw_ipm_host.inc
@@ -86,6 +86,7 @@
         p.sync = (int *)tmp;
         p.tau = p.ttau = p.utau = nullptr;
         p.klow = K;
+        p.hop = c->chain_hop;
         std::vector<int> row_clu((size_t)q.xlen);
         for (int j = 0; j < q.J; j++)
             for (int r = 0; r < c->clu[j].P; r++) row_clu[c->clu[j].coff + r] = j;
@@ -133,6 +134,7 @@
         st->step_inv = all_lds_inv && step_inv_need <= lim;
         const size_t step_need2 = nnK + maxn * maxn + 3 * maxn + 2 * MW_NT + 8;
         st->y_with_x = st->any_xinv && !st->any_xsub && step_need2 <= lim;
+        if (!st->y_with_x && !st->step_inv) c->d.no_xfb = 0;
         if (st->step_inv) st->sm_step = std::max(st->sm_step, step_inv_need * 8);
         if (st->y_with_x) st->sm_step = std::max(st->sm_step, step_need2 * 8);
         MW_DISPATCH(c, {
@@ -376,7 +378,10 @@
     c->ipm_arms_info = true;
     c->d.mark_word = words ? p.sync + 2 : nullptr;
     c->d.mark_value = seq;
+    const bool y_rides = mw_y_riders_ok(c);
+    c->ride_y = y_rides ? p.Y : nullptr;
     rc = mw_cholesky_blocks_dev2(c, p.X, p.Xc, st->y_with_x ? p.Y : nullptr, p.Yi, p.yfail);
+    c->ride_y = nullptr;
     c->d.mark_word = nullptr;
     if (rc) return rc;
     st->xy_with_tail = false;
@@ -390,7 +395,10 @@
     st->d.rec = st->d_rec + (size_t)(st->iter & 1) * MREC_COUNT;
     const bool aff = st->aff_ok && !q.gathered;
     c->d.AX = aff ? st->AX : nullptr;
-    if ((rc = clrs_mw_schur_assemble_dev(c, p.Xc, p.Y))) return rc;
+    c->d.skip_y = y_rides ? 1 : 0;
+    rc = clrs_mw_schur_assemble_dev(c, p.Xc, p.Y);
+    c->d.skip_y = 0;
+    if (rc) return rc;
     if (!words) MWCHECK(hipEventRecord(st->ev[MwIpm::E_ASM], M));
     c->d.mark_word = words ? p.sync + 1 : nullptr;
     const bool split_factor = q.N > 0;
@@ -529,6 +537,8 @@
     c->ipm_arms_info = false;
     c->ride_fwd = nullptr;
     c->ride_wait = nullptr;
+    c->ride_y = nullptr;
+    c->d.skip_y = 0;
     c->d.mark_word = nullptr;
     if (rc) { c->fwd_rode = false; c->ipm->tail_pending = false; }
     return rc;
diff --git a/clusteredlowranksolver.jl_amd/csrc/clrs_mw_kernels.hip.h b/clusteredlowranksolver.jl_amd/csrc/clrs_mw_kernels.hip.h
--- a/clusteredlowranksolver.jl_amd/csrc/clrs_mw_kernels.hip.h
+++ b/clusteredlowranksolver.jl_amd/csrc/clrs_mw_kernels.hip.h
@@ -94,12 +94,12 @@
     const double *uadd;
     int *info;
     int *pcnt;
-    int rank, world, gathered, pad3;
+    int rank, world, gathered, no_xfb;
     double *Qg, *ug;
     const long long *mws_off;
     int mws_on, mwx_on;
     const long long *mwd_off;
-    int mwd_on, pad5;
+    int mwd_on, skip_y;
     const long long *mwx_off;
 };
 
@@ -120,6 +120,28 @@
 __device__ __forceinline__ void stx(P p, long plane, long i, const mw<K> &v) {
 #pragma unroll
     for (int l = 0; l < K; l++) p[(long)l * plane + i] = v.l[l];
+}
+
+template <class T>
+__device__ __forceinline__ void st_wt(T *p, T v, bool wt) {
+    if (wt) __hip_atomic_store(p, v, __ATOMIC_RELAXED, __HIP_MEMORY_SCOPE_AGENT);
+    else *p = v;
+}
+template <class T>
+__device__ __forceinline__ T ld_wt(const T *p, bool wt) {
+    return wt ? __hip_atomic_load(p, __ATOMIC_RELAXED, __HIP_MEMORY_SCOPE_AGENT) : *p;
+}
+template <int K>
+__device__ __forceinline__ void stx_wt(double *p, long plane, long i, const mw<K> &v, bool wt) {
+#pragma unroll
+    for (int l = 0; l < K; l++) st_wt(p + (long)l * plane + i, v.l[l], wt);
+}
+template <int K>
+__device__ __forceinline__ mw<K> ldx_wt(const double *p, long plane, long i, bool wt) {
+    mw<K> r;
+#pragma unroll
+    for (int l = 0; l < K; l++) r.l[l] = ld_wt(p + (long)l * plane + i, wt);
+    return r;
 }
 
 __device__ __forceinline__ void tri_index(int e, int &ii, int &jj) {
@@ -155,7 +177,7 @@
 
 template <int K, bool INV, int NT = MW_NT, bool UT = !INV, class PM, class PR, class PW>
 __device__ __forceinline__ bool wg_potrf(PM M, long plane, int n, int ld, PR rd, long rdplane, PW W, long wplane, int ldw, lds_d *scr, int tid, int cw = 0,
-                                         int cnw = 1) {
+                                         int cnw = 1, bool ut = true) {
     if (INV) {
         for (int e = tid; e < n * n; e += NT) {
             const int i = e % n, c = e / n;
@@ -215,7 +237,7 @@
         stx<K>(rd, rdplane, k, rs);
         stx<K>(M, plane, kk, mul<K>(dt, f));
         stx<K>(fs, n, k, f);
-        if (UT) stx<K>(us, n, k, mul<K>(f, rs));
+        if (UT && ut) stx<K>(us, n, k, mul<K>(f, rs));
     }
     __syncthreads();
 #ifdef MW_STAMPS
@@ -228,7 +250,7 @@
         i += 1;
         if (e < T) {
             const mw<K> a = ldx<K>(M, plane, i + (long)c * ld);
-            if (UT) stx<K>(M, plane, c + (long)i * ld, mul<K>(a, ldx<K>(us, n, c)));
+            if (UT && ut) stx<K>(M, plane, c + (long)i * ld, mul<K>(a, ldx<K>(us, n, c)));
             stx<K>(M, plane, i + (long)c * ld, mul<K>(a, ldx<K>(fs, n, c)));
         } else if (c % cnw == cw) {
             const long idx = w_index(i, c, n, ldw);
@@ -354,6 +376,25 @@
     if (last) __threadfence();
     return last != 0;
 }
+__device__ __forceinline__ bool wg_last_block_wt(int *counter, unsigned total, bool acquire) {
+    __shared__ int last;
+    asm volatile("s_waitcnt vmcnt(0)" ::: "memory");
+    __syncthreads();
+    if (threadIdx.x == 0) {
+        const unsigned old = __hip_atomic_fetch_add((unsigned *)counter, 1u, __ATOMIC_RELAXED, __HIP_MEMORY_SCOPE_AGENT);
+        const int l = (old == total - 1) ? 1 : 0;
+        if (l) {
+            __hip_atomic_store(counter, 0, __ATOMIC_RELAXED, __HIP_MEMORY_SCOPE_AGENT);
+            if (acquire) {
+                __builtin_amdgcn_fence(__ATOMIC_ACQUIRE, "agent");
+                asm volatile("s_waitcnt vmcnt(0)" ::: "memory");
+            }
+        }
+        last = l;
+    }
+    __syncthreads();
+    return last != 0;
+}
 
 template <int K, int NT = MW_NT, class PD, class PS>
 __device__ __forceinline__ void wg_copy(PD dst, long dplane, int ldd, PS src, long splane, int lds_, int rows, int cols, int tid) {
@@ -397,7 +438,8 @@
     const int n = k.n;
     const bool share = w_in_place || (INV && mw_x_shares(k));
     const int cw = share ? blockIdx.y : 0, cnw = share ? gridDim.y : 1;
-    const bool ok = wg_potrf<K, INV, MW_PT, true>(M, plane, n, n, q.xrd + k.rd_off, q.xrdlen, W, wplane, w_in_place ? n : 0, bc, tid, cw, cnw);
+    const bool xfb = !(INV && q.no_xfb);
+    const bool ok = wg_potrf<K, INV, MW_PT, true>(M, plane, n, n, q.xrd + k.rd_off, q.xrdlen, W, wplane, w_in_place ? n : 0, bc, tid, cw, cnw, xfb);
     if (!ok && tid == 0) atomicMin(&q.info[1], bid + 1);
     __syncthreads();
     if (INV && !w_in_place && cnw > 1) {
@@ -409,7 +451,7 @@
         }
     }
     if (cw != 0) return;
-    if (ok) wg_scaled_factors_u<K, MW_PT>(M, plane, n, q.xrd + k.rd_off, q.xrdlen, n, q.Xf + k.xyoff, q.xylen, n, q.Xb + k.xyoff, q.xylen, n, tid);
+    if (ok && xfb) wg_scaled_factors_u<K, MW_PT>(M, plane, n, q.xrd + k.rd_off, q.xrdlen, n, q.Xf + k.xyoff, q.xylen, n, q.Xb + k.xyoff, q.xylen, n, tid);
     for (int e = tid; e < n * n; e += MW_PT) {
         const int i = e % n, c = e / n;
 #pragma unroll
@@ -420,8 +462,8 @@
     }
 }
 template <int K>
-__global__ __launch_bounds__(MW_PT) void k_mw_potrf_x(const MwDev q, const double *__restrict__ X, double *__restrict__ Xc, int lds, const double *__restrict__ Y2,
-                                                      double *__restrict__ Yi, int *__restrict__ yfail) {
+__device__ __forceinline__ void mw_potrf_x_main(const MwDev &q, const double *__restrict__ X, double *__restrict__ Xc, int lds, const double *__restrict__ Y2,
+                                                double *__restrict__ Yi, int *__restrict__ yfail) {
     using namespace mwk;
     mw_mark(q);
     const bool second = (int)blockIdx.x >= q.NB;
@@ -468,8 +510,13 @@
     }
 }
 
+template <int K>
+__global__ __launch_bounds__(MW_PT) void k_mw_potrf_x(const MwDev q, const double *__restrict__ X, double *__restrict__ Xc, int lds, const double *__restrict__ Y2,
+                                                      double *__restrict__ Yi, int *__restrict__ yfail) {
+    mw_potrf_x_main<K>(q, X, Xc, lds, Y2, Yi, yfail);
+}
 template <int K, int KM, int DK, int ZW>
-__device__ __forceinline__ void mw_zt_products_km(const MwDev &q, const MwBlk &k, const double *__restrict__ Y, int c0, int nc, bool with_z) {
+__device__ __forceinline__ void mw_zt_T_km(const MwDev &q, const MwBlk &k, const double *__restrict__ Y, int c0, int nc) {
     using namespace mwk;
     const int n = k.n, tid = threadIdx.x, dl = k.delta, sub = tid % ZW;
     const double *V = q.V + k.v_off;
@@ -485,6 +532,14 @@
         mw<KM> v = lanes_sum<KM, ZW>(acc_result<KM>(s));
         if (live && sub == 0) stx<K>(q.Tm + k.z_off, q.zlen, i + (long)c * n, cvt<K, KM>(v));
     }
+}
+template <int K, int KM, int DK, int ZW>
+__device__ __forceinline__ void mw_zt_products_km(const MwDev &q, const MwBlk &k, const double *__restrict__ Y, int c0, int nc, bool with_z) {
+    using namespace mwk;
+    const int n = k.n, tid = threadIdx.x, sub = tid % ZW;
+    const double *V = q.V + k.v_off;
+    const int *vrow = q.vrow + k.vrow_off;
+    if (!q.skip_y) mw_zt_T_km<K, KM, DK, ZW>(q, k, Y, c0, nc);
     if (!with_z) return;
     const double *Xi = q.Xi + k.xyoff;
     for (int e0 = 0; e0 < n * nc; e0 += MW_NT / ZW) {
@@ -560,34 +615,73 @@
     }
 }
 template <int K, int KM, int DK>
+__device__ __forceinline__ void mw_gram_gy_km(const MwDev &q, const MwBlk &k, int a, int b, int sub, bool live) {
+    using namespace mwk;
+    const int n = k.n, U = k.U, dl = k.delta;
+    const double *V = q.V + k.v_off, *T = q.Tm + k.z_off;
+    acc<KM> s;
+    acc_zero<KM>(s);
+    const int r0 = q.vrow[k.vrow_off + a];
+    for (int i = r0 + sub; i < r0 + dl; i += MW_GRAM_W) acc_fma<KM, KM, DK>(s, ldx<KM>(T, q.zlen, i + (long)b * n), ldx<DK>(V, q.Vp, i + (long)a * n));
+    const mw<K> gy = cvt<K, KM>(lanes_sum<KM, MW_GRAM_W>(acc_result<KM>(s)));
+    if (live && sub == 0) {
+        stx<K>(q.GY + k.g_off, q.glen, a + (long)b * U, gy);
+        stx<K>(q.GY + k.g_off, q.glen, b + (long)a * U, gy);
+    }
+}
+template <int K, int KM, int DK>
 __device__ __forceinline__ void mw_gram_km(const MwDev &q) {
     using namespace mwk;
     const MwBlk &k = q.blk[q.lr_list[blockIdx.y]];
-    const int n = k.n, U = k.U, dl = k.delta;
+    const int n = k.n, U = k.U;
     const int e = blockIdx.x * (MW_NT / MW_GRAM_W) + threadIdx.x / MW_GRAM_W, sub = threadIdx.x % MW_GRAM_W;
     const int tot = U * (U + 1) / 2;
     if (blockIdx.x * (MW_NT / MW_GRAM_W) >= tot) return;
     const bool live = e < tot;
     int a, b;
     tri_index(live ? e : 0, a, b);
-    const double *V = q.V + k.v_off;
     const int *vrow = q.vrow + k.vrow_off;
-    const double *Z = q.Z + k.z_off, *T = q.Tm + k.z_off;
+    const double *Z = q.Z + k.z_off;
     acc<KM> s;
     acc_zero<KM>(s);
     const int i0 = max(vrow[a], vrow[b]);
     for (int i = i0 + sub; i < n; i += MW_GRAM_W) acc_fma<KM, KM, KM>(s, ldx<KM>(Z, q.zlen, i + (long)a * n), ldx<KM>(Z, q.zlen, i + (long)b * n));
     const mw<K> gx = cvt<K, KM>(lanes_sum<KM, MW_GRAM_W>(acc_result<KM>(s)));
-    acc_zero<KM>(s);
-    const int r0 = vrow[a];
-    for (int i = r0 + sub; i < r0 + dl; i += MW_GRAM_W) acc_fma<KM, KM, DK>(s, ldx<KM>(T, q.zlen, i + (long)b * n), ldx<DK>(V, q.Vp, i + (long)a * n));
-    const mw<K> gy = cvt<K, KM>(lanes_sum<KM, MW_GRAM_W>(acc_result<KM>(s)));
     if (live && sub == 0) {
         stx<K>(q.GX + k.g_off, q.glen, a + (long)b * U, gx);
         stx<K>(q.GX + k.g_off, q.glen, b + (long)a * U, gx);
-        stx<K>(q.GY + k.g_off, q.glen, a + (long)b * U, gy);
-        stx<K>(q.GY + k.g_off, q.glen, b + (long)a * U, gy);
-    }
+    }
+    if (!q.skip_y) mw_gram_gy_km<K, KM, DK>(q, k, a, b, sub, live);
+}
+template <int K, int KM, int DK>
+__device__ __forceinline__ void mw_y_pairings_rider_km(const MwDev &q, const MwBlk &k, const double *__restrict__ Y, int c0, int nc) {
+    const bool work = threadIdx.x < MW_NT;
+    if (work) mw_zt_T_km<K, KM, DK, 8>(q, k, Y, c0, nc);
+    __syncthreads();
+    if (!work) return;
+    const int U = k.U, sub = threadIdx.x % MW_GRAM_W, n0 = U - c0, tot = n0 + (nc > 1 ? n0 - 1 : 0);
+    for (int e0 = 0; e0 < tot; e0 += MW_NT / MW_GRAM_W) {
+        const int e = e0 + threadIdx.x / MW_GRAM_W;
+        const bool live = e < tot;
+        const int ee = live ? e : 0;
+        const int b = ee < n0 ? c0 : c0 + 1, a = ee < n0 ? c0 + ee : c0 + 1 + (ee - n0);
+        mw_gram_gy_km<K, KM, DK>(q, k, a, b, sub, live);
+    }
+}
+template <int K, int DK>
+__device__ __forceinline__ void mw_y_pairings_rider(const MwDev &q, const double *__restrict__ Y, int r, int ntile) {
+    if (blockIdx.y != 0) return;
+    const MwBlk &k = q.blk[q.lr_list[r / ntile]];
+    const int c0 = (r % ntile) * 2;
+    if (c0 >= k.U) return;
+    const int nc = min(2, k.U - c0);
+    mw_km_switch<K>(q.km, [&](auto kmc) { mw_y_pairings_rider_km<K, decltype(kmc)::value, DK>(q, k, Y, c0, nc); });
+}
+template <int K, int DK>
+__global__ __launch_bounds__(MW_PT) void k_mw_potrf_x_ride(const MwDev q, const double *__restrict__ X, double *__restrict__ Xc, int lds, const double *__restrict__ Y2,
+                                                           double *__restrict__ Yi, int *__restrict__ yfail, const double *__restrict__ Yr, int base, int ntile) {
+    if ((int)blockIdx.x >= base) { mw_y_pairings_rider<K, DK>(q, Yr, (int)blockIdx.x - base, ntile); return; }
+    mw_potrf_x_main<K>(q, X, Xc, lds, Y2, Yi, yfail);
 }
 template <int K, int DK>
 __global__ __launch_bounds__(MW_NT) void k_mw_gram(const MwDev q, const double *__restrict__ Y) {
```

Measured after the change: 2398 iterations/s (median of 6 runs). 1.03x the previous value.
